# sndels/yuki

Hardware: AMD Instinct MI355X
Metric: Mray/s (primary+secondary), Path integrator @1080p (higher is better)
Workload: dtype f32; 1 GPU; cfg3: city 40x20 displaced icospheres, 1,024,012 triangles, SAH BVH (max_shapes_in_node 1), Path 8 bounces, Stratified 8x8, 1920x1080; triangles=1024012, spp=64, max_depth=8, tiles=8160, partition=single GPU, frames_in_flight=2

## Files before the change

yuki_amd/csrc/yk_context.cpp:

```cpp
#include <hip/hip_runtime.h>

#include <algorithm>
#include <chrono>
#include <cstdio>
#include <cstdlib>
#include <cstring>
#include <mutex>
#include <string>
#include <vector>

#include "yk_internal.h"

extern "C" {

uint32_t yk_abi_version(void) { return YK_ABI_VERSION; }

const char* yk_status_string(yk_status s) {
    switch (s) {
        case YK_OK: return "ok";
        case YK_ERR_INVALID_ARGUMENT: return "invalid argument";
        case YK_ERR_NO_DEVICE: return "no HIP device";
        case YK_ERR_DEVICE: return "HIP error";
        case YK_ERR_OUT_OF_MEMORY: return "out of device memory";
        case YK_ERR_UNSUPPORTED: return "unsupported on the device path";
        case YK_ERR_BVH_BUILD: return "BVH build failed";
        case YK_ERR_CANCELLED: return "cancelled";
        case YK_ERR_STACK_OVERFLOW: return "traversal stack overflow";
    }
    return "unknown";
}

yk_status yk_context_create(int device, yk_context** out) {
    if (!out) return YK_ERR_INVALID_ARGUMENT;
    *out = nullptr;
    int count = 0;
    if (hipGetDeviceCount(&count) != hipSuccess || count <= 0) return YK_ERR_NO_DEVICE;
    if (device < 0 || device >= count) return YK_ERR_INVALID_ARGUMENT;
    if (hipSetDevice(device) != hipSuccess) return YK_ERR_NO_DEVICE;
    yk_context* ctx = new yk_context();
    ctx->device = device;
    hipDeviceProp_t prop;
    if (hipGetDeviceProperties(&prop, device) == hipSuccess) ctx->n_cu = prop.multiProcessorCount;
    if (hipStreamCreateWithFlags(&ctx->stream, hipStreamNonBlocking) != hipSuccess ||
        hipEventCreateWithFlags(&ctx->ws[0].done, hipEventDisableTiming) != hipSuccess ||
        hipEventCreateWithFlags(&ctx->ws[1].done, hipEventDisableTiming) != hipSuccess ||
        hipEventCreateWithFlags(&ctx->ev_in, hipEventDisableTiming) != hipSuccess ||
        hipEventCreateWithFlags(&ctx->ev_out, hipEventDisableTiming) != hipSuccess ||
        hipStreamCreateWithFlags(&ctx->ws[0].side, hipStreamNonBlocking) != hipSuccess ||
        hipEventCreateWithFlags(&ctx->ws[0].ev_shade, hipEventDisableTiming) != hipSuccess ||
        hipEventCreateWithFlags(&ctx->ws[1].ev_shade, hipEventDisableTiming) != hipSuccess ||
        hipEventCreateWithFlags(&ctx->ws[0].ev_acc, hipEventDisableTiming) != hipSuccess ||
        hipEventCreateWithFlags(&ctx->ws[1].ev_acc, hipEventDisableTiming) != hipSuccess ||
        hipEventCreateWithFlags(&ctx->ws[0].ev_batch, hipEventDisableTiming) != hipSuccess ||
        hipEventCreateWithFlags(&ctx->ws[1].ev_batch, hipEventDisableTiming) != hipSuccess) {
        delete ctx;
        return YK_ERR_DEVICE;
    }
    ctx->ws[0].stream = ctx->stream;
    void* host_word = nullptr;
    if (hipHostMalloc(&host_word, 128, hipHostMallocMapped | hipHostMallocCoherent) == hipSuccess) {
        void* dev_word = nullptr;
        if (hipHostGetDevicePointer(&dev_word, host_word, 0) == hipSuccess) {
            ctx->cancel_host = static_cast<unsigned*>(host_word);
            ctx->cancel_host_dev = static_cast<const unsigned*>(dev_word);
            std::memset(host_word, 0, 128);
            ctx->cancel_host[16] = 1u;
        } else {
            (void)hipHostFree(host_word);
        }
    } else {
        (void)hipGetLastError();
    }
    if (const char* w = std::getenv("YK_WIDE_BVH")) ctx->wide_bvh = std::min(std::max(std::atoi(w), 0), 2);
    if (const char* w = std::getenv("YK_PACKET_BOUNCES")) ctx->packet_bounces = std::max(std::atoi(w), 0);
    if (const char* w = std::getenv("YK_PACKET_SHADOW_BOUNCES")) ctx->packet_shadow_bounces = std::max(std::atoi(w), 0);
    if (const char* w = std::getenv("YK_TOP_NODES")) ctx->top_nodes = std::min(std::max(std::atoi(w), 0), YK_TOP_MAX);
    *out = ctx;
    return YK_OK;
}

void yk_context_destroy(yk_context* ctx) {
    if (!ctx) return;
    (void)hipSetDevice(ctx->device);
    (void)hipStreamSynchronize(ctx->stream);
    if (ctx->ws[1].stream) (void)hipStreamSynchronize(ctx->ws[1].stream);
    for (WorkSet& w : ctx->ws) {
        for (int a = 0; a < 2; ++a)
            for (int b = 0; b < 4; ++b) w.path[a][b].release();
        DevBuf* wb[] = {&w.hit, &w.pend, &w.shO, &w.shD, &w.shC, &w.vis, &w.shq, &w.shO2, &w.shD2, &w.shq2, &w.ctrl, &w.spill, &w.spill_side};
        for (DevBuf* b : wb) b->release();
        if (w.done) (void)hipEventDestroy(w.done);
        if (w.ev_shade) (void)hipEventDestroy(w.ev_shade);
        if (w.ev_acc) (void)hipEventDestroy(w.ev_acc);
        if (w.ev_batch) (void)hipEventDestroy(w.ev_batch);
        if (w.side) {
            (void)hipStreamSynchronize(w.side);
            (void)hipStreamDestroy(w.side);
        }
    }
    if (ctx->ws[1].stream) (void)hipStreamDestroy(ctx->ws[1].stream);
    if (ctx->ev_in) (void)hipEventDestroy(ctx->ev_in);
    if (ctx->ev_out) (void)hipEventDestroy(ctx->ev_out);
    DevBuf* all[] = {&ctx->sample_buf, &ctx->pixel_xy, &ctx->pixel_aux, &ctx->tiles, &ctx->tile_off, &ctx->counters, &ctx->stats4, &ctx->hit4};
    for (DevBuf* b : all) b->release();
    for (DevBuf& b : ctx->scratch) b.release();
    ctx->tonemap.partials.release();
    ctx->tonemap.bounds.release();
    ctx->tonemap.samples.release();
    ctx->overlay.ids.release();
    if (ctx->tonemap.staging) (void)hipHostFree(ctx->tonemap.staging);
    if (ctx->tonemap.staged) (void)hipEventDestroy(ctx->tonemap.staged);
    for (hipEvent_t e : ctx->ev_pool) (void)hipEventDestroy(e);
    if (ctx->cancel_stream) {
        (void)hipStreamSynchronize(ctx->cancel_stream);
        (void)hipStreamDestroy(ctx->cancel_stream);
    }
    if (ctx->cancel_host) (void)hipHostFree(ctx->cancel_host);
    (void)hipStreamDestroy(ctx->stream);
    delete ctx;
}

yk_status yk_last_error(const yk_context* ctx, char* buf, size_t cap) {
    if (!ctx || !buf || cap == 0) return YK_ERR_INVALID_ARGUMENT;
    std::snprintf(buf, cap, "%s", ctx->last_error.c_str());
    return YK_OK;
}

void* yk_context_stream(const yk_context* ctx) { return ctx ? (void*)ctx->stream : nullptr; }

yk_status yk_context_set_option(yk_context* ctx, const char* key, int64_t value) {
    if (!ctx || !key) return YK_ERR_INVALID_ARGUMENT;
    YK_LOCK(ctx);
    std::string k(key);
    if (k == "batch_paths") {
        if (value < 64 || value > ((int64_t)1 << 29)) return YK_ERR_INVALID_ARGUMENT;
        ctx->batch_paths = value;
    } else if (k == "sample_buf_cap") {
        if (value < (1 << 20)) return YK_ERR_INVALID_ARGUMENT;
        ctx->sample_buf_cap = value;
    } else if (k == "streams") {
        if (value < 1 || value > 2) return YK_ERR_INVALID_ARGUMENT;
        ctx->streams = value;
    } else if (k == "packet_bounces") {
        if (value < 0) return YK_ERR_INVALID_ARGUMENT;
        ctx->packet_bounces = value;
    } else if (k == "packet_shadow_bounces") {
        if (value < 0) return YK_ERR_INVALID_ARGUMENT;
        ctx->packet_shadow_bounces = value;
    } else if (k == "shade_reorder") {
        ctx->shade_reorder = value != 0;
    } else if (k == "overlap_shadow") {
        ctx->overlap_shadow = value != 0;
    } else if (k == "top_nodes") {
        if (value < 0 || value > YK_TOP_MAX) return YK_ERR_INVALID_ARGUMENT;
        ctx->top_nodes = value;
    } else if (k == "wide_bvh") {
        if (value < 0 || value > 2) return YK_ERR_INVALID_ARGUMENT;
        ctx->wide_bvh = value;
    } else if (k == "bvh_builder") {
        if (value < 0 || value > 1) return YK_ERR_INVALID_ARGUMENT;
        ctx->bvh_builder = value;
    } else if (k == "bvh_small_range") {
        if (value < 0 || value > (1 << 20)) return YK_ERR_INVALID_ARGUMENT;
        ctx->bvh_small_range = value;
    } else if (k == "scene_layout") {
        if (value < 0 || value > 1) return YK_ERR_INVALID_ARGUMENT;
        ctx->scene_layout = value;
    } else if (k == "trace_stage_kernel") {
        if (value < 0 || value > 2) return YK_ERR_INVALID_ARGUMENT;
        ctx->trace_stage_kernel = value;
    } else if (k == "overlay_coop_min") {
        if (value < 1 || value > 65536) return YK_ERR_INVALID_ARGUMENT;
// ... 123 lines not shown
```

yuki_amd/csrc/yk_device.h:

```cpp
#pragma once
#include <hip/hip_runtime.h>
#include <stdint.h>

#include "../../include/yuki_hip.h"
#include "yk_bsdf.h"
#include "yk_rng.h"

namespace yk {

struct DevNode {
    float4 q0, q1, q2;
    uint4 q3;
};
static_assert(sizeof(DevNode) == 64, "DevNode must be 64 bytes");

#define YK_VIS_STRIDE(nl) ((nl) <= 4u ? 4u : (nl))
#define YK_LEAF_BIT 0x80000000u
#define YK_REF_NONE 0xffffffffu
#define YK_AXIS_SHIFT 28
#define YK_AXIS_MASK (3u << YK_AXIS_SHIFT)
#define YK_REF_INDEX_MAX ((1u << YK_AXIS_SHIFT) - 1u)
#define YK_TOP_BIT 0x40000000u
#define YK_TOP_MAX 1023

struct DevNode4 {
    float4 q0, q1, q2, q3, q4, q5;
    uint4 q6, q7;
};
static_assert(sizeof(DevNode4) == 128, "DevNode4 must be 128 bytes");

struct DevLight {
    uint32_t kind;
    float p[3];
    float i[3];
    float cos_total_width, cos_falloff_start;
    float w2l[16];
    float s2w[16];
    float n[3];
    float area;
};

struct DevSphere {
    float o2w[16];
    float w2o[16];
    float radius;
    int material;
    unsigned swaps_handedness;
    unsigned pad;
};

#define YK_PRIM_LAST 1u
#define YK_PRIM_SPHERE 2u
#define YK_PRIM_KIND_SHIFT 4
#define YK_HIT_KIND_SHIFT 28
#define YK_HIT_PRIM_MASK 0x0fffffffu
#define YK_HIT_WORD(prim, pflags) ((int)((prim) | ((((pflags) >> YK_PRIM_KIND_SHIFT) & 7u) << YK_HIT_KIND_SHIFT)))

#define YK_MESH_NORMALS 1u
#define YK_MESH_UVS 2u
#define YK_MESH_SWAPS 4u

struct DevScene {
    const DevNode* nodes;
    const DevNode4* nodes4;
    const DevNode* top_nodes;
    uint32_t n_top;
    const DevNode* top_nodes_any;
    uint32_t n_top_any;
    const float4* tris;
    const uint4* prim_shade;
    const float4* prim_attr;
    const DevSphere* spheres;
    uint32_t n_triangles;
    uint32_t root_ref;
    float root_bmin[3], root_bmax[3];
    const uint32_t* indices;
    const float* points;
    const float* normals;
    const float* uvs;
    const uint32_t* tri_mesh;
    const int32_t* tri_material;
    const int32_t* tri_area_light;
    const uint32_t* mesh_flags;
    const Material* materials;
    const DevLight* lights;
    uint32_t n_lights;
    float background[3];
    const float4* texels;
    const uint4* tex_info;
};

struct DevCamera {
    float c2w[16];
    float r2c[16];
};

struct PathBuffers {
    float4* rayO;
    float4* rayD;
    float4* thru;
    uint4* rngs;
};

#define YK_CTRL_WORDS 1024
#define YK_CTRL_ERR 3
#define YK_CTRL_CANCELLED 2
#define YK_CTRL_CAM_O (YK_CTRL_WORDS + 32)
#define YK_CTRL_ALLOC_WORDS (YK_CTRL_WORDS + 64)
#define YK_CTRL_HEADS 8
#define YK_CTRL_STRIDE 8
#define YK_CTRL_BOUNCE(b) (8 + YK_CTRL_STRIDE * (b))
#define YK_CTRL_SHQ 1
#define YK_CTRL_SHQ2 2
#define YK_CTRL_HEAD 3
#define YK_CTRL_MAX_DEPTH ((YK_CTRL_WORDS - 8) / YK_CTRL_STRIDE - 1)

struct CancelRef {
    const unsigned* host;
    unsigned* dev;
};
#define YK_HEAD_POISON 0xC0000000u

__device__ __forceinline__ bool cancel_raised(const CancelRef& c) { return c.dev && *c.dev != 0u; }
__device__ __forceinline__ bool cancel_relay(const CancelRef& c, unsigned* head) {
    if (!c.host || __hip_atomic_load(c.host, __ATOMIC_RELAXED, __HIP_MEMORY_SCOPE_SYSTEM) == 0u) return false;
    atomicOr(c.dev, 1u);
    atomicMax(head, YK_HEAD_POISON);
    return true;
}

struct RenderParams {
    SamplerCfg sampler;
    uint32_t max_depth;
    uint32_t has_clamp;
    float clamp;
    uint32_t integrator;
    uint32_t spe;
    uint32_t sample_base;
    CancelRef cancel;
};

__device__ __forceinline__ void split_sample_id(uint32_t sid, uint32_t spe, uint32_t& entry, uint32_t& k) {
    if ((spe & (spe - 1u)) == 0u) {
        entry = sid >> (31u - (uint32_t)__clz((int)spe));
        k = sid & (spe - 1u);
    } else {
        entry = sid / spe;
        k = sid % spe;
    }
}

}
```

yuki_amd/csrc/yk_internal.h:

```cpp
#pragma once
#include <hip/hip_runtime.h>

#include <atomic>
#include <chrono>
#include <memory>
#include <mutex>
#include <string>
#include <vector>

#include "yk_device.h"
#include "yk_host.h"
#include "yk_kernels.h"

using namespace yk;

struct DevBuf {
    void* p = nullptr;
    size_t bytes = 0;
    hipError_t ensure(size_t want) {
        if (want <= bytes) return hipSuccess;
        if (p) (void)hipFree(p);
        p = nullptr;
        bytes = 0;
        hipError_t e = hipMalloc(&p, want);
        if (e == hipSuccess) bytes = want;
        return e;
    }
    void release() {
        if (p) (void)hipFree(p);
        p = nullptr;
        bytes = 0;
    }
    template <class T> T* as() const { return reinterpret_cast<T*>(p); }
};

#define YK_BVH_SMALL_RANGE 32

struct yk_context {
    int device = 0;
    hipStream_t stream = nullptr;
    std::string last_error;
    int n_cu = 256;
    int64_t batch_paths = 128 << 20;
    int64_t packet_bounces = 1;
    int64_t packet_shadow_bounces = 1;
    int64_t shade_reorder = 1;
    int64_t overlap_shadow = 1;
    int64_t wide_bvh = 2;
    int64_t top_nodes = YK_TOP_MAX;
    int64_t bvh_builder = 0;
    int64_t bvh_small_range = YK_BVH_SMALL_RANGE;
    int64_t scene_layout = 0;
    int64_t trace_stage_kernel = 0;
    int64_t sample_buf_cap = (int64_t)64 << 30;
    int64_t time_kernels = 1;
    int64_t streams = 2;
    struct WorkSet {
        DevBuf path[2][4];
        DevBuf hit, pend, shO, shD, shC, vis, shq, shO2, shD2, shq2, ctrl, spill, spill_side;
        size_t cap_paths = 0;
        unsigned cap_lights = 0, cap_area = 0, cap_delta = 0;
        hipStream_t stream = nullptr;
        hipStream_t side = nullptr;
        hipEvent_t done = nullptr, ev_shade = nullptr, ev_acc = nullptr;
        hipEvent_t ev_batch = nullptr;
    } ws[2];
    DevBuf sample_buf, pixel_xy, pixel_aux, tiles, tile_off, counters, stats4, hit4, scratch[8];
    std::vector<hipEvent_t> ev_pool;
    hipEvent_t ev_in = nullptr, ev_out = nullptr;
    unsigned* cancel_host = nullptr;
    const unsigned* cancel_host_dev = nullptr;
    hipStream_t cancel_stream = nullptr;
    bool want_cancel_stream = false;
    std::atomic<bool> cancel_raised{false};
    struct ToneMapState {
        DevBuf partials, bounds, samples;
        uint32_t* staging = nullptr;
        size_t staging_words = 0;
        hipEvent_t staged = nullptr;
    } tonemap;
    struct OverlayState {
        DevBuf ids;
        int64_t coop_min = 32;
    } overlay;
    std::recursive_mutex mu;
};

typedef yk_context::WorkSet WorkSet;
static const uint32_t YK_WIDE_MAX_PATHS = 6u << 20;

struct DeviceTree {
    DevBuf nodes, depth, order;
    uint32_t n_nodes = 0, n_shapes = 0;
    uint32_t root_words[8] = {};
    void release() {
        nodes.release();
        depth.release();
        order.release();
    }
};

struct yk_scene {
    int device = -1;
    std::shared_ptr<const HostBvh> bvh;
    std::shared_ptr<HostBvh> bvh_lazy;
    DevBuf tree_nodes, tree_order;
    mutable std::once_flag tree_once;
    mutable std::atomic<uint32_t> tree_fetched{1};
    yk_scene_layout_info layout = {};
    size_t record_bytes[7] = {};
    uint32_t n_triangles = 0, n_spheres = 0, n_lights = 0, n_delta_lights = 0;
    bool wide_auto = false;
    yk_scene_info info;
    yk_bvh_build_info build_info;
    std::vector<uint8_t> shape_kind;
    DevBuf nodes, nodes4, top_nodes, top_nodes_any, tris, prim_shade, prim_attr, indices, points, normals, uvs, tri_mesh, tri_material, tri_area_light, mesh_flags, materials, lights, spheres, texels, tex_info;
    DevScene dev;
    bool on_device = false;
};

static inline DevScene dev_scene_for(const yk_scene* scene, uint64_t n) {
    DevScene ds = scene->dev;
    if (scene->wide_auto && n > YK_WIDE_MAX_PATHS) ds.nodes4 = nullptr;
    return ds;
}

struct yk_tile_list {
    int device = -1;
    std::vector<yk_tile> tiles;
    std::vector<uint16_t> samples;
    std::vector<uint32_t> off;
    DevBuf pixel_xy, pixel_sample;
};

static inline yk_status fail(yk_context* ctx, yk_status st, const std::string& msg) {
    if (ctx) ctx->last_error = msg;
    return st;
}

#define YK_LOCK(ctx) std::lock_guard<std::recursive_mutex> yk_lock_((ctx)->mu)
#define HIP_TRY(ctx, expr)                                                                                           \
    do {                                                                                                             \
        hipError_t _e = (expr);                                                                                      \
        if (_e != hipSuccess) {                                                                                      \
            return fail(ctx, _e == hipErrorOutOfMemory ? YK_ERR_OUT_OF_MEMORY : YK_ERR_DEVICE,                       \
                        std::string(#expr) + ": " + hipGetErrorString(_e));                                          \
        }                                                                                                            \
    } while (0)

#define YK_CATCH(ctx)                                                                                         \
    catch (const std::bad_alloc&) { return fail(ctx, YK_ERR_OUT_OF_MEMORY, "host allocation failed"); }      \
    catch (const std::exception& e) { return fail(ctx, YK_ERR_INVALID_ARGUMENT, std::string("exception: ") + e.what()); }


struct SceneImage;
yk_status yk_build_scene_image(yk_context* opt_ctx, const yk_scene_desc* d, std::shared_ptr<SceneImage>& out, bool device_builder_allowed = true);
yk_status yk_upload_scene_image(yk_context* ctx, const std::shared_ptr<SceneImage>& img, yk_scene** out);

const HostBvh* scene_host_tree(const yk_scene* scene);

static inline double now_seconds() {
    return std::chrono::duration<double>(std::chrono::steady_clock::now().time_since_epoch()).count();
}

bool build_bvh_device(yk_context* ctx, const std::vector<ShapeBounds>& bounds, uint32_t max_shapes_in_node, uint32_t split_method, uint32_t small_range, HostBvh& out, yk_bvh_build_info& bi,
                      DeviceTree* keep = nullptr);
bool build_bvh_levels(const std::vector<ShapeBounds>& bounds, uint32_t max_shapes_in_node, uint32_t split_method, uint32_t small_range, HostBvh& out, yk_bvh_build_info& bi);

uint32_t layout_scene_device(yk_context* ctx, yk_scene* s, const DeviceTree& tree, const uint32_t* d_user_order, const uint8_t* d_mat_kind, bool has_attr, uint32_t tree_depth, bool* order_applied);

Material make_material(const yk_material_desc& m);
DevLight make_light(const yk_light_desc& l);

#define YK_COUNTER_BYTES 256
unsigned* error_block(yk_context* ctx);
CancelRef cancel_ref(yk_context* ctx);
yk_status ensure_work_buffers(yk_context* ctx, WorkSet& ws, size_t paths, unsigned n_lights, unsigned n_delta_lights);
yk_status ensure_spill(yk_context* ctx, WorkSet& ws);
unsigned trace_grid(const yk_context* ctx);
PathBuffers path_buffers(WorkSet& ws, int which);
yk_status make_params(yk_context* ctx, const yk_sampler_desc* smp, const yk_integrator_desc* integ, RenderParams& prm);

struct KernelTimer {
    yk_context* ctx;
    bool on;
    std::vector<std::pair<int, int>> spans[3];
    size_t used = 0;
    int begin(hipStream_t s) {
        if (!on) return -1;
        if (used + 2 > ctx->ev_pool.size()) {
            size_t old = ctx->ev_pool.size();
            ctx->ev_pool.resize(old + 256);
            for (size_t i = old; i < ctx->ev_pool.size(); ++i) (void)hipEventCreate(&ctx->ev_pool[i]);
        }
        int a = (int)used;
        used += 2;
        (void)hipEventRecord(ctx->ev_pool[a], s);
        return a;
    }
    void end(int a, int cls, hipStream_t s) {
        if (a < 0) return;
        (void)hipEventRecord(ctx->ev_pool[a + 1], s);
        spans[cls].push_back(std::make_pair(a, a + 1));
    }
    double total(int cls) {
        double ms = 0.0;
        for (auto& sp : spans[cls]) {
            float t = 0.0f;
            if (hipEventElapsedTime(&t, ctx->ev_pool[sp.first], ctx->ev_pool[sp.second]) == hipSuccess) ms += t;
        }
        return ms * 1e-3;
    }
};

bool packet_kernel_traces_bounce(const yk_context* ctx, const yk_scene* scene, unsigned b);
void run_bounces(yk_context* ctx, WorkSet& ws, hipStream_t st, const yk_scene* scene, const RenderParams& prm, const uint32_t* pixel_xy,
                 const uint32_t* sample_index_tab, float4* sample_buf, KernelTimer& kt, unsigned long long* counters, bool coherent,
                 uint32_t n_paths, uint32_t sid_base, bool lean_camera_bounce, uint32_t* n_shadow_launches = nullptr);
```

yuki_amd/csrc/yk_kernels.h:

```cpp
#pragma once
#include <hip/hip_runtime.h>

#include "yk_device.h"

namespace yk {

unsigned trace_block_size();
unsigned trace_spill_depth();
unsigned trace_top_nodes();
unsigned trace_top_nodes_any();
unsigned packet_blocks_per_cu();
void launch_trace_closest_packet(hipStream_t s, unsigned grid, const DevScene& sc, const float4* rayO, const float4* rayD, const unsigned* count_ptr,
                                 unsigned* head, int* hit_tri, unsigned long long* ray_counter, const float4* lean_origin = nullptr, CancelRef cancel = CancelRef{nullptr, nullptr});
void launch_trace_any_packet(hipStream_t s, unsigned grid, const DevScene& sc, const float4* shO, const float4* shD, const unsigned* slot_of,
                             const unsigned* count_ptr, unsigned* head, unsigned char* vis, unsigned long long* shadow_counter, CancelRef cancel = CancelRef{nullptr, nullptr});
unsigned trace_blocks_per_cu();

void launch_pixel_table(hipStream_t s, const yk_tile* tiles, const uint32_t* tile_offset, uint32_t n_tiles, uint32_t n_pixels, uint32_t* pixel_xy,
                        const uint16_t* tile_sample = nullptr, uint32_t* pixel_sample = nullptr);
void launch_pixel_table_one(hipStream_t s, const yk_tile& tile, uint32_t n_pixels, uint32_t* pixel_xy, uint32_t tile_sample, uint32_t* pixel_sample);
void launch_raygen(hipStream_t s, const DevCamera& cam, const RenderParams& prm, const uint32_t* pixel_xy, const uint32_t* pixel_sample, uint64_t work0,
                   uint32_t n, PathBuffers out, float4* sample_buf, unsigned* count, float4* lean_origin = nullptr, const uint4* pixel_aux = nullptr);
void launch_pixel_sampler(hipStream_t s, const SamplerCfg& cfg, const uint32_t* pixel_xy, uint32_t n_pixels, uint4* pixel_aux);
void launch_raygen_user(hipStream_t s, const RenderParams& prm, const float* o, const float* d, const uint16_t* pixel, const uint32_t* sample_index,
                        uint32_t dimension, uint32_t n, PathBuffers out, float4* sample_buf, uint32_t* pixel_xy, unsigned* ctrl);
void launch_trace_closest(hipStream_t s, unsigned grid, const DevScene& sc, const float4* rayO, const float4* rayD, const float* t_max_opt,
                          const unsigned* count_ptr, unsigned* head, int* hit_tri, float4* hit_out, uint4* stats_out, uint2* spill,
                          unsigned spill_stride, unsigned* ctrl, unsigned long long* ray_counter, const unsigned* cancel_host = nullptr);
void launch_whitted(hipStream_t s, unsigned grid, const DevScene& sc, const RenderParams& prm, const uint32_t* pixel_xy, const uint32_t* sample_index_tab,
                    PathBuffers cur, uint32_t n, float4* sample_buf, uint2* spill, unsigned spill_stride, unsigned* ctrl, unsigned long long* counters);
unsigned whitted_max_depth();
void launch_path_debug(hipStream_t s, unsigned grid, const DevScene& sc, const RenderParams& prm, const uint32_t* pixel_xy, const uint32_t* sample_index_tab,
                       PathBuffers cur, uint32_t n, float4* sample_buf, uint32_t* out_counts, float4* out_rays, unsigned ray_cap, uint32_t* out_n_rays,
                       float min_len, uint2* spill, unsigned spill_stride, unsigned* ctrl);
void launch_trace_any(hipStream_t s, unsigned grid, const DevScene& sc, const float4* shO, const float4* shD, const unsigned* slot_of,
                      const unsigned* count_ptr, unsigned* head, unsigned char* vis, uint2* spill, unsigned spill_stride, unsigned* ctrl,
                      unsigned long long* shadow_counter, const unsigned* cancel_host = nullptr);
void launch_shade(hipStream_t s, unsigned grid, const DevScene& sc, const RenderParams& prm, const uint32_t* pixel_xy, const uint32_t* sample_index_tab,
                  PathBuffers cur, PathBuffers nxt, const int* hit_tri, float4* pend, float4* shO, float4* shD, float4* shC, unsigned char* vis,
                  unsigned* shq, float4* shO2, float4* shD2, unsigned* shq2, unsigned* bc, unsigned split_delta, unsigned reorder, unsigned block_slots, unsigned sid_base, const float4* lean_origin);
void launch_accumulate(hipStream_t s, unsigned grid, const RenderParams& prm, PathBuffers cur, const float4* pend, const float4* shC,
                       const unsigned char* vis, unsigned nl, float4* sample_buf, const unsigned* bc, unsigned first, unsigned sid_base);
void launch_resolve(hipStream_t s, const float4* sample_buf, uint32_t n_pixels, uint32_t spp, float* out_rgb);
void launch_resolve_passes(hipStream_t s, const float4* sample_buf, uint32_t n_pixels, uint32_t n_passes, float* out_rgb, size_t pass_stride);
void launch_film_scatter(hipStream_t s, const uint32_t* pixel_xy, uint32_t n_pixels, const float* tile_rgb, uint32_t res_x, float* film_rgb, int accumulate,
                         uint32_t n_passes = 1, size_t pass_stride = 0);
void launch_debug_shade(hipStream_t s, const DevScene& sc, uint32_t integrator, PathBuffers cur, const int* hit_tri, const uint4* stats, uint32_t n,
                        float4* sample_buf);
void launch_device_math(hipStream_t s, int fn, size_t n, const float* a, const float* b, float* out);
void launch_sampler_sequence(hipStream_t s, const SamplerCfg& cfg, uint32_t px, uint32_t py, uint32_t sample_index, const uint8_t* dims, size_t n_draws,
                             float* out);
void launch_light_test(hipStream_t s, const DevLight& L, int index, size_t n, const float* p, const float* ng, const float* u, float* out);
void launch_bsdf_test(hipStream_t s, const Material& m, size_t n, const float* ng, const float* ns, const float* dpdu, const float* wo,
                      const float* wi_or_u, int sample, float* out);
void launch_pack_rays(hipStream_t s, size_t n, const float* o, const float* d, float4* rayO, float4* rayD);
void launch_pack_shadow_rays(hipStream_t s, size_t n, const float* o, const float* d, const float* t_max, const int* area_light, float4* shO,
                             float4* shD);
void launch_unpack_rays(hipStream_t s, size_t n, const float4* rayO, const float4* rayD, float* o, float* d);

}
```

yuki_amd/csrc/yk_kernels.hip:

```cpp
#include <hip/hip_runtime.h>

#include "yk_device.h"
#include "yk_geom.h"
#include "yk_kernels.h"
#include "yk_rng.h"
#include "yk_shade.h"
#include "yk_wave.h"

namespace yk {

__global__ void k_pixel_table(const yk_tile* tiles, const uint32_t* tile_offset, uint32_t n_tiles, uint32_t n_pixels,
                              uint32_t* pixel_xy, const uint16_t* tile_sample, uint32_t* pixel_sample) {
    uint32_t i = blockIdx.x * blockDim.x + threadIdx.x;
    if (i >= n_pixels) return;
    uint32_t lo = 0, hi = n_tiles;
    while (hi - lo > 1) {
        uint32_t mid = (lo + hi) >> 1;
        if (tile_offset[mid] <= i)
            lo = mid;
        else
            hi = mid;
    }
    yk_tile t = tiles[lo];
    uint32_t w = (uint32_t)t.x1 - t.x0;
    uint32_t r = i - tile_offset[lo];
    uint32_t x = t.x0 + r % w, y = t.y0 + r / w;
    pixel_xy[i] = x | (y << 16);
    if (tile_sample) pixel_sample[i] = tile_sample[lo];
}

__global__ void k_pixel_table_one(yk_tile t, uint32_t n_pixels, uint32_t* pixel_xy, uint32_t tile_sample, uint32_t* pixel_sample) {
    uint32_t i = blockIdx.x * blockDim.x + threadIdx.x;
    if (i >= n_pixels) return;
    uint32_t w = (uint32_t)t.x1 - t.x0;
    pixel_xy[i] = (t.x0 + i % w) | ((t.y0 + i / w) << 16);
    if (pixel_sample) pixel_sample[i] = tile_sample;
}

__global__ void k_pixel_sampler(SamplerCfg cfg, const uint32_t* pixel_xy, uint32_t n_pixels, uint4* pixel_aux) {
    uint32_t i = blockIdx.x * blockDim.x + threadIdx.x;
    if (i >= n_pixels) return;
    const uint32_t xy = pixel_xy[i];
    const PixelSampler ps = pixel_sampler(cfg, xy & 0xffffu, xy >> 16);
    pixel_aux[i] = make_uint4((unsigned)ps.stream, (unsigned)(ps.stream >> 32), ps.hash0, 0u);
}

__device__ __forceinline__ void camera_ray(const DevCamera& cam, float fx, float fy, V3& o, V3& d) {
    V3 p_camera = xf_point(cam.r2c, V3{fx, fy, 0.0f});
    V3 dir = normalize(p_camera);
    o = xf_point(cam.c2w, V3{0.0f, 0.0f, 0.0f});
    d = xf_vector(cam.c2w, dir);
}

__global__ void k_raygen(DevCamera cam, RenderParams prm, const uint32_t* pixel_xy, const uint32_t* pixel_sample, uint64_t work0, uint32_t n,
                         PathBuffers out, float4* sample_buf, unsigned* count, float4* lean_origin, const uint4* pixel_aux) {
    uint32_t i = blockIdx.x * blockDim.x + threadIdx.x;
    if (cancel_raised(prm.cancel)) return;
    if (i == 0) *count = n;
    if (i >= n) return;
    const uint32_t w = (uint32_t)(work0 + i);
    uint32_t pix, ks;
    split_sample_id(w, prm.spe, pix, ks);
    const uint32_t s = (pixel_sample ? pixel_sample[pix] : prm.sample_base) + ks;
    uint32_t xy = pixel_xy[pix];
    uint32_t px = xy & 0xffffu, py = xy >> 16;
    SamplerState st;
    float ux, uy;
    if (pixel_aux) {
        const uint4 a = pixel_aux[pix];
        PixelSampler ps;
        ps.stream = (u64)a.x | ((u64)a.y << 32);
        ps.hash0 = a.z;
        st = sampler_start_camera(prm.sampler, ps, px, py, s, ux, uy);
    } else {
        st = sampler_start(prm.sampler, px, py, s, 0);
        sampler_get_2d(prm.sampler, st, ux, uy);
    }
    V3 o, d;
    camera_ray(cam, (float)px + ux, (float)py + uy, o, d);
    if (lean_origin) {
        if (i == 0) *lean_origin = make_float4(o.x, o.y, o.z, __uint_as_float(0u));
    } else {
        out.rayO[i] = make_float4(o.x, o.y, o.z, __uint_as_float(0u));
        out.thru[i] = make_float4(1.0f, 1.0f, 1.0f, __uint_as_float(st.dimension));
    }
    out.rayD[i] = make_float4(d.x, d.y, d.z, __uint_as_float((uint32_t)w));
    out.rngs[i] = make_uint4((unsigned)st.rng.state, (unsigned)(st.rng.state >> 32), (unsigned)st.rng.inc, (unsigned)(st.rng.inc >> 32));
    if (prm.integrator != YK_INTEGRATOR_PATH || prm.max_depth == 0) sample_buf[w] = make_float4(0.0f, 0.0f, 0.0f, 0.0f);
}

__global__ void k_raygen_user(RenderParams prm, const float* ray_o, const float* ray_d, const uint16_t* pixel, const uint32_t* sample_index,
                              uint32_t dimension, uint32_t n, PathBuffers out, float4* sample_buf, uint32_t* pixel_xy, unsigned* count) {
    uint32_t i = blockIdx.x * blockDim.x + threadIdx.x;
    if (i == 0) *count = n;
    if (i >= n) return;
    uint32_t px = pixel[2 * i], py = pixel[2 * i + 1];
    pixel_xy[i] = px | (py << 16);
    SamplerState st = sampler_start(prm.sampler, px, py, sample_index[i], dimension);
    if (prm.sampler.kind == 1) st.dimension = dimension;
    out.rayO[i] = make_float4(ray_o[3 * i], ray_o[3 * i + 1], ray_o[3 * i + 2], __uint_as_float(0u));
    out.rayD[i] = make_float4(ray_d[3 * i], ray_d[3 * i + 1], ray_d[3 * i + 2], __uint_as_float(i));
    out.thru[i] = make_float4(1.0f, 1.0f, 1.0f, __uint_as_float(st.dimension));
    out.rngs[i] = make_uint4((unsigned)st.rng.state, (unsigned)(st.rng.state >> 32), (unsigned)st.rng.inc, (unsigned)(st.rng.inc >> 32));
    if (prm.integrator != YK_INTEGRATOR_PATH || prm.max_depth == 0) sample_buf[i] = make_float4(0.0f, 0.0f, 0.0f, 0.0f);
}

#ifndef SHADE_CAP
#define SHADE_CAP 335
#endif
#ifndef SHADE_CAPQ
#define SHADE_CAPQ 768
#endif
#ifndef SHADE_WIN
#define SHADE_WIN 8
#endif
#ifndef SHADE_MIN_WAVES
#define SHADE_MIN_WAVES 3
#endif
template <int CAP, int CAPQ> struct ShadeStaging {
    float4 pO[CAP], pD[CAP], pT[CAP];
    uint4 pR[CAP];
    float4 qO[CAPQ], qD[CAPQ];
    unsigned qS[CAPQ];
    unsigned fill_p, fill_q, gbase;
    unsigned q_delta;
    unsigned cancel;
    unsigned bucket[8];
    unsigned short order[SHADE_WIN * 256];
};

__device__ __forceinline__ unsigned block_append(bool want, unsigned* lds_fill) {
    unsigned long long mask = __ballot(want);
    unsigned total = (unsigned)__popcll(mask);
    unsigned prefix = (unsigned)__popcll(mask & ((1ull << lane_id()) - 1ull));
    unsigned base = 0;
    if (total && lane_id() == 0) base = atomicAdd(lds_fill, total);
    base = __shfl(base, 0);
    return base + prefix;
}

__device__ __forceinline__ unsigned valid_light_kind(const DevScene& sc, unsigned l) { return sc.lights[l].kind; }

#ifdef YK_SHADE_PROFILE
#include "../../tools/micro/shade_profile.h"
#else
#define YK_PROF_DECL
#define YK_PROF_STAMP(k)
#define YK_PROF_FLUSH
#endif

template <int BLOCK, int CAP, int CAPQ>
__global__ __launch_bounds__(BLOCK, SHADE_MIN_WAVES) void k_shade(DevScene sc, RenderParams prm, const uint32_t* pixel_xy, const uint32_t* sample_index_tab,
                                                 PathBuffers cur, PathBuffers nxt,
                                                 const int* hit_tri, float4* pend, float4* shO, float4* shD, float4* shC, unsigned char* vis,
                                                 unsigned* shq, float4* shO2, float4* shD2, unsigned* shq2, unsigned* bc, unsigned split_delta, unsigned reorder,
                                                 unsigned win_max, unsigned block_slots, unsigned sid_base, const float4* __restrict__ lean_origin) {
    const unsigned win_iters = min(win_max, max(1u, bc[0] / (BLOCK * block_slots)));
    static_assert(sizeof(ShadeStaging<CAP, CAPQ>) <= 53296, "k_shade: more LDS than the measured 53296 bytes per block (42 granules = 53760 cost the third block per CU)");
    __shared__ ShadeStaging<CAP, CAPQ> stg;
    const unsigned nl = sc.n_lights;
    unsigned* next_count = bc + YK_CTRL_STRIDE;
    unsigned* shq_count = bc + YK_CTRL_SHQ;
    if (threadIdx.x == 0) {
        stg.fill_p = 0;
        stg.fill_q = 0;
        stg.q_delta = 0;
        stg.cancel = cancel_raised(prm.cancel) ? 1u : 0u;
    }
    __syncthreads();
    const unsigned n = __builtin_amdgcn_readfirstlane((int)stg.cancel) ? 0u : bc[0];
    auto flush_q = [&](unsigned fill, unsigned delta) {
        if (threadIdx.x == 0) stg.gbase = atomicAdd(delta ? bc + YK_CTRL_SHQ2 : shq_count, fill);
        __syncthreads();
        const unsigned gb = stg.gbase;
        float4* dO = delta ? shO2 : shO;
        float4* dD = delta ? shD2 : shD;
        unsigned* dS = delta ? shq2 : shq;
        for (unsigned k = threadIdx.x; k < fill; k += BLOCK) {
            dO[gb + k] = stg.qO[k];
            dD[gb + k] = stg.qD[k];
            dS[gb + k] = stg.qS[k];
        }
        __syncthreads();
        if (threadIdx.x == 0) stg.fill_q = 0;
        __syncthreads();
    };
    auto flush_p = [&](unsigned fill) {
        if (threadIdx.x == 0) stg.gbase = atomicAdd(next_count, fill);
        __syncthreads();
        const unsigned gb = stg.gbase;
        for (unsigned k = threadIdx.x; k < fill; k += BLOCK) {
            nxt.rayO[gb + k] = stg.pO[k];
            nxt.rayD[gb + k] = stg.pD[k];
            nxt.thru[gb + k] = stg.pT[k];
            nxt.rngs[gb + k] = stg.pR[k];
        }
        __syncthreads();
        if (threadIdx.x == 0) stg.fill_p = 0;
        __syncthreads();
    };
    const bool per_iter = !split_delta && BLOCK * nl <= (unsigned)CAPQ;
    const unsigned WIN = win_iters * BLOCK;
    const unsigned n_win = (n + WIN - 1) / WIN;
    YK_PROF_DECL
    for (unsigned w = blockIdx.x; w < n_win; w += gridDim.x) {
      const unsigned wbase = w * WIN;
      unsigned n_sub = win_iters;
      YK_PROF_STAMP(0)
      if (reorder) {
        if (threadIdx.x < 8) stg.bucket[threadIdx.x] = 0;
        __syncthreads();
        unsigned key[SHADE_WIN], rank[SHADE_WIN];
#pragma unroll
        for (int k = 0; k < SHADE_WIN; ++k) {
            const unsigned i0 = wbase + k * BLOCK + threadIdx.x;
            const bool in = (unsigned)k < win_iters && i0 < n;
            const int t = in ? hit_tri[i0] : -1;
            key[k] = !in ? 7u : (t < 0 ? 6u : ((unsigned)t >> YK_HIT_KIND_SHIFT));
        }
#pragma unroll
        for (int k = 0; k < SHADE_WIN; ++k) {
            rank[k] = 0;
            if ((unsigned)k >= win_iters) continue;
            for (unsigned q = 0; q < 8; ++q) {
                const unsigned long long m = __ballot(key[k] == q);
                if (m == 0ull) continue;
                unsigned b0 = 0;
                if (lane_id() == 0) b0 = atomicAdd(&stg.bucket[q], (unsigned)__popcll(m));
                b0 = __shfl(b0, 0);
                if (key[k] == q) rank[k] = b0 + (unsigned)__popcll(m & ((1ull << lane_id()) - 1ull));
            }
        }
        __syncthreads();
        unsigned first[8];
        {
            unsigned acc = 0;
            for (unsigned q = 0; q < 8; ++q) {
                first[q] = acc;
                acc += stg.bucket[q];
            }
            n_sub = (acc - stg.bucket[7] + BLOCK - 1) / BLOCK;
        }
#pragma unroll
        for (int k = 0; k < SHADE_WIN; ++k)
            if ((unsigned)k < win_iters) stg.order[first[key[k]] + rank[k]] = (unsigned short)(k * BLOCK + threadIdx.x);
        __syncthreads();
      } else {
        const unsigned left = n - wbase;
        n_sub = left >= WIN ? win_iters : (left + BLOCK - 1) / BLOCK;
      }
      for (unsigned sub = 0; sub < n_sub; ++sub) {
        const unsigned i = wbase + (reorder ? (unsigned)stg.order[sub * BLOCK + threadIdx.x] : sub * BLOCK + threadIdx.x);
        const bool valid = i < n;
        bool alive = false;
        YK_PROF_STAMP(1)
        if (per_iter) {
            __syncthreads();
            const unsigned fq = stg.fill_q, fp = stg.fill_p, staged = stg.q_delta;
            __syncthreads();
            if (fq && fq + BLOCK * nl > CAPQ) flush_q(fq, staged);
            if (fp + BLOCK > CAP) flush_p(fp);
        }
        float4 nO = make_float4(0, 0, 0, 0), nD = nO, nT = nO;
        uint4 nR = make_uint4(0, 0, 0, 0);
        V3 o = V3{0, 0, 0}, d = V3{0, 0, 1};
        RGB beta = RGB{0, 0, 0};
        unsigned flags = 0, sid = 0, bounces = 0;
        bool specular_bounce = false, hit = false;
        SamplerState st;
        st.rng.state = 0;
        st.rng.inc = 1;
        st.px = st.py = st.sample_index = st.dimension = 0;
        PathVertex v;
        v.sf.p = v.sf.n = v.sf.ns = v.sf.dpdus = v.sf.wo = V3{0, 0, 1};
        v.sf.material = 0;
        v.sf.area_light = -1;
        v.sf.u = v.sf.v = 0.0f;
        v.mat.kind = MK_BLACK;
        v.fr.s = v.fr.t = v.fr.n = v.fr.ng = V3{0, 0, 1};
        v.wo = V3{0, 0, 1};
        if (valid) {
            float4 a, c;
            const float4 b = cur.rayD[i];
            if (lean_origin) {
                a = *lean_origin;
                c = make_float4(1.0f, 1.0f, 1.0f, __uint_as_float(2u));
            } else {
                a = cur.rayO[i];
                c = cur.thru[i];
            }
            uint4 r = cur.rngs[i];
            o = f4_xyz(a);
            d = f4_xyz(b);
            flags = __float_as_uint(a.w);
            sid = __float_as_uint(b.w);
            beta = RGB{c.x, c.y, c.z};
            bounces = flags & 0xffu;
            specular_bounce = (flags >> 8) & 1u;
            st = path_sampler(prm, pixel_xy, sample_index_tab, r, __float_as_uint(c.w), sid);
            int tri = hit_tri[i];
            hit = tri >= 0;
            if (hit) vertex_setup(sc, (uint32_t)tri & YK_HIT_PRIM_MASK, o, d, v);
        }
        YK_PROF_STAMP(2)
        const unsigned vs = YK_VIS_STRIDE(nl);
        unsigned vword = 0u;
        for (unsigned l = 0; l < nl; ++l) {
            const unsigned slot = i * nl + l, vslot = i * vs + l;
            NeeSample ne;
            ne.want = false;
            ne.contrib = RGB{0, 0, 0};
            ne.so = V3{0, 0, 0};
            ne.sd = V3{0, 0, 1};
            ne.al = -1;
            if (valid && hit) ne = vertex_light(sc, prm, st, l, v);
            const bool want = ne.want;
            if (vs == 4u)
                vword |= (want ? 1u : 0u) << (8u * l);
            else if (valid)
                vis[vslot] = want ? 1 : 0;
            if (!per_iter) {
                __syncthreads();
                const unsigned f = stg.fill_q, staged = stg.q_delta;
                const unsigned delta = (split_delta && valid_light_kind(sc, l) != YK_LIGHT_RECT) ? 1u : 0u;
                __syncthreads();
                if (f && (staged != delta || f + BLOCK > CAPQ)) flush_q(f, staged);
                if (threadIdx.x == 0) stg.q_delta = delta;
            }
            unsigned q = block_append(want, &stg.fill_q);
            if (want) {
                stg.qO[q] = make_float4(ne.so.x, ne.so.y, ne.so.z, 0.9999f);
                stg.qD[q] = make_float4(ne.sd.x, ne.sd.y, ne.sd.z, __uint_as_float((unsigned)ne.al));
                stg.qS[q] = vslot;
                shC[slot] = make_float4(ne.contrib.r, ne.contrib.g, ne.contrib.b, 0.0f);
            }
        }
        if (vs == 4u && valid) reinterpret_cast<unsigned*>(vis)[i] = vword;
        YK_PROF_STAMP(3)
        if (valid) {
            unsigned kind = 0;
            RGB term = RGB{0, 0, 0};
            if (!hit) {
                term = vertex_miss_term(sc, beta);
                kind = YK_PEND_MISS;
            } else {
                VertexEnd e = vertex_finish(sc, prm, st, v, beta, bounces, specular_bounce);
                term = e.term;
                kind = e.kind;
                alive = e.alive;
                if (e.sampled) {
                    nO = make_float4(e.no.x, e.no.y, e.no.z, __uint_as_float((bounces & 0xffu) | (specular_bounce ? 0x100u : 0u)));
                    nD = make_float4(e.wi.x, e.wi.y, e.wi.z, __uint_as_float(sid));
                    nT = make_float4(beta.r, beta.g, beta.b, __uint_as_float(st.dimension));
                    nR = make_uint4((unsigned)st.rng.state, (unsigned)(st.rng.state >> 32), (unsigned)st.rng.inc, (unsigned)(st.rng.inc >> 32));
                }
            }
            pend[i] = make_float4(term.r, term.g, term.b, __uint_as_float((kind << YK_PEND_KIND_SHIFT) | (sid - sid_base)));
        }
        YK_PROF_STAMP(4)
        if (!per_iter) {
            __syncthreads();
            const unsigned f = stg.fill_p;
            __syncthreads();
            if (f + BLOCK > CAP) flush_p(f);
        }
        unsigned j = block_append(alive, &stg.fill_p);
        if (alive) {
            stg.pO[j] = nO;
            stg.pD[j] = nD;
            stg.pT[j] = nT;
            stg.pR[j] = nR;
        }
        YK_PROF_STAMP(5)
      }
      if (reorder) __syncthreads();
    }
    YK_PROF_FLUSH
    __syncthreads();
    {
        const unsigned fq = stg.fill_q, fp = stg.fill_p;
        if (fq) flush_q(fq, stg.q_delta);
        if (fp) flush_p(fp);
    }
}

__global__ void k_accumulate(RenderParams prm, PathBuffers cur, const float4* pend, const float4* shC, const unsigned char* vis, unsigned nl,
                             float4* sample_buf, const unsigned* bc, unsigned first, unsigned sid_base) {
    const unsigned n = cancel_raised(prm.cancel) ? 0u : bc[0];
    for (unsigned i = blockIdx.x * blockDim.x + threadIdx.x; i < n; i += gridDim.x * blockDim.x) {
        float4 p = pend[i];
        const unsigned kind = __float_as_uint(p.w) >> YK_PEND_KIND_SHIFT;
        const unsigned sid = sid_base + (__float_as_uint(p.w) & YK_PEND_SID_MASK);
        RGB beta = RGB{1.0f, 1.0f, 1.0f};
        if (!first && !(kind & YK_PEND_MISS)) {
            const float4 c = cur.thru[i];
            beta = RGB{c.x, c.y, c.z};
        }
        RGB L = RGB{0.0f, 0.0f, 0.0f};
        if (!first) {
            const float4 acc = sample_buf[sid];
            L = RGB{acc.x, acc.y, acc.z};
        }
        RGB radiance = RGB{0.0f, 0.0f, 0.0f};
        if (!(kind & YK_PEND_MISS)) {
            const unsigned vs = YK_VIS_STRIDE(nl);
            const unsigned vword = vs == 4u ? reinterpret_cast<const unsigned*>(vis)[i] : 0u;
            for (unsigned l = 0; l < nl; ++l) {
                const unsigned slot = i * nl + l;
                const unsigned verdict = vs == 4u ? (vword >> (8u * l)) & 255u : (unsigned)vis[i * vs + l];
                if (verdict == 1u) {
                    float4 ct = shC[slot];
                    radiance = radiance + RGB{ct.x, ct.y, ct.z};
                }
            }
        }
        L = vertex_accumulate(prm, L, beta, radiance, RGB{p.x, p.y, p.z}, kind);
        sample_buf[sid] = make_float4(L.r, L.g, L.b, 0.0f);
    }
}

__global__ void k_resolve(const float4* sample_buf, uint32_t n_pixels, uint32_t spp, float* out_rgb) {
    uint32_t p = blockIdx.x * blockDim.x + threadIdx.x;
    if (p >= n_pixels) return;
    RGB color = RGB{0.0f, 0.0f, 0.0f};
    const float4* s = sample_buf + (size_t)p * spp;
    uint32_t k = 0;
    for (; k + 8 <= spp; k += 8) {
        float4 v[8];
#pragma unroll
        for (int j = 0; j < 8; ++j) v[j] = s[k + j];
#pragma unroll
        for (int j = 0; j < 8; ++j) color = color + RGB{v[j].x, v[j].y, v[j].z};
    }
    for (; k < spp; ++k) {
        float4 v = s[k];
        color = color + RGB{v.x, v.y, v.z};
    }
    color = color / (float)spp;
    out_rgb[3 * (size_t)p + 0] = color.r;
    out_rgb[3 * (size_t)p + 1] = color.g;
    out_rgb[3 * (size_t)p + 2] = color.b;
}

__global__ void k_resolve_passes(const float4* sample_buf, uint32_t n_pixels, uint32_t n_passes, float* out_rgb, size_t pass_stride) {
    const size_t i = (size_t)blockIdx.x * blockDim.x + threadIdx.x;
    if (i >= (size_t)n_pixels * n_passes) return;
    const uint32_t p = (uint32_t)(i / n_passes), k = (uint32_t)(i % n_passes);
    const float4 v = sample_buf[i];
    float* o = out_rgb + (size_t)k * pass_stride + 3 * (size_t)p;
    o[0] = v.x;
    o[1] = v.y;
    o[2] = v.z;
}

__global__ void k_film_scatter(const uint32_t* pixel_xy, uint32_t n_pixels, const float* tile_rgb, uint32_t res_x, float* film_rgb, int accumulate,
                               uint32_t n_passes, size_t pass_stride) {
    uint32_t p = blockIdx.x * blockDim.x + threadIdx.x;
    if (p >= n_pixels) return;
    uint32_t xy = pixel_xy[p];
    size_t dst = (size_t)(xy >> 16) * res_x + (xy & 0xffffu);
    if (accumulate) {
        float r = film_rgb[3 * dst + 0], g = film_rgb[3 * dst + 1], b = film_rgb[3 * dst + 2];
        for (uint32_t k = 0; k < n_passes; ++k) {
            const float* t = tile_rgb + (size_t)k * pass_stride + 3 * (size_t)p;
            r += t[0];
            g += t[1];
            b += t[2];
        }
        film_rgb[3 * dst + 0] = r;
        film_rgb[3 * dst + 1] = g;
        film_rgb[3 * dst + 2] = b;
        return;
    }
    film_rgb[3 * dst + 0] = tile_rgb[3 * (size_t)p + 0];
    film_rgb[3 * dst + 1] = tile_rgb[3 * (size_t)p + 1];
    film_rgb[3 * dst + 2] = tile_rgb[3 * (size_t)p + 2];
}

__global__ void k_debug_shade(DevScene sc, uint32_t integrator, PathBuffers cur, const int* hit_tri, const uint4* stats, uint32_t n,
                              float4* sample_buf) {
    uint32_t i = blockIdx.x * blockDim.x + threadIdx.x;
    if (i >= n) return;
    unsigned sid = __float_as_uint(cur.rayD[i].w);
    int tri = hit_tri[i];
    RGB c = RGB{0.0f, 0.0f, 0.0f};
    if (integrator == YK_INTEGRATOR_BVH_INTERSECTIONS) {
        uint4 s = stats[i];
        c = RGB{(float)s.x, (float)s.y, tri >= 0 ? (float)s.y : 0.0f};
    } else if (tri >= 0 && integrator == YK_INTEGRATOR_SHADING_UVS) {
        V3 o = f4_xyz(cur.rayO[i]), d = f4_xyz(cur.rayD[i]);
        Surface sf = hit_surface_prim(sc, (uint32_t)tri & YK_HIT_PRIM_MASK, o, d, true);
        c = RGB{sf.u, sf.v, 0.0f};
    } else if (tri >= 0) {
        V3 o = f4_xyz(cur.rayO[i]), d = f4_xyz(cur.rayD[i]);
        Surface sf = hit_surface_prim(sc, (uint32_t)tri & YK_HIT_PRIM_MASK, o, d);
        V3 nn = integrator == YK_INTEGRATOR_GEOMETRY_NORMALS ? sf.n : sf.ns;
// ... 99 lines not shown
        out[8 * i + 4] = s.f.g;
        out[8 * i + 5] = s.f.b;
        out[8 * i + 6] = s.pdf;
        out[8 * i + 7] = (float)s.type;
    }
}

__global__ void k_light_test(DevLight L, int index, size_t n, const float* p, const float* ng, const float* u, float* out) {
    size_t i = blockIdx.x * (size_t)blockDim.x + threadIdx.x;
    if (i >= n) return;
    const V3 sp = ld3(p, (uint32_t)i), nn = ld3(ng, (uint32_t)i);
    LightSample ls = sample_light(L, index, sp, u[2 * i], u[2 * i + 1]);
    V3 offset = nn * 0.001f;
    V3 so = dot(ls.p1 - sp, nn) > 0.0f ? sp + offset : sp - offset;
    V3 sd = ls.p1 - so;
    float* o = out + 18 * i;
    o[0] = ls.l.x; o[1] = ls.l.y; o[2] = ls.l.z;
    o[3] = ls.li.r; o[4] = ls.li.g; o[5] = ls.li.b;
    o[6] = ls.pdf;
    o[7] = ls.has_vis ? 1.0f : 0.0f;
    o[8] = (float)ls.area_light;
    o[9] = ls.p1.x; o[10] = ls.p1.y; o[11] = ls.p1.z;
    o[12] = so.x; o[13] = so.y; o[14] = so.z;
    o[15] = sd.x; o[16] = sd.y; o[17] = sd.z;
}

__global__ void k_pack_rays(size_t n, const float* o, const float* d, float4* rayO, float4* rayD) {
    size_t i = blockIdx.x * (size_t)blockDim.x + threadIdx.x;
    if (i >= n) return;
    rayO[i] = make_float4(o[3 * i], o[3 * i + 1], o[3 * i + 2], 0.0f);
    rayD[i] = make_float4(d[3 * i], d[3 * i + 1], d[3 * i + 2], 0.0f);
}
__global__ void k_pack_shadow_rays(size_t n, const float* o, const float* d, const float* t_max, const int* area_light, float4* shO, float4* shD) {
    size_t i = blockIdx.x * (size_t)blockDim.x + threadIdx.x;
    if (i >= n) return;
    shO[i] = make_float4(o[3 * i], o[3 * i + 1], o[3 * i + 2], t_max[i]);
    shD[i] = make_float4(d[3 * i], d[3 * i + 1], d[3 * i + 2], __uint_as_float((unsigned)(area_light ? area_light[i] : -1)));
}
__global__ void k_unpack_rays(size_t n, const float4* rayO, const float4* rayD, float* o, float* d) {
    size_t i = blockIdx.x * (size_t)blockDim.x + threadIdx.x;
    if (i >= n) return;
    float4 a = rayO[i], b = rayD[i];
    o[3 * i] = a.x; o[3 * i + 1] = a.y; o[3 * i + 2] = a.z;
    d[3 * i] = b.x; d[3 * i + 1] = b.y; d[3 * i + 2] = b.z;
}

#ifdef YK_SHADE_PROFILE
}
extern "C" int yk_debug_shade_profile(unsigned long long* out8, int reset) {
    unsigned long long zero[8] = {0, 0, 0, 0, 0, 0, 0, 0};
    (void)hipDeviceSynchronize();
    int rc = (int)hipMemcpyFromSymbol(out8, HIP_SYMBOL(yk::yk_shade_prof), sizeof(zero));
    if (reset) rc |= (int)hipMemcpyToSymbol(HIP_SYMBOL(yk::yk_shade_prof), zero, sizeof(zero));
    return rc;
}
namespace yk {
#endif

static inline unsigned blocks_for(size_t n, unsigned bs) { return (unsigned)((n + bs - 1) / bs); }

void launch_pixel_table(hipStream_t s, const yk_tile* tiles, const uint32_t* tile_offset, uint32_t n_tiles, uint32_t n_pixels, uint32_t* pixel_xy,
                        const uint16_t* tile_sample, uint32_t* pixel_sample) {
    if (!n_pixels) return;
    hipLaunchKernelGGL(k_pixel_table, dim3(blocks_for(n_pixels, 256)), dim3(256), 0, s, tiles, tile_offset, n_tiles, n_pixels, pixel_xy, tile_sample,
                       pixel_sample);
}
void launch_pixel_table_one(hipStream_t s, const yk_tile& tile, uint32_t n_pixels, uint32_t* pixel_xy, uint32_t tile_sample, uint32_t* pixel_sample) {
    if (!n_pixels) return;
    hipLaunchKernelGGL(k_pixel_table_one, dim3(blocks_for(n_pixels, 256)), dim3(256), 0, s, tile, n_pixels, pixel_xy, tile_sample, pixel_sample);
}
void launch_pixel_sampler(hipStream_t s, const SamplerCfg& cfg, const uint32_t* pixel_xy, uint32_t n_pixels, uint4* pixel_aux) {
    if (!n_pixels) return;
    hipLaunchKernelGGL(k_pixel_sampler, dim3(blocks_for(n_pixels, 256)), dim3(256), 0, s, cfg, pixel_xy, n_pixels, pixel_aux);
}
void launch_raygen(hipStream_t s, const DevCamera& cam, const RenderParams& prm, const uint32_t* pixel_xy, const uint32_t* pixel_sample, uint64_t work0,
                   uint32_t n, PathBuffers out, float4* sample_buf, unsigned* count, float4* lean_origin, const uint4* pixel_aux) {
    hipLaunchKernelGGL(k_raygen, dim3(blocks_for(n, 256)), dim3(256), 0, s, cam, prm, pixel_xy, pixel_sample, work0, n, out, sample_buf, count, lean_origin, pixel_aux);
}
void launch_raygen_user(hipStream_t s, const RenderParams& prm, const float* o, const float* d, const uint16_t* pixel, const uint32_t* sample_index,
                        uint32_t dimension, uint32_t n, PathBuffers out, float4* sample_buf, uint32_t* pixel_xy, unsigned* ctrl) {
    hipLaunchKernelGGL(k_raygen_user, dim3(blocks_for(n, 256)), dim3(256), 0, s, prm, o, d, pixel, sample_index, dimension, n, out, sample_buf,
                       pixel_xy, ctrl);
}
void launch_shade(hipStream_t s, unsigned grid, const DevScene& sc, const RenderParams& prm, const uint32_t* pixel_xy, const uint32_t* sample_index_tab,
                  PathBuffers cur, PathBuffers nxt,
                  const int* hit_tri, float4* pend, float4* shO, float4* shD, float4* shC, unsigned char* vis, unsigned* shq, float4* shO2,
                  float4* shD2, unsigned* shq2, unsigned* bc, unsigned split_delta, unsigned reorder, unsigned block_slots, unsigned sid_base, const float4* lean_origin) {
    hipLaunchKernelGGL((k_shade<256, SHADE_CAP, SHADE_CAPQ>), dim3(grid), dim3(256), 0, s, sc, prm, pixel_xy, sample_index_tab, cur, nxt, hit_tri, pend, shO, shD, shC, vis, shq,
                       shO2, shD2, shq2, bc, split_delta, reorder, (unsigned)SHADE_WIN, block_slots, sid_base, lean_origin);
}
void launch_accumulate(hipStream_t s, unsigned grid, const RenderParams& prm, PathBuffers cur, const float4* pend, const float4* shC,
                       const unsigned char* vis, unsigned nl, float4* sample_buf, const unsigned* bc, unsigned first, unsigned sid_base) {
    hipLaunchKernelGGL(k_accumulate, dim3(grid), dim3(256), 0, s, prm, cur, pend, shC, vis, nl, sample_buf, bc, first, sid_base);
}
void launch_resolve(hipStream_t s, const float4* sample_buf, uint32_t n_pixels, uint32_t spp, float* out_rgb) {
    if (!n_pixels) return;
    hipLaunchKernelGGL(k_resolve, dim3(blocks_for(n_pixels, 256)), dim3(256), 0, s, sample_buf, n_pixels, spp, out_rgb);
}
void launch_resolve_passes(hipStream_t s, const float4* sample_buf, uint32_t n_pixels, uint32_t n_passes, float* out_rgb, size_t pass_stride) {
    if (!n_pixels) return;
    hipLaunchKernelGGL(k_resolve_passes, dim3(blocks_for((size_t)n_pixels * n_passes, 256)), dim3(256), 0, s, sample_buf, n_pixels, n_passes, out_rgb, pass_stride);
}
void launch_film_scatter(hipStream_t s, const uint32_t* pixel_xy, uint32_t n_pixels, const float* tile_rgb, uint32_t res_x, float* film_rgb, int accumulate,
                         uint32_t n_passes, size_t pass_stride) {
    if (!n_pixels) return;
    hipLaunchKernelGGL(k_film_scatter, dim3(blocks_for(n_pixels, 256)), dim3(256), 0, s, pixel_xy, n_pixels, tile_rgb, res_x, film_rgb, accumulate, n_passes, pass_stride);
}
void launch_debug_shade(hipStream_t s, const DevScene& sc, uint32_t integrator, PathBuffers cur, const int* hit_tri, const uint4* stats, uint32_t n,
                        float4* sample_buf) {
    hipLaunchKernelGGL(k_debug_shade, dim3(blocks_for(n, 256)), dim3(256), 0, s, sc, integrator, cur, hit_tri, stats, n, sample_buf);
}
void launch_device_math(hipStream_t s, int fn, size_t n, const float* a, const float* b, float* out) {
    hipLaunchKernelGGL(k_device_math, dim3(blocks_for(n, 256)), dim3(256), 0, s, fn, n, a, b, out);
}
void launch_sampler_sequence(hipStream_t s, const SamplerCfg& cfg, uint32_t px, uint32_t py, uint32_t sample_index, const uint8_t* dims, size_t n_draws,
                             float* out) {
    hipLaunchKernelGGL(k_sampler_sequence, dim3(1), dim3(64), 0, s, cfg, px, py, sample_index, dims, n_draws, out);
}
void launch_light_test(hipStream_t s, const DevLight& L, int index, size_t n, const float* p, const float* ng, const float* u, float* out) {
    hipLaunchKernelGGL(k_light_test, dim3(blocks_for(n, 256)), dim3(256), 0, s, L, index, n, p, ng, u, out);
}
void launch_bsdf_test(hipStream_t s, const Material& m, size_t n, const float* ng, const float* ns, const float* dpdu, const float* wo,
                      const float* wi_or_u, int sample, float* out) {
    hipLaunchKernelGGL(k_bsdf_test, dim3(blocks_for(n, 256)), dim3(256), 0, s, m, n, ng, ns, dpdu, wo, wi_or_u, sample, out);
}
void launch_pack_rays(hipStream_t s, size_t n, const float* o, const float* d, float4* rayO, float4* rayD) {
    hipLaunchKernelGGL(k_pack_rays, dim3(blocks_for(n, 256)), dim3(256), 0, s, n, o, d, rayO, rayD);
}
void launch_pack_shadow_rays(hipStream_t s, size_t n, const float* o, const float* d, const float* t_max, const int* area_light, float4* shO,
                             float4* shD) {
    hipLaunchKernelGGL(k_pack_shadow_rays, dim3(blocks_for(n, 256)), dim3(256), 0, s, n, o, d, t_max, area_light, shO, shD);
}
void launch_unpack_rays(hipStream_t s, size_t n, const float4* rayO, const float4* rayD, float* o, float* d) {
    hipLaunchKernelGGL(k_unpack_rays, dim3(blocks_for(n, 256)), dim3(256), 0, s, n, rayO, rayD, o, d);
}

}
```

yuki_amd/csrc/yk_packet.hip:

```cpp
#include <hip/hip_runtime.h>

#include "yk_device.h"
#include "yk_geom.h"
#include "yk_kernels.h"
#include "yk_traverse.h"
#include "yk_wave.h"

namespace yk {

#define YK_PKT_STACK 64
#define YK_PKT_BLOCK 256

__device__ __forceinline__ unsigned uni(unsigned v) { return (unsigned)__builtin_amdgcn_readfirstlane((int)v); }
__device__ __forceinline__ unsigned long long uni64(unsigned long long v) { return (unsigned long long)uni((unsigned)v) | ((unsigned long long)uni((unsigned)(v >> 32)) << 32); }
__device__ __forceinline__ bool in_mask(unsigned long long m) { return (m >> lane_id()) & 1ull; }

struct PktStack {
    uint4* base;
    __device__ __forceinline__ void push(int sp, unsigned ref, unsigned which, unsigned long long mask) {
        if (lane_id() == 0) base[sp] = make_uint4(ref, which, (unsigned)mask, (unsigned)(mask >> 32));
    }
    __device__ __forceinline__ void at(int sp, unsigned& ref, unsigned& which, unsigned long long& mask) const {
        const uint4 e = base[sp];
        ref = uni(e.x);
// ... 33 lines not shown
    int sp = 0;
    for (;;) {
        bool need_pop = false;
        if (cur & YK_LEAF_BIT) {
            leaf_closest<SPHERES, true, false>(sc, cur & ~YK_LEAF_BIT, in_mask(cmask), r, nullptr, [&](unsigned prim, float4, unsigned pflags, const TriHit&) {
                best = YK_HIT_WORD(prim, pflags);
            });
            need_pop = true;
        } else {
            const NodeBoxes nb = load_node_uniform(sc.nodes, cur);
            const bool mine = in_mask(cmask);
            float t0, t1;
            const float t_def = deferred_t_max(r.t_max);
            const bool r0 = mine && slab(nb.lo0, nb.hi0, r.o, r.inv, t_def, t0);
            const bool r1 = mine && slab(nb.lo1, nb.hi1, r.o, r.inv, t_def, t1);
            const bool h0 = r0 && t0 <= r.t_max, h1 = r1 && t1 <= r.t_max;
            const unsigned long long m0 = __ballot(h0), m1 = __ballot(h1);
            const bool swap = (sg >> nb.axis) & 1u;
            const unsigned near_ref = swap ? nb.ref1 : nb.ref0, far_ref = swap ? nb.ref0 : nb.ref1;
            const unsigned long long m_near = swap ? m1 : m0, m_far = swap ? m0 : m1;
            const unsigned long long m_far_def = __ballot(swap ? r0 : r1);
            if (m_near) {
                if (m_far_def) {
                    stk.push(sp, cur, swap ? 0u : 1u, m_far_def);
                    ++sp;
                }
                cur = near_ref;
                cmask = m_near;
            } else if (m_far) {
                cur = far_ref;
                cmask = m_far;
            } else {
                need_pop = true;
            }
        }
        if (need_pop) {
            for (;;) {
                if (sp == 0) return;
                --sp;
                unsigned parent, which;
                unsigned long long mask;
                stk.at(sp, parent, which, mask);
                const NodeBoxes nb = load_node_uniform(sc.nodes, parent);
                float t;
                const bool h = in_mask(mask) && (which ? slab(nb.lo1, nb.hi1, r.o, r.inv, r.t_max, t) : slab(nb.lo0, nb.hi0, r.o, r.inv, r.t_max, t));
                const unsigned long long m = __ballot(h);
                if (m) {
                    cur = which ? nb.ref1 : nb.ref0;
                    cmask = m;
                    break;
                }
            }
        }
    }
}

template <bool SPHERES>
__global__ __launch_bounds__(YK_PKT_BLOCK, 8) void k_trace_closest_packet(DevScene sc, const float4* __restrict__ rayO, const float4* __restrict__ rayD,
                                                                          const unsigned* count_ptr, unsigned* head, int* __restrict__ hit_tri,
                                                                          unsigned long long* ray_counter, const float4* __restrict__ lean_origin, CancelRef cancel) {
    __shared__ uint4 lds_stack[(YK_PKT_BLOCK / YK_WAVE) * YK_PKT_STACK];
    PktStack stk;
    stk.base = lds_stack + (threadIdx.x / YK_WAVE) * YK_PKT_STACK;
    const unsigned n = queue_length(count_ptr, cancel, ray_counter);
    claim_packets(n, head, cancel, [&](unsigned base) {
        const unsigned idx = base + lane_id();
        const bool valid = idx < n;
        const float4 ro = !valid ? make_float4(0, 0, 0, 0) : (rayO ? rayO[idx] : *lean_origin), rd = valid ? rayD[idx] : make_float4(0, 0, 1, 0);
        TraceRay r = ray_setup(f4_xyz(ro), f4_xyz(rd), __builtin_inff());
        const bool alive = valid && root_hit(sc, r);
        int best = -1;
        unsigned long long remaining = __ballot(alive);
        while (remaining) {
            const int first = __ffsll((long long)remaining) - 1;
            const unsigned sg = (unsigned)__builtin_amdgcn_readlane((int)r.negmask, first);
            const unsigned long long group = __ballot(alive && r.negmask == sg);
            remaining &= ~group;
            pkt_closest_group<SPHERES>(sc, stk, r, best, group, sg);
        }
        if (valid) hit_tri[idx] = best;
    });
}

template <bool SPHERES>
__global__ __launch_bounds__(YK_PKT_BLOCK, 8) void k_trace_any_packet(DevScene sc, const float4* __restrict__ shO, const float4* __restrict__ shD,
                                                                      const unsigned* __restrict__ slot_of, const unsigned* count_ptr, unsigned* head,
                                                                      unsigned char* __restrict__ vis, unsigned long long* shadow_counter, CancelRef cancel) {
    __shared__ uint4 lds_stack[(YK_PKT_BLOCK / YK_WAVE) * YK_PKT_STACK];
    PktStack stk;
    stk.base = lds_stack + (threadIdx.x / YK_WAVE) * YK_PKT_STACK;
    const unsigned n = queue_length(count_ptr, cancel, shadow_counter);
    claim_packets(n, head, cancel, [&](unsigned base) {
        const unsigned k = base + lane_id();
        const bool valid = k < n;
        const float4 ro = valid ? shO[k] : make_float4(0, 0, 0, 0), rd = valid ? shD[k] : make_float4(0, 0, 1, 0);
        const TraceRay r = ray_setup(f4_xyz(ro), f4_xyz(rd), ro.w);
        const int area_light = (int)__float_as_uint(rd.w);
        const unsigned slot = valid ? (slot_of ? slot_of[k] : k) : 0u;
        const bool alive = valid && root_hit(sc, r);
        bool occluded = false;
        unsigned long long cmask = __ballot(alive);
        if (cmask) {
            const unsigned sg = (unsigned)__builtin_amdgcn_readlane((int)r.negmask, __ffsll((long long)cmask) - 1);
            unsigned cur = sc.root_ref;
            int sp = 0;
            for (;;) {
                bool need_pop = false;
                if (cur & YK_LEAF_BIT) {
                    unsigned prim = cur & ~YK_LEAF_BIT;
                    for (;;) {
                        cf4* tq = as_const(sc.tris + 3 * prim);
                        const float4 v0 = ldc(tq, 0), v1 = ldc(tq, 1), v2 = ldc(tq, 2);
                        TriHit h;
                        if (in_mask(cmask) && !occluded && prim_hit<SPHERES>(sc, r, v0, v1, v2, h) && occludes(v0, area_light)) occluded = true;
                        if (__float_as_uint(v2.w) & YK_PRIM_LAST) break;
                        ++prim;
                    }
                    need_pop = true;
                } else {
                    const NodeBoxes nb = load_node_uniform(sc.nodes, cur);
                    const bool mine = in_mask(cmask) && !occluded;
                    float t0, t1;
                    const bool h0 = mine && slab(nb.lo0, nb.hi0, r.o, r.inv, r.t_max, t0);
                    const bool h1 = mine && slab(nb.lo1, nb.hi1, r.o, r.inv, r.t_max, t1);
                    const unsigned long long m0 = __ballot(h0), m1 = __ballot(h1);
                    const bool swap = (sg >> nb.axis) & 1u;
                    const unsigned near_ref = swap ? nb.ref1 : nb.ref0, far_ref = swap ? nb.ref0 : nb.ref1;
                    const unsigned long long m_near = swap ? m1 : m0, m_far = swap ? m0 : m1;
                    if (m_near) {
                        if (m_far) {
                            stk.push(sp, far_ref, 0u, m_far);
                            ++sp;
                        }
                        cur = near_ref;
                        cmask = m_near;
                    } else if (m_far) {
                        cur = far_ref;
                        cmask = m_far;
                    } else {
                        need_pop = true;
                    }
                }
                if (need_pop) {
                    const unsigned long long occ = __ballot(occluded);
                    bool done = false;
                    for (;;) {
                        if (sp == 0) {
                            done = true;
                            break;
                        }
                        --sp;
                        unsigned ref, which;
                        unsigned long long mask;
                        stk.at(sp, ref, which, mask);
                        mask &= ~occ;
                        if (mask) {
                            cur = ref;
                            cmask = mask;
                            break;
                        }
                    }
                    if (done) break;
                }
            }
        }
        if (valid) {
            if (occluded)
                vis[slot] = slot_of ? 2 : 1;
            else if (!slot_of)
                vis[slot] = 0;
        }
    });
}

unsigned packet_blocks_per_cu() { return 8u; }

void launch_trace_closest_packet(hipStream_t s, unsigned grid, const DevScene& sc, const float4* rayO, const float4* rayD, const unsigned* count_ptr,
                                 unsigned* head, int* hit_tri, unsigned long long* ray_counter, const float4* lean_origin, CancelRef cancel) {
    if (sc.spheres)
        hipLaunchKernelGGL((k_trace_closest_packet<true>), dim3(grid), dim3(YK_PKT_BLOCK), 0, s, sc, rayO, rayD, count_ptr, head, hit_tri, ray_counter, lean_origin, cancel);
    else
        hipLaunchKernelGGL((k_trace_closest_packet<false>), dim3(grid), dim3(YK_PKT_BLOCK), 0, s, sc, rayO, rayD, count_ptr, head, hit_tri, ray_counter, lean_origin, cancel);
}
void launch_trace_any_packet(hipStream_t s, unsigned grid, const DevScene& sc, const float4* shO, const float4* shD, const unsigned* slot_of,
                             const unsigned* count_ptr, unsigned* head, unsigned char* vis, unsigned long long* shadow_counter, CancelRef cancel) {
    if (sc.spheres)
        hipLaunchKernelGGL((k_trace_any_packet<true>), dim3(grid), dim3(YK_PKT_BLOCK), 0, s, sc, shO, shD, slot_of, count_ptr, head, vis, shadow_counter, cancel);
    else
        hipLaunchKernelGGL((k_trace_any_packet<false>), dim3(grid), dim3(YK_PKT_BLOCK), 0, s, sc, shO, shD, slot_of, count_ptr, head, vis, shadow_counter, cancel);
}

}
```

yuki_amd/csrc/yk_render.cpp:

```cpp
#include <hip/hip_runtime.h>

#include <algorithm>
#include <chrono>
#include <cstdio>
#include <cstdlib>
#include <cstring>
#include <mutex>
#include <string>
#include <thread>
#include <vector>

#include "yk_internal.h"
#ifdef YK_EXPERIMENT_SORT
#include "../../tools/micro/ray_sort_experiment.h"
#endif
#ifdef YK_EXPERIMENT_GRAPH
#include "../../tools/micro/graph_replay_experiment.h"
#endif

unsigned* error_block(yk_context* ctx) { return reinterpret_cast<unsigned*>(ctx->counters.as<unsigned long long>() + 16); }
CancelRef cancel_ref(yk_context* ctx) { return CancelRef{ctx->cancel_host_dev, ctx->cancel_host_dev ? error_block(ctx) + YK_CTRL_CANCELLED : nullptr}; }

yk_status ensure_work_buffers(yk_context* ctx, WorkSet& ws, size_t paths, unsigned n_lights, unsigned n_delta_lights) {
    HIP_TRY(ctx, ctx->counters.ensure(YK_COUNTER_BYTES));
    unsigned nl = std::max(1u, n_lights);
    unsigned na = nl, nd = std::max(1u, n_delta_lights);
    if (paths <= ws.cap_paths && nl <= ws.cap_lights && na <= ws.cap_area && nd <= ws.cap_delta) return YK_OK;
    paths = std::max(paths, ws.cap_paths);
    nl = std::max(nl, ws.cap_lights);
    na = std::max(na, ws.cap_area);
    nd = std::max(nd, ws.cap_delta);
    for (int a = 0; a < 2; ++a)
        for (int b = 0; b < 4; ++b) HIP_TRY(ctx, ws.path[a][b].ensure(paths * 16));
    HIP_TRY(ctx, ws.hit.ensure(paths * 4));
    HIP_TRY(ctx, ws.pend.ensure(paths * 16));
    HIP_TRY(ctx, ws.shC.ensure(paths * nl * 16));
    HIP_TRY(ctx, ws.vis.ensure(paths * YK_VIS_STRIDE(nl)));
    HIP_TRY(ctx, ws.shO.ensure(paths * na * 16));
    HIP_TRY(ctx, ws.shD.ensure(paths * na * 16));
    HIP_TRY(ctx, ws.shq.ensure(paths * na * 4));
    HIP_TRY(ctx, ws.shO2.ensure(paths * nd * 16));
    HIP_TRY(ctx, ws.shD2.ensure(paths * nd * 16));
    HIP_TRY(ctx, ws.shq2.ensure(paths * nd * 4));
    HIP_TRY(ctx, ws.ctrl.ensure(YK_CTRL_ALLOC_WORDS * 4));
    ws.cap_paths = paths;
    ws.cap_lights = nl;
    ws.cap_area = na;
    ws.cap_delta = nd;
    return YK_OK;
}

unsigned trace_grid(const yk_context* ctx) { return (unsigned)ctx->n_cu * trace_blocks_per_cu(); }

yk_status ensure_spill(yk_context* ctx, WorkSet& ws) {
    size_t threads = (size_t)trace_grid(ctx) * trace_block_size();
    HIP_TRY(ctx, ws.spill.ensure(threads * trace_spill_depth() * 8));
    HIP_TRY(ctx, ws.spill_side.ensure(threads * trace_spill_depth() * 8));
    return YK_OK;
}

PathBuffers path_buffers(WorkSet& ws, int which) {
    PathBuffers p;
    p.rayO = ws.path[which][0].as<float4>();
    p.rayD = ws.path[which][1].as<float4>();
    p.thru = ws.path[which][2].as<float4>();
    p.rngs = ws.path[which][3].as<uint4>();
    return p;
}

yk_status make_params(yk_context* ctx, const yk_sampler_desc* smp, const yk_integrator_desc* integ, RenderParams& prm) {
    if (!smp || !integ) return fail(ctx, YK_ERR_INVALID_ARGUMENT, "null sampler/integrator");
    std::memset(&prm, 0, sizeof(prm));
    prm.sampler.kind = smp->kind;
    prm.sampler.nx = smp->nx;
    prm.sampler.ny = smp->kind == YK_SAMPLER_UNIFORM ? 1 : smp->ny;
    prm.sampler.jitter = smp->jitter;
    prm.sampler.seed = smp->seed;
    if (smp->kind > 1 || prm.sampler.nx == 0 || prm.sampler.ny == 0) return fail(ctx, YK_ERR_INVALID_ARGUMENT, "bad sampler");
    uint64_t spp = (uint64_t)prm.sampler.nx * prm.sampler.ny;
    if (spp > 0xFFFFu) return fail(ctx, YK_ERR_INVALID_ARGUMENT, "samples per pixel exceed u16 (integrators/mod.rs:139)");
    prm.sampler.spp = (unsigned)spp;
    prm.spe = (unsigned)spp;
    prm.max_depth = integ->max_depth;
    prm.has_clamp = integ->has_clamp;
    prm.clamp = integ->indirect_clamp;
    prm.integrator = integ->kind;
    if (integ->kind == YK_INTEGRATOR_WHITTED && integ->max_depth > whitted_max_depth())
        return fail(ctx, YK_ERR_UNSUPPORTED, "Whitted: max_depth above 16 is not supported on the device");
    if (integ->kind > YK_INTEGRATOR_SHADING_UVS) return fail(ctx, YK_ERR_INVALID_ARGUMENT, "bad integrator kind");
    return YK_OK;
}


bool packet_kernel_traces_bounce(const yk_context* ctx, const yk_scene* scene, unsigned b) {
    return b < (unsigned)ctx->packet_bounces && scene->bvh->depth <= 64;
}

void run_bounces(yk_context* ctx, WorkSet& ws, hipStream_t st, const yk_scene* scene, const RenderParams& prm, const uint32_t* pixel_xy,
                        const uint32_t* sample_index_tab, float4* sample_buf, KernelTimer& kt, unsigned long long* counters, bool coherent,
                        uint32_t n_paths, uint32_t sid_base, bool lean_camera_bounce, uint32_t* n_shadow_launches) {
    unsigned* ctrl = ws.ctrl.as<unsigned>();
    unsigned* errblk = error_block(ctx);
    const DevScene ds = dev_scene_for(scene, n_paths);
    auto fit = [](unsigned full, uint64_t items) { return (unsigned)std::min<uint64_t>(full, std::max<uint64_t>(1, (items + 255) / 256)); };
    const uint64_t n_shadow_max = (uint64_t)n_paths * std::max(1u, scene->n_lights);
    const unsigned tg = fit(trace_grid(ctx), n_paths), tg_any = fit(trace_grid(ctx), n_shadow_max);
    const unsigned pg_full = (unsigned)ctx->n_cu * packet_blocks_per_cu();
    const unsigned pg = fit(pg_full, n_paths), pg_any = fit(pg_full, n_shadow_max);
    static const unsigned shade_bpc = std::getenv("YK_SHADE_BPC") ? (unsigned)std::atoi(std::getenv("YK_SHADE_BPC")) : 256u;
    const unsigned sg = fit((unsigned)ctx->n_cu * shade_bpc, n_paths);
    const unsigned spill_stride = trace_grid(ctx) * trace_block_size();
    unsigned cur = 0;
    const bool overlap = ctx->overlap_shadow != 0 && ws.side != nullptr;
    hipStream_t sb = overlap ? ws.side : st;
    for (unsigned b = 0; b < prm.max_depth; ++b) {
        PathBuffers pc = path_buffers(ws, (int)cur), pn = path_buffers(ws, (int)(cur ^ 1u));
        const bool packet = coherent && packet_kernel_traces_bounce(ctx, scene, b);
        const float4* lean_origin = (b == 0 && lean_camera_bounce) ? reinterpret_cast<const float4*>(ctrl + YK_CTRL_CAM_O) : nullptr;
        const bool packet_shadow = coherent && b < (unsigned)ctx->packet_shadow_bounces && scene->bvh->depth <= 64 && scene->n_delta_lights > 0;
        const bool split = packet_shadow && scene->n_lights > scene->n_delta_lights;
        const bool all_delta = packet_shadow && !split;
        unsigned* bc = ctrl + YK_CTRL_BOUNCE(b);
        int e = kt.begin(st);
        if (packet)
            launch_trace_closest_packet(st, pg, ds, lean_origin ? nullptr : pc.rayO, pc.rayD, bc, bc + YK_CTRL_HEAD, ws.hit.as<int>(), counters, lean_origin, prm.cancel);
        else {
            launch_trace_closest(st, tg, ds, pc.rayO, pc.rayD, nullptr, bc, bc + YK_CTRL_HEAD, ws.hit.as<int>(), nullptr, nullptr,
                                 ws.spill.as<uint2>(), spill_stride, errblk, counters, prm.cancel.host);
        }
        kt.end(e, 0, st);
        if (overlap && b > 0) (void)hipStreamWaitEvent(st, ws.ev_acc, 0);
        e = kt.begin(st);
        launch_shade(st, sg, ds, prm, pixel_xy, sample_index_tab, pc, pn, ws.hit.as<int>(), ws.pend.as<float4>(), ws.shO.as<float4>(),
                     ws.shD.as<float4>(), ws.shC.as<float4>(), ws.vis.as<unsigned char>(), ws.shq.as<unsigned>(), ws.shO2.as<float4>(),
                     ws.shD2.as<float4>(), ws.shq2.as<unsigned>(), bc, split ? 1u : 0u, (b > 0 && ctx->shade_reorder) ? 1u : 0u, 3u * (unsigned)ctx->n_cu, sid_base, lean_origin);
        kt.end(e, 2, st);
#ifdef YK_EXPERIMENT_SORT
        YK_SORT_AFTER_SHADE
#endif
        if (overlap) {
            (void)hipEventRecord(ws.ev_shade, st);
            (void)hipStreamWaitEvent(sb, ws.ev_shade, 0);
        }
        e = kt.begin(sb);
        uint2* any_spill = (overlap ? ws.spill_side : ws.spill).as<uint2>();
        if (all_delta) {
            launch_trace_any_packet(sb, pg_any, ds, ws.shO.as<float4>(), ws.shD.as<float4>(), ws.shq.as<unsigned>(), bc + YK_CTRL_SHQ,
                                    bc + YK_CTRL_HEAD + 1, ws.vis.as<unsigned char>(), counters + 1, prm.cancel);
        } else {
            launch_trace_any(sb, tg_any, ds, ws.shO.as<float4>(), ws.shD.as<float4>(), ws.shq.as<unsigned>(), bc + YK_CTRL_SHQ,
                             bc + YK_CTRL_HEAD + 1, ws.vis.as<unsigned char>(), any_spill, spill_stride, errblk, counters + 1, prm.cancel.host);
            if (split && n_shadow_launches) ++*n_shadow_launches;
            if (split)
                launch_trace_any_packet(sb, pg_any, ds, ws.shO2.as<float4>(), ws.shD2.as<float4>(), ws.shq2.as<unsigned>(), bc + YK_CTRL_SHQ2,
                                        bc + YK_CTRL_HEAD + 2, ws.vis.as<unsigned char>(), counters + 1, prm.cancel);
        }
        kt.end(e, 1, sb);
        if (n_shadow_launches) ++*n_shadow_launches;
        launch_accumulate(sb, sg, prm, pc, ws.pend.as<float4>(), ws.shC.as<float4>(), ws.vis.as<unsigned char>(), ds.n_lights, sample_buf, bc, b == 0 ? 1u : 0u, sid_base);
        if (overlap) (void)hipEventRecord(ws.ev_acc, sb);
        if (kt.on && std::getenv("YK_DEBUG_BOUNCES")) {
            unsigned h[YK_CTRL_STRIDE + 1];
            (void)hipStreamSynchronize(st);
            (void)hipStreamSynchronize(sb);
            (void)hipMemcpy(h, bc, sizeof(h), hipMemcpyDeviceToHost);
            float tt = 0, ts = 0, th = 0;
            (void)hipEventElapsedTime(&tt, ctx->ev_pool[kt.spans[0].back().first], ctx->ev_pool[kt.spans[0].back().second]);
            (void)hipEventElapsedTime(&ts, ctx->ev_pool[kt.spans[1].back().first], ctx->ev_pool[kt.spans[1].back().second]);
            (void)hipEventElapsedTime(&th, ctx->ev_pool[kt.spans[2].back().first], ctx->ev_pool[kt.spans[2].back().second]);
            std::fprintf(stderr, "bounce %u: rays %u trace %.3f ms (%.0f Mray/s) | shadow rays %u %.3f ms (%.0f Mray/s) | shade %.3f ms | survivors %u\n", b, h[0],
                         tt, h[0] / (tt * 1e3), h[YK_CTRL_SHQ] + h[YK_CTRL_SHQ2], ts, (h[YK_CTRL_SHQ] + h[YK_CTRL_SHQ2]) / (ts * 1e3), th, h[YK_CTRL_STRIDE]);
        }
        cur ^= 1u;
    }
    if (overlap) (void)hipStreamWaitEvent(st, ws.ev_acc, 0);
}

static double now_ms() { return std::chrono::duration<double, std::milli>(std::chrono::steady_clock::now().time_since_epoch()).count(); }
static const bool g_debug_cancel = std::getenv("YK_DEBUG_CANCEL") != nullptr;

static void raise_cancel(yk_context* ctx, bool from_render_thread = true) {
    if (!ctx->cancel_host) return;
    const double t0 = g_debug_cancel ? now_ms() : 0.0;
    ctx->cancel_raised.store(true, std::memory_order_release);
    __atomic_store_n(ctx->cancel_host, 1u, __ATOMIC_RELEASE);
    if (from_render_thread && !ctx->cancel_stream) ctx->want_cancel_stream = true;
    if (from_render_thread && ctx->cancel_stream && ctx->counters.p)
        (void)hipMemcpyAsync(error_block(ctx) + YK_CTRL_CANCELLED, ctx->cancel_host + 16, 4, hipMemcpyHostToDevice, ctx->cancel_stream);
    if (g_debug_cancel) std::fprintf(stderr, "[yk cancel] raise: %s, %.3f ms\n", ctx->cancel_stream ? "host word + device word" : "host word only (first interruption)", now_ms() - t0);
}

static yk_status clear_cancel(yk_context* ctx) {
    if (!ctx->cancel_host || !ctx->cancel_raised.load(std::memory_order_acquire)) return YK_OK;
    HIP_TRY(ctx, hipStreamSynchronize(ctx->stream));
    if (ctx->cancel_stream) HIP_TRY(ctx, hipStreamSynchronize(ctx->cancel_stream));
    for (WorkSet& w : ctx->ws) {
        if (w.stream && w.stream != ctx->stream) HIP_TRY(ctx, hipStreamSynchronize(w.stream));
        if (w.side) HIP_TRY(ctx, hipStreamSynchronize(w.side));
    }
    __atomic_store_n(ctx->cancel_host, 0u, __ATOMIC_RELEASE);
    ctx->cancel_raised.store(false, std::memory_order_release);
    if (ctx->want_cancel_stream && !ctx->cancel_stream) {
        if (hipStreamCreateWithFlags(&ctx->cancel_stream, hipStreamNonBlocking) != hipSuccess) ctx->cancel_stream = nullptr;
        ctx->want_cancel_stream = false;
    }
    return YK_OK;
}

static bool poll_until(yk_context* ctx, hipEvent_t done, yk_cancel_fn cancel, void* user) {
    while (hipEventQuery(done) == hipErrorNotReady) {
        if (cancel(user)) {
            raise_cancel(ctx);
            return true;
        }
        std::this_thread::sleep_for(std::chrono::microseconds(100));
    }
    return false;
}
static bool wait_polling(yk_context* ctx, hipEvent_t done, hipStream_t st, yk_cancel_fn cancel, void* user) {
    const bool fired = cancel ? poll_until(ctx, done, cancel, user) : false;
    (void)hipStreamSynchronize(st);
    return fired;
}

static yk_status render_tiles_impl(yk_context* ctx, const yk_scene* scene, const yk_camera* camera, const yk_sampler_desc* sampler,
                                   const yk_integrator_desc* integrator, const yk_tile* tiles, const uint16_t* tile_samples, size_t n_tiles,
                                   void* d_out_rgb, void* stream, yk_render_stats* stats, yk_cancel_fn cancel, void* user,
                                   const yk_tile_list* prepared = nullptr, uint32_t n_passes = 1, int64_t uniform_first_sample = -1) try {
    if (!ctx) return YK_ERR_INVALID_ARGUMENT;
    YK_LOCK(ctx);
    if (prepared) {
        if (prepared->device != ctx->device) return fail(ctx, YK_ERR_INVALID_ARGUMENT, "tile list was not created on this context's device");
        tiles = prepared->tiles.data();
        tile_samples = prepared->samples.empty() ? nullptr : prepared->samples.data();
        n_tiles = prepared->tiles.size();
    }
    if (!scene || !camera || !tiles || n_tiles == 0 || !d_out_rgb) return fail(ctx, YK_ERR_INVALID_ARGUMENT, "null argument");
    if (!scene->on_device || scene->device != ctx->device) return fail(ctx, YK_ERR_INVALID_ARGUMENT, "scene was not created on this context's device");
    RenderParams prm;
    yk_status ps = make_params(ctx, sampler, integrator, prm);
    if (ps != YK_OK) return ps;
    if (prm.integrator == YK_INTEGRATOR_PATH && prm.max_depth > YK_CTRL_MAX_DEPTH)
        return fail(ctx, YK_ERR_INVALID_ARGUMENT, "max_depth too large");
    (void)hipSetDevice(ctx->device);
    {
        yk_status cs = clear_cancel(ctx);
        if (cs != YK_OK) return cs;
    }
    hipStream_t caller = (hipStream_t)stream;
    hipStream_t st = ctx->stream;
    if (caller) {
        HIP_TRY(ctx, hipEventRecord(ctx->ev_in, caller));
        HIP_TRY(ctx, hipStreamWaitEvent(st, ctx->ev_in, 0));
    }
    struct HandBack {
        yk_context* c;
        hipStream_t caller, st;
        ~HandBack() {
            if (!caller) return;
            if (hipEventRecord(c->ev_out, st) == hipSuccess) (void)hipStreamWaitEvent(caller, c->ev_out, 0);
        }
    } hand_back{ctx, caller, st};

    std::vector<uint32_t> off(n_tiles + 1, 0);
    uint64_t total_px = 0;
    for (size_t t = 0; t < n_tiles; ++t) {
        if (tiles[t].x0 >= tiles[t].x1 || tiles[t].y0 >= tiles[t].y1) return fail(ctx, YK_ERR_INVALID_ARGUMENT, "Bounds2 with a dimension <= 0");
        total_px += (uint64_t)(tiles[t].x1 - tiles[t].x0) * (uint64_t)(tiles[t].y1 - tiles[t].y0);
        if (total_px > 0xFFFFFFFFull) return fail(ctx, YK_ERR_INVALID_ARGUMENT, "too many pixels in one call");
        off[t + 1] = (uint32_t)total_px;
    }
    const bool accumulating = tile_samples != nullptr || uniform_first_sample >= 0;
    if (tile_samples && uniform_first_sample >= 0) return fail(ctx, YK_ERR_INVALID_ARGUMENT, "an accumulating tile list carries its own sample indices");
    if (n_passes == 0 || n_passes > 0xFFFFu || (!accumulating && n_passes != 1)) return fail(ctx, YK_ERR_INVALID_ARGUMENT, "bad number of passes");
    const uint32_t spp = accumulating ? n_passes : prm.sampler.spp;
    prm.spe = spp;
    if (accumulating) {
        for (size_t t = 0; tile_samples && t < n_tiles; ++t)
            if ((uint64_t)tile_samples[t] + n_passes > prm.sampler.spp)
                return fail(ctx, YK_ERR_INVALID_ARGUMENT, "FilmTile.sample (+ passes) beyond the sampler's samples per pixel");
        if (uniform_first_sample >= 0 && (uint64_t)uniform_first_sample + n_passes > prm.sampler.spp)
            return fail(ctx, YK_ERR_INVALID_ARGUMENT, "first_sample (+ passes) beyond the sampler's samples per pixel");
        if (uniform_first_sample >= 0) prm.sample_base = (uint32_t)uniform_first_sample;
    }
    const bool sample_table = tile_samples != nullptr;
    uint64_t max_px_chunk = std::min<uint64_t>(0xFFFFFFF0ull / spp, (uint64_t)ctx->sample_buf_cap / (16ull * spp));
    if (max_px_chunk == 0) return fail(ctx, YK_ERR_INVALID_ARGUMENT, "sample_buf_cap too small for one pixel");

    DevCamera cam;
    std::memcpy(cam.c2w, camera->camera_to_world, 64);
    std::memcpy(cam.r2c, camera->raster_to_camera, 64);

    const bool is_path = prm.integrator == YK_INTEGRATOR_PATH;
    const uint64_t total_work = total_px * spp;
    size_t batch = (size_t)std::min<uint64_t>((uint64_t)ctx->batch_paths, total_work);
    const int n_ws = (ctx->streams >= 2 && is_path && !stream && total_work > batch) ? 2 : 1;
    {
        size_t free_b = 0, total_b = 0;
        if (batch > ctx->ws[0].cap_paths && hipMemGetInfo(&free_b, &total_b) == hipSuccess) {
            const size_t per_path = (148 + 53 * (size_t)std::max(1u, scene->n_lights) + 36) * (size_t)n_ws;
            const size_t fit = (free_b / 2) / per_path;
            if (fit >= 65536 && batch > fit) batch = fit;
        }
    }
    if (n_ws == 2 && !ctx->ws[1].stream) {
        HIP_TRY(ctx, hipStreamCreateWithFlags(&ctx->ws[1].stream, hipStreamNonBlocking));
        HIP_TRY(ctx, hipStreamCreateWithFlags(&ctx->ws[1].side, hipStreamNonBlocking));
    }
    for (int w = 0; w < n_ws; ++w) {
        yk_status wb = ensure_work_buffers(ctx, ctx->ws[w], batch, scene->n_lights, scene->n_delta_lights);
        if (wb != YK_OK) return wb;
        if ((wb = ensure_spill(ctx, ctx->ws[w])) != YK_OK) return wb;
    }
    HIP_TRY(ctx, ctx->tiles.ensure(n_tiles * sizeof(yk_tile)));
    HIP_TRY(ctx, ctx->tile_off.ensure((n_tiles + 1) * 4));
    if (!is_path && prm.integrator == YK_INTEGRATOR_BVH_INTERSECTIONS) HIP_TRY(ctx, ctx->stats4.ensure(batch * 16));

    unsigned long long* counters = ctx->counters.as<unsigned long long>();
    HIP_TRY(ctx, hipMemsetAsync(counters, 0, YK_COUNTER_BYTES, st));
    unsigned* errblk = error_block(ctx);
    prm.cancel = cancel_ref(ctx);
    KernelTimer kt;
    kt.ctx = ctx;
    kt.on = stats != nullptr && ctx->time_kernels != 0 && (total_work >= (1u << 20) || ctx->time_kernels > 1);
    struct EventPair {
        hipEvent_t a = nullptr, b = nullptr;
        ~EventPair() {
            if (a) (void)hipEventDestroy(a);
            if (b) (void)hipEventDestroy(b);
        }
    } frame_ev;
    hipEvent_t& ev0 = frame_ev.a;
    hipEvent_t& ev1 = frame_ev.b;
    if (stats) {
        HIP_TRY(ctx, hipEventCreate(&ev0));
        HIP_TRY(ctx, hipEventCreate(&ev1));
        HIP_TRY(ctx, hipEventRecord(ev0, st));
    }
#ifdef YK_EXPERIMENT_GRAPH
    YK_GRAPH_BEGIN
#endif
    uint32_t n_batches = 0, n_trace = 0, n_shadow = 0;
    float* out = reinterpret_cast<float*>(d_out_rgb);

    size_t t_begin = 0;
    while (t_begin < n_tiles) {
        size_t t_end = t_begin;
        while (t_end < n_tiles && (uint64_t)(off[t_end + 1] - off[t_begin]) <= max_px_chunk) ++t_end;
        if (t_end == t_begin) return fail(ctx, YK_ERR_INVALID_ARGUMENT, "a single tile exceeds sample_buf_cap");
        const uint32_t px0 = off[t_begin], npx = off[t_end] - off[t_begin];
        HIP_TRY(ctx, ctx->sample_buf.ensure((size_t)npx * spp * 16));
        float4* sample_buf = ctx->sample_buf.as<float4>();
        uint32_t* pixel_xy = nullptr;
        uint32_t* pixel_sample = nullptr;
        const uint16_t* d_tile_sample = nullptr;
        if (prepared) {
            pixel_xy = prepared->pixel_xy.as<uint32_t>() + px0;
            if (sample_table) pixel_sample = prepared->pixel_sample.as<uint32_t>() + px0;
        } else if (t_end - t_begin == 1) {
            HIP_TRY(ctx, ctx->pixel_xy.ensure((size_t)npx * 4));
            pixel_xy = ctx->pixel_xy.as<uint32_t>();
            if (sample_table) {
                HIP_TRY(ctx, ctx->scratch[5].ensure((size_t)npx * 4));
                pixel_sample = ctx->scratch[5].as<uint32_t>();
            }
            launch_pixel_table_one(st, tiles[t_begin], npx, pixel_xy, sample_table ? tile_samples[t_begin] : 0u, pixel_sample);
        } else {
        std::vector<uint32_t> loc(t_end - t_begin + 1);
        for (size_t t = t_begin; t <= t_end; ++t) loc[t - t_begin] = off[t] - px0;
        HIP_TRY(ctx, hipMemcpyAsync(ctx->tiles.p, tiles + t_begin, (t_end - t_begin) * sizeof(yk_tile), hipMemcpyHostToDevice, st));
        HIP_TRY(ctx, hipMemcpyAsync(ctx->tile_off.p, loc.data(), loc.size() * 4, hipMemcpyHostToDevice, st));
        HIP_TRY(ctx, hipStreamSynchronize(st));
        HIP_TRY(ctx, ctx->pixel_xy.ensure((size_t)npx * 4));
        pixel_xy = ctx->pixel_xy.as<uint32_t>();
        if (sample_table) {
            HIP_TRY(ctx, ctx->scratch[4].ensure((t_end - t_begin) * 2));
            HIP_TRY(ctx, ctx->scratch[5].ensure((size_t)npx * 4));
            HIP_TRY(ctx, hipMemcpyAsync(ctx->scratch[4].p, tile_samples + t_begin, (t_end - t_begin) * 2, hipMemcpyHostToDevice, st));
            d_tile_sample = ctx->scratch[4].as<uint16_t>();
            pixel_sample = ctx->scratch[5].as<uint32_t>();
        }
        launch_pixel_table(st, ctx->tiles.as<yk_tile>(), ctx->tile_off.as<uint32_t>(), (uint32_t)(t_end - t_begin), npx, pixel_xy, d_tile_sample, pixel_sample);
        }
        HIP_TRY(ctx, ctx->pixel_aux.ensure((size_t)npx * 16));
        launch_pixel_sampler(st, prm.sampler, pixel_xy, npx, ctx->pixel_aux.as<uint4>());
        if (n_ws == 2) {
            HIP_TRY(ctx, hipEventRecord(ctx->ws[0].done, st));
            HIP_TRY(ctx, hipStreamWaitEvent(ctx->ws[1].stream, ctx->ws[0].done, 0));
        }

        const uint64_t work = (uint64_t)npx * spp;
        int which = 0;
        bool ws_busy[2] = {false, false};
        for (uint64_t w0 = 0; w0 < work; w0 += batch) {
            WorkSet& ws = ctx->ws[which];
            bool fired = cancel && ws_busy[which] && poll_until(ctx, ws.ev_batch, cancel, user);
            if (!fired && cancel && cancel(user)) {
                raise_cancel(ctx);
                fired = true;
            }
            if (fired) {
                const double t0 = g_debug_cancel ? now_ms() : 0.0;
                (void)hipStreamSynchronize(st);
                const double t1 = g_debug_cancel ? now_ms() : 0.0;
                if (n_ws == 2) (void)hipStreamSynchronize(ctx->ws[1].stream);
                if (g_debug_cancel) {
                    unsigned words[4] = {0, 0, 0, 0};
                    (void)hipMemcpy(words, error_block(ctx), sizeof words, hipMemcpyDeviceToHost);
                    std::fprintf(stderr, "[yk cancel] drain: stream0 %.3f ms, stream1 %.3f ms, batch %llu of %llu, device word %u\n", t1 - t0, now_ms() - t1,
                                 (unsigned long long)(w0 / batch), (unsigned long long)((work + batch - 1) / batch), words[YK_CTRL_CANCELLED]);
                }
                return fail(ctx, YK_ERR_CANCELLED, "cancelled by early_termination_predicate");
            }
            hipStream_t bs = n_ws == 2 ? ws.stream : st;
            unsigned* ctrl = ws.ctrl.as<unsigned>();
            const uint32_t n = (uint32_t)std::min<uint64_t>(batch, work - w0);
            HIP_TRY(ctx, hipMemsetAsync(ctrl, 0, YK_CTRL_WORDS * 4, bs));
            const bool lean = is_path && prm.max_depth > 0 && packet_kernel_traces_bounce(ctx, scene, 0);
            launch_raygen(bs, cam, prm, pixel_xy, pixel_sample, w0, n, path_buffers(ws, 0), sample_buf, ctrl + YK_CTRL_BOUNCE(0),
                          lean ? reinterpret_cast<float4*>(ctrl + YK_CTRL_CAM_O) : nullptr, ctx->pixel_aux.as<uint4>());
            ++n_batches;
            if (is_path) {
                run_bounces(ctx, ws, bs, scene, prm, pixel_xy, pixel_sample, sample_buf, kt, counters, true, n, (uint32_t)w0, lean, &n_shadow);
                n_trace += prm.max_depth;
            } else if (prm.integrator == YK_INTEGRATOR_WHITTED) {
                int e = kt.begin(bs);
                launch_whitted(bs, trace_grid(ctx), scene->dev, prm, pixel_xy, pixel_sample, path_buffers(ws, 0), n, sample_buf, ws.spill.as<uint2>(),
                               trace_grid(ctx) * trace_block_size(), errblk, counters);
                kt.end(e, 0, bs);
                ++n_trace;
            } else {
                PathBuffers pc = path_buffers(ws, 0);
                const bool want_stats = prm.integrator == YK_INTEGRATOR_BVH_INTERSECTIONS;
                int e = kt.begin(bs);
                launch_trace_closest(bs, trace_grid(ctx), dev_scene_for(scene, n), pc.rayO, pc.rayD, nullptr, ctrl + YK_CTRL_BOUNCE(0), ctrl + YK_CTRL_BOUNCE(0) + YK_CTRL_HEAD, ws.hit.as<int>(), nullptr,
                                     want_stats ? ctx->stats4.as<uint4>() : nullptr, ws.spill.as<uint2>(), trace_grid(ctx) * trace_block_size(), errblk,
                                     counters);
                kt.end(e, 0, bs);
                launch_debug_shade(bs, scene->dev, prm.integrator, pc, ws.hit.as<int>(), ctx->stats4.as<uint4>(), n, sample_buf);
                ++n_trace;
            }
            if (cancel) {
                HIP_TRY(ctx, hipEventRecord(ws.ev_batch, bs));
                ws_busy[which] = true;
            }
            if (n_ws == 2) which ^= 1;
        }
        if (n_ws == 2) {
            HIP_TRY(ctx, hipEventRecord(ctx->ws[1].done, ctx->ws[1].stream));
            HIP_TRY(ctx, hipStreamWaitEvent(st, ctx->ws[1].done, 0));
        }
        if (accumulating)
            launch_resolve_passes(st, sample_buf, npx, spp, out + 3 * (size_t)px0, 3 * (size_t)total_px);
        else
            launch_resolve(st, sample_buf, npx, spp, out + 3 * (size_t)px0);
        t_begin = t_end;
    }
    HIP_TRY(ctx, hipGetLastError());
#ifdef YK_EXPERIMENT_GRAPH
    YK_GRAPH_END
#endif
    if (stats) {
        HIP_TRY(ctx, hipEventRecord(ev1, st));
        if (wait_polling(ctx, ev1, st, cancel, user)) return fail(ctx, YK_ERR_CANCELLED, "cancelled by early_termination_predicate");
        if (ctx->cancel_raised.load(std::memory_order_acquire)) return fail(ctx, YK_ERR_CANCELLED, "interrupted (yk_context_interrupt)");
        HIP_TRY(ctx, hipGetLastError());
        std::memset(stats, 0, sizeof(*stats));
        unsigned long long host_counters[YK_COUNTER_BYTES / 8];
        HIP_TRY(ctx, hipMemcpy(host_counters, counters, YK_COUNTER_BYTES, hipMemcpyDeviceToHost));
        unsigned host_err[4];
        std::memcpy(host_err, host_counters + 16, sizeof(host_err));
        float ms = 0.0f;
        (void)hipEventElapsedTime(&ms, ev0, ev1);
        stats->rays = host_counters[0];
        stats->shadow_rays = host_counters[1];
        stats->samples = total_px * spp;
        stats->seconds_total = ms * 1e-3;
        stats->seconds_trace = kt.total(0);
        stats->seconds_shadow = kt.total(1);
        stats->seconds_shade = kt.total(2);
        stats->trace_launches = n_trace;
        stats->shadow_launches = n_shadow;
        stats->batches = n_batches;
        if (host_err[YK_CTRL_ERR] & 1u) return fail(ctx, YK_ERR_STACK_OVERFLOW, "BVH traversal stack exceeded 64 entries (bvh.rs:174)");
    } else if (scene->bvh->depth > 64) {
        unsigned host_err[4];
        HIP_TRY(ctx, hipMemcpyAsync(host_err, errblk, sizeof(host_err), hipMemcpyDeviceToHost, st));
        HIP_TRY(ctx, hipStreamSynchronize(st));
        if (host_err[YK_CTRL_ERR] & 1u) return fail(ctx, YK_ERR_STACK_OVERFLOW, "BVH traversal stack exceeded 64 entries (bvh.rs:174)");
    }
    return YK_OK;
} YK_CATCH(ctx)

static yk_status render_tiles_host(yk_context* ctx, const yk_scene* scene, const yk_camera* camera, const yk_sampler_desc* sampler,
                                   const yk_integrator_desc* integrator, const yk_tile* tiles, const uint16_t* tile_samples, size_t n_tiles,
                                   float* out_rgb, yk_render_stats* stats, yk_cancel_fn cancel, void* user, uint32_t n_passes = 1);

extern "C" {

yk_status yk_render_tiles_device(yk_context* ctx, const yk_scene* scene, const yk_camera* camera, const yk_sampler_desc* sampler,
                                 const yk_integrator_desc* integrator, const yk_tile* tiles, size_t n_tiles, void* d_out_rgb, void* stream,
                                 yk_render_stats* stats, yk_cancel_fn cancel, void* user) {
    return render_tiles_impl(ctx, scene, camera, sampler, integrator, tiles, nullptr, n_tiles, d_out_rgb, stream, stats, cancel, user);
}

yk_status yk_render_tiles_accumulating_device(yk_context* ctx, const yk_scene* scene, const yk_camera* camera, const yk_sampler_desc* sampler,
                                              const yk_integrator_desc* integrator, const yk_tile* tiles, const uint16_t* tile_samples, size_t n_tiles,
                                              void* d_out_rgb, void* stream, yk_render_stats* stats, yk_cancel_fn cancel, void* user) {
    if (!ctx) return YK_ERR_INVALID_ARGUMENT;
    YK_LOCK(ctx);
// ... 187 lines not shown
    yk_status st = yk_render_tiles(ctx, scene, camera, sampler, integrator, tile, 1, tile_pixels, &stats, nullptr, nullptr);
    if (st == YK_OK && out_rays) *out_rays = stats.rays;
    return st;
}

}

static yk_status film_tiles_device(yk_context* ctx, const yk_tile* tiles, size_t n_tiles, const void* d_tile_rgb, uint16_t res_x, uint16_t res_y,
                                   void* d_film_rgb, void* stream, int accumulate);

extern "C" {

yk_status yk_film_update_tiles_device(yk_context* ctx, const yk_tile* tiles, size_t n_tiles, const void* d_tile_rgb, uint16_t res_x, uint16_t res_y,
                                      void* d_film_rgb, void* stream) {
    return film_tiles_device(ctx, tiles, n_tiles, d_tile_rgb, res_x, res_y, d_film_rgb, stream, 0);
}

yk_status yk_film_accumulate_tiles_device(yk_context* ctx, const yk_tile* tiles, size_t n_tiles, const void* d_tile_rgb, uint16_t res_x, uint16_t res_y,
                                          void* d_film_rgb, void* stream) {
    return film_tiles_device(ctx, tiles, n_tiles, d_tile_rgb, res_x, res_y, d_film_rgb, stream, 1);
}

}

static yk_status film_tiles_device(yk_context* ctx, const yk_tile* tiles, size_t n_tiles, const void* d_tile_rgb, uint16_t res_x, uint16_t res_y,
                                   void* d_film_rgb, void* stream, int accumulate) try {
    if (!ctx) return YK_ERR_INVALID_ARGUMENT;
    YK_LOCK(ctx);
    if (!tiles || !d_tile_rgb || !d_film_rgb || n_tiles == 0) return fail(ctx, YK_ERR_INVALID_ARGUMENT, "null argument");
    (void)hipSetDevice(ctx->device);
    hipStream_t st = stream ? (hipStream_t)stream : ctx->stream;
    std::vector<uint32_t> off(n_tiles + 1, 0);
    uint64_t total = 0;
    for (size_t t = 0; t < n_tiles; ++t) {
        if (tiles[t].x1 > res_x || tiles[t].y1 > res_y || tiles[t].x0 >= tiles[t].x1 || tiles[t].y0 >= tiles[t].y1)
            return fail(ctx, YK_ERR_INVALID_ARGUMENT, "update_tile: Tile doesn't fit film");
        total += (uint64_t)(tiles[t].x1 - tiles[t].x0) * (uint64_t)(tiles[t].y1 - tiles[t].y0);
        if (total > 0xFFFFFFFFull) return fail(ctx, YK_ERR_INVALID_ARGUMENT, "too many pixels");
        off[t + 1] = (uint32_t)total;
    }
    HIP_TRY(ctx, ctx->scratch[1].ensure(n_tiles * sizeof(yk_tile)));
    HIP_TRY(ctx, ctx->scratch[2].ensure((n_tiles + 1) * 4));
    HIP_TRY(ctx, ctx->scratch[3].ensure(total * 4));
    HIP_TRY(ctx, hipMemcpyAsync(ctx->scratch[1].p, tiles, n_tiles * sizeof(yk_tile), hipMemcpyHostToDevice, st));
    HIP_TRY(ctx, hipMemcpyAsync(ctx->scratch[2].p, off.data(), off.size() * 4, hipMemcpyHostToDevice, st));
    HIP_TRY(ctx, hipStreamSynchronize(st));
    launch_pixel_table(st, ctx->scratch[1].as<yk_tile>(), ctx->scratch[2].as<uint32_t>(), (uint32_t)n_tiles, (uint32_t)total, ctx->scratch[3].as<uint32_t>());
    launch_film_scatter(st, ctx->scratch[3].as<uint32_t>(), (uint32_t)total, reinterpret_cast<const float*>(d_tile_rgb), res_x,
                        reinterpret_cast<float*>(d_film_rgb), accumulate);
    HIP_TRY(ctx, hipGetLastError());
    HIP_TRY(ctx, hipStreamSynchronize(st));
    return YK_OK;
} YK_CATCH(ctx)

extern "C" {

yk_status yk_li(yk_context* ctx, const yk_scene* scene, const yk_sampler_desc* sampler, const yk_integrator_desc* integrator, size_t n,
                const float* ray_o, const float* ray_d, const uint16_t* pixel_xy, const uint32_t* sample_index, uint32_t dimension, float* out_li,
                uint32_t* out_ray_counts) try {
    if (!ctx) return YK_ERR_INVALID_ARGUMENT;
    YK_LOCK(ctx);
    if (!scene || !ray_o || !ray_d || !pixel_xy || !sample_index || !out_li || n == 0) return fail(ctx, YK_ERR_INVALID_ARGUMENT, "null argument");
    if (!scene->on_device || scene->device != ctx->device) return fail(ctx, YK_ERR_INVALID_ARGUMENT, "scene was not created on this context's device");
    if (n > ((size_t)1 << 28)) return fail(ctx, YK_ERR_INVALID_ARGUMENT, "too many rays");
    RenderParams prm;
    yk_status ps = make_params(ctx, sampler, integrator, prm);
    if (ps != YK_OK) return ps;
    if (prm.integrator != YK_INTEGRATOR_PATH && prm.integrator != YK_INTEGRATOR_WHITTED)
        return fail(ctx, YK_ERR_UNSUPPORTED, "yk_li implements the Path and Whitted integrators");
    prm.spe = 1;
    for (size_t i = 0; i < n; ++i)
        if (sample_index[i] >= prm.sampler.spp) return fail(ctx, YK_ERR_INVALID_ARGUMENT, "sample_index >= samples per pixel");
    if (prm.max_depth > YK_CTRL_MAX_DEPTH) return fail(ctx, YK_ERR_INVALID_ARGUMENT, "max_depth too large");
    (void)hipSetDevice(ctx->device);
    hipStream_t st = ctx->stream;
    yk_status wb = ensure_work_buffers(ctx, ctx->ws[0], n, scene->n_lights, scene->n_delta_lights);
    if (wb != YK_OK) return wb;
    if ((wb = ensure_spill(ctx, ctx->ws[0])) != YK_OK) return wb;
    HIP_TRY(ctx, ctx->scratch[4].ensure(n * 12));
    HIP_TRY(ctx, ctx->scratch[5].ensure(n * 12));
    HIP_TRY(ctx, ctx->scratch[6].ensure(n * 4));
    HIP_TRY(ctx, ctx->scratch[7].ensure(n * 4));
    HIP_TRY(ctx, ctx->pixel_xy.ensure(n * 4));
    HIP_TRY(ctx, ctx->sample_buf.ensure(n * 16));
    HIP_TRY(ctx, hipMemcpyAsync(ctx->scratch[4].p, ray_o, n * 12, hipMemcpyHostToDevice, st));
    HIP_TRY(ctx, hipMemcpyAsync(ctx->scratch[5].p, ray_d, n * 12, hipMemcpyHostToDevice, st));
    HIP_TRY(ctx, hipMemcpyAsync(ctx->scratch[6].p, pixel_xy, n * 4, hipMemcpyHostToDevice, st));
    HIP_TRY(ctx, hipMemcpyAsync(ctx->scratch[7].p, sample_index, n * 4, hipMemcpyHostToDevice, st));
    unsigned* ctrl = ctx->ws[0].ctrl.as<unsigned>();
    unsigned long long* counters = ctx->counters.as<unsigned long long>();
    HIP_TRY(ctx, hipMemsetAsync(counters, 0, YK_COUNTER_BYTES, st));
    HIP_TRY(ctx, hipMemsetAsync(ctrl, 0, YK_CTRL_WORDS * 4, st));
    launch_raygen_user(st, prm, ctx->scratch[4].as<float>(), ctx->scratch[5].as<float>(), ctx->scratch[6].as<uint16_t>(), ctx->scratch[7].as<uint32_t>(),
                       dimension, (uint32_t)n, path_buffers(ctx->ws[0], 0), ctx->sample_buf.as<float4>(), ctx->pixel_xy.as<uint32_t>(), ctrl + YK_CTRL_BOUNCE(0));
    KernelTimer kt;
    kt.ctx = ctx;
    kt.on = false;
    if (prm.integrator == YK_INTEGRATOR_WHITTED)
        launch_whitted(st, trace_grid(ctx), scene->dev, prm, ctx->pixel_xy.as<uint32_t>(), ctx->scratch[7].as<uint32_t>(), path_buffers(ctx->ws[0], 0), (uint32_t)n,
                       ctx->sample_buf.as<float4>(), ctx->ws[0].spill.as<uint2>(), trace_grid(ctx) * trace_block_size(), error_block(ctx), counters);
    else
        run_bounces(ctx, ctx->ws[0], st, scene, prm, ctx->pixel_xy.as<uint32_t>(), ctx->scratch[7].as<uint32_t>(), ctx->sample_buf.as<float4>(), kt, counters, false, (uint32_t)n, 0u, false);
    HIP_TRY(ctx, hipGetLastError());
    std::vector<float> tmp(n * 4);
    unsigned host_err[4];
    HIP_TRY(ctx, hipMemcpyAsync(tmp.data(), ctx->sample_buf.p, n * 16, hipMemcpyDeviceToHost, st));
    HIP_TRY(ctx, hipMemcpyAsync(host_err, error_block(ctx), sizeof(host_err), hipMemcpyDeviceToHost, st));
    HIP_TRY(ctx, hipStreamSynchronize(st));
    if (host_err[YK_CTRL_ERR] & 1u) return fail(ctx, YK_ERR_STACK_OVERFLOW, "BVH traversal stack exceeded 64 entries (bvh.rs:174)");
    for (size_t i = 0; i < n; ++i) {
        out_li[3 * i] = tmp[4 * i];
        out_li[3 * i + 1] = tmp[4 * i + 1];
        out_li[3 * i + 2] = tmp[4 * i + 2];
    }
    if (out_ray_counts) std::memset(out_ray_counts, 0, n * 4);
    return YK_OK;
} YK_CATCH(ctx)

yk_status yk_li_debug(yk_context* ctx, const yk_scene* scene, const yk_sampler_desc* sampler, const yk_integrator_desc* integrator, size_t n,
                      const float* ray_o, const float* ray_d, const uint16_t* pixel_xy, const uint32_t* sample_index, uint32_t dimension, uint32_t ray_cap,
                      float* out_li, uint32_t* out_ray_counts, yk_integrator_ray* out_rays, uint32_t* out_n_rays) try {
    if (!ctx) return YK_ERR_INVALID_ARGUMENT;
    YK_LOCK(ctx);
    if (!scene || !ray_o || !ray_d || !pixel_xy || !sample_index || !out_li || !out_n_rays || (ray_cap && !out_rays) || n == 0)
        return fail(ctx, YK_ERR_INVALID_ARGUMENT, "null argument");
    if (!scene->on_device || scene->device != ctx->device) return fail(ctx, YK_ERR_INVALID_ARGUMENT, "scene was not created on this context's device");
    if (n > ((size_t)1 << 28)) return fail(ctx, YK_ERR_INVALID_ARGUMENT, "too many rays");
    if ((uint64_t)n * ray_cap > YK_LI_DEBUG_MAX_RECORDS) return fail(ctx, YK_ERR_INVALID_ARGUMENT, "n * ray_cap exceeds YK_LI_DEBUG_MAX_RECORDS");
    RenderParams prm;
    yk_status ps = make_params(ctx, sampler, integrator, prm);
    if (ps != YK_OK) return ps;
    if (prm.integrator != YK_INTEGRATOR_PATH) return fail(ctx, YK_ERR_UNSUPPORTED, "yk_li_debug implements the Path integrator (the others keep the trait's default)");
    prm.spe = 1;
    for (size_t i = 0; i < n; ++i)
        if (sample_index[i] >= prm.sampler.spp) return fail(ctx, YK_ERR_INVALID_ARGUMENT, "sample_index >= samples per pixel");
    (void)hipSetDevice(ctx->device);
    yk_status cs = clear_cancel(ctx);
    if (cs != YK_OK) return cs;
    hipStream_t st = ctx->stream;
    yk_status wb = ensure_work_buffers(ctx, ctx->ws[0], n, scene->n_lights, scene->n_delta_lights);
    if (wb != YK_OK) return wb;
    if ((wb = ensure_spill(ctx, ctx->ws[0])) != YK_OK) return wb;
    const size_t rec_bytes = (size_t)n * ray_cap * sizeof(yk_integrator_ray);
    HIP_TRY(ctx, ctx->scratch[0].ensure(std::max<size_t>(rec_bytes, 32)));
    HIP_TRY(ctx, ctx->scratch[1].ensure(n * 4));
    HIP_TRY(ctx, ctx->scratch[2].ensure(n * 4));
    HIP_TRY(ctx, ctx->scratch[4].ensure(n * 12));
    HIP_TRY(ctx, ctx->scratch[5].ensure(n * 12));
    HIP_TRY(ctx, ctx->scratch[6].ensure(n * 4));
    HIP_TRY(ctx, ctx->scratch[7].ensure(n * 4));
    HIP_TRY(ctx, ctx->pixel_xy.ensure(n * 4));
    HIP_TRY(ctx, ctx->sample_buf.ensure(n * 16));
    HIP_TRY(ctx, hipMemcpyAsync(ctx->scratch[4].p, ray_o, n * 12, hipMemcpyHostToDevice, st));
    HIP_TRY(ctx, hipMemcpyAsync(ctx->scratch[5].p, ray_d, n * 12, hipMemcpyHostToDevice, st));
    HIP_TRY(ctx, hipMemcpyAsync(ctx->scratch[6].p, pixel_xy, n * 4, hipMemcpyHostToDevice, st));
    HIP_TRY(ctx, hipMemcpyAsync(ctx->scratch[7].p, sample_index, n * 4, hipMemcpyHostToDevice, st));
    unsigned* ctrl = ctx->ws[0].ctrl.as<unsigned>();
    HIP_TRY(ctx, hipMemsetAsync(ctx->counters.p, 0, YK_COUNTER_BYTES, st));
    HIP_TRY(ctx, hipMemsetAsync(ctrl, 0, YK_CTRL_WORDS * 4, st));
    if (rec_bytes) HIP_TRY(ctx, hipMemsetAsync(ctx->scratch[0].p, 0, rec_bytes, st));
    prm.cancel = cancel_ref(ctx);
    launch_raygen_user(st, prm, ctx->scratch[4].as<float>(), ctx->scratch[5].as<float>(), ctx->scratch[6].as<uint16_t>(), ctx->scratch[7].as<uint32_t>(),
                       dimension, (uint32_t)n, path_buffers(ctx->ws[0], 0), ctx->sample_buf.as<float4>(), ctx->pixel_xy.as<uint32_t>(), ctrl + YK_CTRL_BOUNCE(0));
    const float* lo = scene->dev.root_bmin;
    const float* hi = scene->dev.root_bmax;
    const float dx = hi[0] - lo[0], dy = hi[1] - lo[1], dz = hi[2] - lo[2];
    const int axis = (dx > dy && dx > dz) ? 0 : (dy > dz ? 1 : 2);
    const float min_len = (hi[axis] - lo[axis]) / 10.0f;
    launch_path_debug(st, trace_grid(ctx), scene->dev, prm, ctx->pixel_xy.as<uint32_t>(), ctx->scratch[7].as<uint32_t>(), path_buffers(ctx->ws[0], 0), (uint32_t)n,
                      ctx->sample_buf.as<float4>(), ctx->scratch[1].as<uint32_t>(), ctx->scratch[0].as<float4>(), ray_cap, ctx->scratch[2].as<uint32_t>(), min_len,
                      ctx->ws[0].spill.as<uint2>(), trace_grid(ctx) * trace_block_size(), error_block(ctx));
    HIP_TRY(ctx, hipGetLastError());
    std::vector<float> tmp(n * 4);
    std::vector<uint32_t> counts(n), n_rays(n);
    unsigned host_err[4];
    HIP_TRY(ctx, hipMemcpyAsync(tmp.data(), ctx->sample_buf.p, n * 16, hipMemcpyDeviceToHost, st));
    HIP_TRY(ctx, hipMemcpyAsync(counts.data(), ctx->scratch[1].p, n * 4, hipMemcpyDeviceToHost, st));
    HIP_TRY(ctx, hipMemcpyAsync(n_rays.data(), ctx->scratch[2].p, n * 4, hipMemcpyDeviceToHost, st));
    HIP_TRY(ctx, hipMemcpyAsync(host_err, error_block(ctx), sizeof(host_err), hipMemcpyDeviceToHost, st));
    HIP_TRY(ctx, hipStreamSynchronize(st));
    if (ctx->cancel_raised.load(std::memory_order_acquire) || host_err[YK_CTRL_CANCELLED])
        return fail(ctx, YK_ERR_CANCELLED, "interrupted (yk_context_interrupt)");
    if (host_err[YK_CTRL_ERR] & 1u) return fail(ctx, YK_ERR_STACK_OVERFLOW, "BVH traversal stack exceeded 64 entries (bvh.rs:174)");
    if (rec_bytes) HIP_TRY(ctx, hipMemcpy(out_rays, ctx->scratch[0].p, rec_bytes, hipMemcpyDeviceToHost));
    for (size_t i = 0; i < n; ++i) {
        out_li[3 * i] = tmp[4 * i];
        out_li[3 * i + 1] = tmp[4 * i + 1];
        out_li[3 * i + 2] = tmp[4 * i + 2];
    }
    if (out_ray_counts) std::memcpy(out_ray_counts, counts.data(), n * 4);
    std::memcpy(out_n_rays, n_rays.data(), n * 4);
    return YK_OK;
} YK_CATCH(ctx)

}
```

yuki_amd/csrc/yk_shade.h:

```cpp
#pragma once
#include "yk_device.h"
#include "yk_geom.h"
#include "yk_rng.h"

namespace yk {

struct PathVertex {
    Surface sf;
    Material mat;
    Frame fr;
    V3 wo;
};

__device__ __forceinline__ SamplerState path_sampler(const RenderParams& prm, const uint32_t* pixel_xy, const uint32_t* sample_index_tab, uint4 rng,
                                                     uint32_t dimension, uint32_t sid) {
    SamplerState st;
    st.rng.state = (u64)rng.x | ((u64)rng.y << 32);
    st.rng.inc = (u64)rng.z | ((u64)rng.w << 32);
    st.dimension = dimension;
    uint32_t pix, ks;
    split_sample_id(sid, prm.spe, pix, ks);
    const uint32_t xy = pixel_xy[pix];
    st.px = xy & 0xffffu;
    st.py = xy >> 16;
    st.sample_index = (sample_index_tab ? sample_index_tab[pix] : prm.sample_base) + ks;
    return st;
}

__device__ __forceinline__ void vertex_setup_material(const DevScene& sc, V3 d, PathVertex& v) {
    v.mat = sc.materials[v.sf.material];
    if (v.mat.tex) {
        RGB kd = texture_eval(sc, v.mat.tex - 1u, v.sf.u, v.sf.v);
        v.mat.a[0] = kd.r;
        v.mat.a[1] = kd.g;
        v.mat.a[2] = kd.b;
        if (is_black(kd)) v.mat.kind = MK_BLACK;
    }
    v.fr = make_frame(v.sf.n, v.sf.ns, v.sf.dpdus);
    v.wo = -d;
}
__device__ __forceinline__ void vertex_setup(const DevScene& sc, uint32_t prim, V3 o, V3 d, PathVertex& v) {
    v.sf = hit_surface_prim(sc, prim, o, d);
    vertex_setup_material(sc, d, v);
}

struct NeeSample {
    bool want;
    bool has_ray;
    RGB contrib;
    V3 so, sd;
    int al;
};
__device__ __forceinline__ void vertex_shadow_ray(const PathVertex& v, const LightSample& ls, V3& so, V3& sd) {
    V3 offset = v.sf.n * 0.001f;
    so = dot(ls.p1 - v.sf.p, v.sf.n) > 0.0f ? v.sf.p + offset : v.sf.p - offset;
    sd = ls.p1 - so;
}
template <bool RAY_ALWAYS = false>
__device__ __forceinline__ NeeSample vertex_light(const DevScene& sc, const RenderParams& prm, SamplerState& st, unsigned l, const PathVertex& v) {
    NeeSample r;
    r.want = false;
    r.has_ray = false;
    r.contrib = RGB{0, 0, 0};
    r.so = V3{0, 0, 0};
    r.sd = V3{0, 0, 1};
    r.al = -1;
    float ux, uy;
    sampler_get_2d(prm.sampler, st, ux, uy);
    LightSample ls = sample_light(sc.lights[l], (int)l, v.sf.p, ux, uy);
    if (!is_black(ls.li)) {
        RGB f = bsdf_f(v.mat, v.fr, v.sf.wo, ls.l);
        if (ls.has_vis && !is_black(f)) {
            r.contrib = f * ls.li * rclamp(dot_nv(v.sf.ns, ls.l), 0.0f, 1.0f) / ls.pdf;
            vertex_shadow_ray(v, ls, r.so, r.sd);
            r.al = ls.area_light;
            r.want = true;
        } else if (RAY_ALWAYS && ls.has_vis) {
            vertex_shadow_ray(v, ls, r.so, r.sd);
            r.has_ray = true;
        }
    }
    return r;
}

#define YK_PEND_MISS 1u
#define YK_PEND_EMISSION 2u
#define YK_PEND_CLAMP 4u
#define YK_PEND_KIND_SHIFT 29
#define YK_PEND_SID_MASK 0x1fffffffu

__device__ __forceinline__ RGB vertex_miss_term(const DevScene& sc, RGB beta) { return beta * RGB{sc.background[0], sc.background[1], sc.background[2]}; }

struct VertexEnd {
    RGB term;
    unsigned kind;
    bool alive, sampled;
    V3 no, wi;
    unsigned lobe;
};
__device__ __forceinline__ VertexEnd vertex_finish(const DevScene& sc, const RenderParams& prm, SamplerState& st, const PathVertex& v, RGB& beta, unsigned& bounces,
                                                    bool& specular_bounce) {
    VertexEnd e;
    e.term = RGB{0, 0, 0};
    e.kind = 0;
    e.alive = false;
// ... 47 lines not shown
```

yuki_amd/csrc/yk_trace.hip:

```cpp
#include <hip/hip_runtime.h>

#include "yk_device.h"
#include "yk_geom.h"
#include "yk_kernels.h"
#include "yk_shade.h"
#include "yk_traverse.h"
#include "yk_wave.h"

#ifndef TRACE_BLOCK
#define TRACE_BLOCK 256
#endif
#ifndef TRACE_LDS
#define TRACE_LDS 8
#endif
#ifndef TRACE_TOP
#define TRACE_TOP 95
#endif
#ifndef TRACE_ANY_TOP
#define TRACE_ANY_TOP 224
#endif
#ifndef TRACE_ANY_LDS
#define TRACE_ANY_LDS TRACE_LDS
#endif
#ifndef TRACE_MIN_WAVES
// ... 300 lines not shown
                prefetch(idx);
                pf_valid = true;
            }
        }
        if (!__any(active)) {
            if (work.exhausted && !__any(pf_valid)) break;
            continue;
        }
        const bool on_leaf = active && (cur & YK_LEAF_BIT);
        const bool on_node = active && !(cur & YK_LEAF_BIT);
        const unsigned n_leaf = (unsigned)__popcll(__ballot(on_leaf));
        if (__any(on_node) && n_leaf < (unsigned)LEAF_MIN) {
            if (on_node) active = node_step();
        } else if (on_leaf) {
            active = leaf_step();
        }
    }
}

template <int BLOCK, int LDS_DEPTH, int PF_MIN, int START_MIN, int LEAF_MIN, int CHUNK, bool SPHERES, bool API, bool WIDE>
__global__ __launch_bounds__(BLOCK, TRACE_MIN_WAVES) void k_trace_closest_pt(DevScene sc, const float4* __restrict__ rayO, const float4* __restrict__ rayD,
                                                            const float* __restrict__ t_max_opt, const unsigned* count_ptr, unsigned* head,
                                                            int* __restrict__ hit_tri, float4* __restrict__ hit_out, uint2* spill,
                                                            unsigned spill_stride, unsigned* ctrl, unsigned long long* ray_counter, const unsigned* cancel_host) {
    __shared__ unsigned long long lds_stack[LDS_DEPTH * BLOCK];
    __shared__ float4 lds_top[WIDE ? 1 : TRACE_TOP * 4];
    if (!WIDE) fill_top<BLOCK>(lds_top, sc.top_nodes, sc.n_top);
    auto stk = make_stack<BLOCK, LDS_DEPTH>(lds_stack, spill, spill_stride);
    const CancelRef cancel = CancelRef{cancel_host, cancel_host ? ctrl + YK_CTRL_CANCELLED : nullptr};
    const unsigned n = queue_length(count_ptr, cancel, ray_counter);
    const unsigned root = WIDE ? 0u : (sc.n_top ? YK_TOP_BIT : sc.root_ref);
    unsigned* err = ctrl + YK_CTRL_ERR;

    float4 pf_o = make_float4(0, 0, 0, 0), pf_d = make_float4(0, 0, 1, 0);
    float pf_t = 0.0f;
    unsigned pf_idx = 0, ray_i = 0, cur = 0;
    TraceRay r = idle_ray();
    int sp = 0, best = -1;
    TriHit best_hit = TriHit{0, 0, 0, 0};
    const auto retire = [&]() {
        hit_tri[ray_i] = best;
        if (API && hit_out) hit_out[ray_i] = make_float4(best_hit.t, best_hit.b0, best_hit.b1, best_hit.b2);
        return false;
    };
    persistent_rays<PF_MIN, START_MIN, LEAF_MIN, CHUNK>(
        n, head, cancel, cur,
        [&](unsigned idx) {
            pf_o = rayO[idx];
            pf_d = rayD[idx];
            pf_t = (API && t_max_opt) ? t_max_opt[idx] : __builtin_inff();
            pf_idx = idx;
        },
        [&]() {
            r = ray_setup(f4_xyz(pf_o), f4_xyz(pf_d), API ? pf_t : __builtin_inff());
            ray_i = pf_idx;
            if (!root_hit(sc, r)) {
                hit_tri[ray_i] = -1;
                return false;
            }
            cur = root;
            sp = 0;
            best = -1;
            return true;
        },
        [&]() {
            if (WIDE) {
                if (node4_step<true>(sc.nodes4, r, stk, sp, cur, err)) return true;
            } else {
                const NodeBoxes nb = load_node(lds_top, sc.nodes, cur);
                YK_EXPERIMENT_NODE(sc.nodes + cur, nb);
                if (node2_closest<false>(nb, r, stk, sp, cur, err, nullptr) != STEP_POP) return true;
            }
            return pop_closest<false>(stk, sp, r.t_max, cur, nullptr) || retire();
        },
        [&]() {
            leaf_closest<SPHERES, false, false>(sc, cur & ~YK_LEAF_BIT, true, r, nullptr, [&](unsigned prim, float4 v1, unsigned pflags, const TriHit& h) {
                if (API) best_hit = h;
                best = API ? (int)__float_as_uint(v1.w) : YK_HIT_WORD(prim, pflags);
            });
            return pop_closest<false>(stk, sp, r.t_max, cur, nullptr) || retire();
        });
}

template <int BLOCK, int LDS_DEPTH, int PF_MIN, int START_MIN, int LEAF_MIN, int CHUNK, bool SPHERES, bool WIDE>
__global__ __launch_bounds__(BLOCK, TRACE_MIN_WAVES) void k_trace_any_pt(DevScene sc, const float4* __restrict__ shO, const float4* __restrict__ shD,
                                                        const unsigned* __restrict__ slot_of, const unsigned* count_ptr, unsigned* head,
                                                        unsigned char* __restrict__ vis, uint2* spill, unsigned spill_stride, unsigned* ctrl,
                                                        unsigned long long* shadow_counter, const unsigned* cancel_host) {
    __shared__ unsigned lds_stack[LDS_DEPTH * BLOCK];
    __shared__ float4 lds_top[WIDE ? 1 : TRACE_ANY_TOP * 4];
    if (!WIDE) fill_top<BLOCK>(lds_top, sc.top_nodes_any, sc.n_top_any);
    auto stk = make_stack<BLOCK, LDS_DEPTH>(lds_stack, spill, spill_stride);
    const CancelRef cancel = CancelRef{cancel_host, cancel_host ? ctrl + YK_CTRL_CANCELLED : nullptr};
    const unsigned n = queue_length(count_ptr, cancel, shadow_counter);
    const unsigned root = WIDE ? 0u : (sc.n_top_any ? YK_TOP_BIT : sc.root_ref);
    unsigned* err = ctrl + YK_CTRL_ERR;

    float4 pf_o = make_float4(0, 0, 0, 0), pf_d = make_float4(0, 0, 1, 0);
    unsigned pf_slot = 0, slot = 0, cur = 0;
    TraceRay r = idle_ray();
    int sp = 0, area_light = -1;
    const auto unoccluded = [&]() {
        if (!slot_of) vis[slot] = 0;
        return false;
    };
    persistent_rays<PF_MIN, START_MIN, LEAF_MIN, CHUNK>(
        n, head, cancel, cur,
        [&](unsigned k) {
            pf_o = shO[k];
            pf_d = shD[k];
            pf_slot = slot_of ? slot_of[k] : k;
        },
        [&]() {
            r = ray_setup(f4_xyz(pf_o), f4_xyz(pf_d), pf_o.w);
            area_light = (int)__float_as_uint(pf_d.w);
            slot = pf_slot;
            if (!root_hit(sc, r)) return unoccluded();
            cur = root;
            sp = 0;
            return true;
        },
        [&]() {
            const bool entered = WIDE ? node4_step<false>(sc.nodes4, r, stk, sp, cur, err)
                                      : node2_any(load_node(lds_top, sc.nodes, cur), r, stk, sp, cur, err) != STEP_POP;
            if (entered) return true;
            return pop_any(stk, sp, cur) || unoccluded();
        },
        [&]() {
            if (leaf_any<SPHERES>(sc, cur & ~YK_LEAF_BIT, r, area_light)) {
                vis[slot] = slot_of ? 2 : 1;
                return false;
            }
            return pop_any(stk, sp, cur) || unoccluded();
        });
}

template <int BLOCK, int LDS_DEPTH, bool STATS>
__global__ __launch_bounds__(BLOCK) void k_trace_closest(DevScene sc, const float4* rayO, const float4* rayD, const float* t_max_opt,
                                                         const unsigned* count_ptr, unsigned* head, int* hit_tri, float4* hit_out,
                                                         uint4* stats_out, uint2* spill, unsigned spill_stride, unsigned* ctrl,
                                                         unsigned long long* ray_counter) {
    __shared__ unsigned long long lds_stack[LDS_DEPTH * BLOCK];
    auto stk = make_stack<BLOCK, LDS_DEPTH>(lds_stack, spill, spill_stride);
    const unsigned n = queue_length(count_ptr, CancelRef{nullptr, nullptr}, ray_counter);
    for (;;) {
        unsigned base = 0;
        if (lane_id() == 0) base = atomicAdd(head, YK_WAVE);
        base = __shfl(base, 0);
        if (base >= n) break;
        unsigned i = base + lane_id();
        if (i < n) {
            float4 ro = rayO[i], rd = rayD[i];
            float tm = t_max_opt ? t_max_opt[i] : __builtin_inff();
            int tri;
            TriHit h = TriHit{0.0f, 0.0f, 0.0f, 0.0f};
            TraceStats s = TraceStats{0, 0, 0};
            traverse_closest<STATS>(sc, ray_setup(f4_xyz(ro), f4_xyz(rd), tm), stk, tri, h, &s, ctrl + YK_CTRL_ERR);
            hit_tri[i] = tri;
            if (hit_out) hit_out[i] = make_float4(h.t, h.b0, h.b1, h.b2);
            if (STATS) stats_out[i] = make_uint4(s.node_tests, s.node_hits, s.shape_tests, 0u);
        }
    }
}


#define YK_WHITTED_MAX_DEPTH 16
struct WhittedFrame {
    RGB sum;
    RGB pend_f;
    float pend_cos;
    bool t_valid;
    V3 t_o, t_d;
    RGB t_f;
    float t_cos;
};

template <int BLOCK, int LDS_DEPTH>
__global__ __launch_bounds__(BLOCK) void k_whitted(DevScene sc, RenderParams prm, const uint32_t* pixel_xy, const uint32_t* sample_index_tab, PathBuffers cur,
                                                   uint32_t n, float4* sample_buf, uint2* spill, unsigned spill_stride, unsigned* ctrl,
                                                   unsigned long long* counters) {
    __shared__ unsigned long long lds_stack[LDS_DEPTH * BLOCK];
    auto stk = make_stack<BLOCK, LDS_DEPTH>(lds_stack, spill, spill_stride);
    unsigned* err = ctrl + YK_CTRL_ERR;
    unsigned long long n_rays = 0, n_shadow = 0;
    if (cancel_raised(prm.cancel)) n = 0;
    for (uint32_t i = blockIdx.x * BLOCK + threadIdx.x; i < n; i += gridDim.x * BLOCK) {
        const float4 a = cur.rayO[i], b = cur.rayD[i], c = cur.thru[i];
        V3 o = f4_xyz(a), d = f4_xyz(b);
        const unsigned sid = __float_as_uint(b.w);
        SamplerState st = path_sampler(prm, pixel_xy, sample_index_tab, cur.rngs[i], __float_as_uint(c.w), sid);
        WhittedFrame frames[YK_WHITTED_MAX_DEPTH];
        int sp = 0;
        bool is_specular = false;
        RGB ret = RGB{0.0f, 0.0f, 0.0f};
        for (;;) {
            n_rays += 1;
            int shape;
            TriHit th = TriHit{0.0f, 0.0f, 0.0f, 0.0f};
            traverse_closest<false>(sc, ray_setup(o, d, __builtin_inff()), stk, shape, th, nullptr, err);
            bool called = false;
            if (shape < 0) {
                ret = RGB{sc.background[0], sc.background[1], sc.background[2]};
            } else {
                Surface sf = hit_surface(sc, (uint32_t)shape, o, d);
                Material mat = sc.materials[sf.material];
                if (mat.tex) {
                    RGB kd = texture_eval(sc, mat.tex - 1u, sf.u, sf.v);
                    mat.a[0] = kd.r;
                    mat.a[1] = kd.g;
                    mat.a[2] = kd.b;
                    if (is_black(kd)) mat.kind = MK_BLACK;
                }
                const Frame fr = make_frame(sf.n, sf.ns, sf.dpdus);
                RGB sum = RGB{0.0f, 0.0f, 0.0f};
                for (unsigned l = 0; l < sc.n_lights; ++l) {
                    float ux, uy;
                    sampler_get_2d(prm.sampler, st, ux, uy);
                    LightSample ls = sample_light(sc.lights[l], (int)l, sf.p, ux, uy);
                    if (is_black(ls.li)) continue;
                    RGB f = bsdf_f(mat, fr, sf.wo, ls.l);
                    if (!ls.has_vis || is_black(f)) continue;
                    V3 offset = sf.n * 0.001f;
                    V3 so = dot(ls.p1 - sf.p, sf.n) > 0.0f ? sf.p + offset : sf.p - offset;
                    n_shadow += 1;
                    if (!traverse_any(sc, ray_setup(so, ls.p1 - so, 0.9999f), ls.area_light, stk, err))
                        sum = sum + f * ls.li * rclamp(dot_nv(sf.ns, ls.l), 0.0f, 1.0f) / ls.pdf;
                }
                if (sp == 0 || is_specular) {
                    if (sf.area_light >= 0) {
                        const DevLight& L = sc.lights[sf.area_light];
                        sum = sum + (dot_nv(sf.n, -d) > 0.0f ? RGB{L.i[0], L.i[1], L.i[2]} : RGB{0.0f, 0.0f, 0.0f});
                    } else {
                        sum = sum + RGB{0.0f, 0.0f, 0.0f};
                    }
                }
                ret = sum;
                if ((unsigned)sp + 1u < prm.max_depth && mat.kind == MK_GLASS) {
                    BsdfSample rs = bsdf_sample_specular(mat, fr, sf.wo, BX_REFLECTION);
                    BsdfSample ts = bsdf_sample_specular(mat, fr, sf.wo, BX_TRANSMISSION);
                    if (rs.type != BX_NONE || ts.type != BX_NONE) {
                        WhittedFrame& fm = frames[sp];
                        fm.sum = sum;
                        fm.t_valid = false;
                        const BsdfSample& first = rs.type != BX_NONE ? rs : ts;
                        if (rs.type != BX_NONE && ts.type != BX_NONE) {
                            fm.t_valid = true;
                            fm.t_o = spawn_origin(sf.p, sf.n, ts.wi);
                            fm.t_d = ts.wi;
                            fm.t_f = ts.f;
                            fm.t_cos = fabsf(dot_nv(ts.wi, sf.ns));
                        }
                        fm.pend_f = first.f;
                        fm.pend_cos = fabsf(dot_nv(first.wi, sf.ns));
                        o = spawn_origin(sf.p, sf.n, first.wi);
                        d = first.wi;
                        is_specular = true;
                        ++sp;
                        called = true;
                    }
                }
            }
            if (called) continue;
            bool again = false;
            while (sp > 0) {
                WhittedFrame& fm = frames[sp - 1];
                fm.sum = fm.sum + fm.pend_f * ret * fm.pend_cos;
                if (fm.t_valid) {
                    fm.t_valid = false;
                    fm.pend_f = fm.t_f;
                    fm.pend_cos = fm.t_cos;
                    o = fm.t_o;
                    d = fm.t_d;
                    is_specular = true;
                    again = true;
                    break;
                }
                ret = fm.sum;
                --sp;
            }
            if (!again) break;
        }
        sample_buf[sid] = make_float4(ret.r, ret.g, ret.b, 0.0f);
    }
    for (int off = 32; off > 0; off >>= 1) {
        n_rays += __shfl_down(n_rays, off);
        n_shadow += __shfl_down(n_shadow, off);
    }
    if (lane_id() == 0 && counters) {
        if (n_rays) atomicAdd(counters, n_rays);
        if (n_shadow) atomicAdd(counters + 1, n_shadow);
    }
}

__device__ __forceinline__ void debug_ray_store(float4* out, uint32_t i, unsigned ray_cap, unsigned k, V3 o, V3 d, float t_max, unsigned type) {
    if (k >= ray_cap) return;
    float4* r = out + 2 * ((size_t)i * ray_cap + k);
    r[0] = make_float4(o.x, o.y, o.z, d.x);
    r[1] = make_float4(d.y, d.z, t_max, __uint_as_float(type));
}
__device__ __forceinline__ float root_exit(const DevScene& sc, V3 o, V3 d, float miss_len) {
    const float ix = 1.0f / d.x, iy = 1.0f / d.y, iz = 1.0f / d.z;
    const float t0x = (sc.root_bmin[0] - o.x) * ix, t0y = (sc.root_bmin[1] - o.y) * iy, t0z = (sc.root_bmin[2] - o.z) * iz;
    const float t1x = (sc.root_bmax[0] - o.x) * ix, t1y = (sc.root_bmax[1] - o.y) * iy, t1z = (sc.root_bmax[2] - o.z) * iz;
    const float tmin = rmax(rmax(rmin(t0x, t1x), rmax(rmin(t0y, t1y), rmin(t0z, t1z))), 0.0f);
    const float tmax = rmin(rmin(rmax(t0x, t1x), rmin(rmax(t0y, t1y), rmax(t0z, t1z))), __builtin_inff());
    return tmin <= tmax ? tmax : miss_len;
}

template <int BLOCK, int LDS_DEPTH>
__global__ __launch_bounds__(BLOCK) void k_path_debug(DevScene sc, RenderParams prm, const uint32_t* pixel_xy, const uint32_t* sample_index_tab, PathBuffers cur,
                                                      uint32_t n, float4* sample_buf, uint32_t* out_counts, float4* out_rays, unsigned ray_cap,
                                                      uint32_t* out_n_rays, float min_len, uint2* spill, unsigned spill_stride, unsigned* ctrl) {
    __shared__ unsigned long long lds_stack[LDS_DEPTH * BLOCK];
    auto stk = make_stack<BLOCK, LDS_DEPTH>(lds_stack, spill, spill_stride);
    unsigned* err = ctrl + YK_CTRL_ERR;
    if (cancel_raised(prm.cancel)) n = 0;
    for (uint32_t i = blockIdx.x * BLOCK + threadIdx.x; i < n; i += gridDim.x * BLOCK) {
        const float4 a = cur.rayO[i], b = cur.rayD[i], c = cur.thru[i];
        V3 o = f4_xyz(a), d = f4_xyz(b);
        const unsigned sid = __float_as_uint(b.w);
        SamplerState st = path_sampler(prm, pixel_xy, sample_index_tab, cur.rngs[i], __float_as_uint(c.w), sid);
        RGB L = RGB{0.0f, 0.0f, 0.0f}, beta = RGB{c.x, c.y, c.z};
        unsigned bounces = 0, n_closest = 0, k = 0, type = YK_RAY_DIRECT;
        bool specular_bounce = false, alive = prm.max_depth > 0;
        while (alive) {
            n_closest += 1;
            int shape;
            TriHit th = TriHit{0.0f, 0.0f, 0.0f, 0.0f};
            traverse_closest<false>(sc, ray_setup(o, d, __builtin_inff()), stk, shape, th, nullptr, err);
            if (shape < 0) {
                debug_ray_store(out_rays, i, ray_cap, k++, o, d, type == YK_RAY_DIRECT ? __builtin_inff() : root_exit(sc, o, d, min_len), type);
                L = vertex_accumulate(prm, L, RGB{1.0f, 1.0f, 1.0f}, RGB{0.0f, 0.0f, 0.0f}, vertex_miss_term(sc, beta), YK_PEND_MISS);
                break;
            }
            debug_ray_store(out_rays, i, ray_cap, k++, o, d, th.t, type);
            PathVertex v;
            v.sf = hit_surface(sc, (uint32_t)shape, o, d);
            vertex_setup_material(sc, d, v);
            debug_ray_store(out_rays, i, ray_cap, k++, v.sf.p, v.sf.n, min_len, YK_RAY_NORMAL);
            RGB radiance = RGB{0.0f, 0.0f, 0.0f};
            for (unsigned l = 0; l < sc.n_lights; ++l) {
                const NeeSample ne = vertex_light<true>(sc, prm, st, l, v);
                if (ne.want || ne.has_ray) debug_ray_store(out_rays, i, ray_cap, k++, ne.so, ne.sd, 0.9999f, YK_RAY_SHADOW);
                if (ne.want && !traverse_any(sc, ray_setup(ne.so, ne.sd, 0.9999f), ne.al, stk, err)) radiance = radiance + ne.contrib;
            }
            const RGB beta_in = beta;
            const VertexEnd e = vertex_finish(sc, prm, st, v, beta, bounces, specular_bounce);
            L = vertex_accumulate(prm, L, beta_in, radiance, e.term, e.kind);
            alive = e.alive;
            o = e.no;
            d = e.wi;
            type = (e.lobe & BX_REFLECTION) ? YK_RAY_REFLECTION : YK_RAY_REFRACTION;
        }
        sample_buf[sid] = make_float4(L.r, L.g, L.b, 0.0f);
        out_counts[i] = n_closest;
        out_n_rays[i] = k;
    }
}

#ifndef TRACE_PF_MIN
#define TRACE_PF_MIN 16
#endif
#ifndef TRACE_START_MIN
#define TRACE_START_MIN 8
#endif
#ifndef TRACE_LEAF_MIN
#define TRACE_LEAF_MIN 16
#endif
#ifndef TRACE_CHUNK
#define TRACE_CHUNK 128
#endif

unsigned trace_block_size() { return TRACE_BLOCK; }
unsigned trace_spill_depth() { return YK_STACK_CAP - TRACE_LDS; }
unsigned trace_top_nodes() { return TRACE_TOP; }
unsigned trace_top_nodes_any() { return TRACE_ANY_TOP; }
static_assert(TRACE_ANY_LDS * TRACE_BLOCK * 4 + TRACE_ANY_TOP * 64 <= TRACE_LDS * TRACE_BLOCK * 8 + TRACE_TOP * 64 + 1024, "the any-hit kernel must fit the block count of the closest-hit kernel");
static_assert(TRACE_ANY_LDS >= TRACE_LDS, "the spill buffer is sized for TRACE_LDS entries in LDS");
unsigned trace_blocks_per_cu() {
    unsigned by_lds = (160u * 1024u) / (TRACE_LDS * TRACE_BLOCK * 8u + TRACE_TOP * 64u);
    unsigned by_waves = (unsigned)TRACE_MIN_WAVES * 256u / TRACE_BLOCK;
    return by_lds < by_waves ? by_lds : by_waves;
}

void launch_trace_closest(hipStream_t s, unsigned grid, const DevScene& sc, const float4* rayO, const float4* rayD, const float* t_max_opt,
                          const unsigned* count_ptr, unsigned* head, int* hit_tri, float4* hit_out, uint4* stats_out, uint2* spill,
                          unsigned spill_stride, unsigned* ctrl, unsigned long long* ray_counter, const unsigned* cancel_host) {
    if (stats_out)
        hipLaunchKernelGGL((k_trace_closest<TRACE_BLOCK, TRACE_LDS, true>), dim3(grid), dim3(TRACE_BLOCK), 0, s, sc, rayO, rayD, t_max_opt, count_ptr,
                           head, hit_tri, hit_out, stats_out, spill, spill_stride, ctrl, ray_counter);
    else {
        const bool api = t_max_opt != nullptr || hit_out != nullptr;
#define YK_LAUNCH_CLOSEST(SPH, API, WIDE)                                                                                                              \
    hipLaunchKernelGGL((k_trace_closest_pt<TRACE_BLOCK, TRACE_LDS, TRACE_PF_MIN, TRACE_START_MIN, TRACE_LEAF_MIN, TRACE_CHUNK, SPH, API, WIDE>), dim3(grid), \
                       dim3(TRACE_BLOCK), 0, s, sc, rayO, rayD, t_max_opt, count_ptr, head, hit_tri, hit_out, spill, spill_stride, ctrl, ray_counter, cancel_host)
#define YK_LAUNCH_CLOSEST_W(SPH, API) \
    if (sc.nodes4) YK_LAUNCH_CLOSEST(SPH, API, true); else YK_LAUNCH_CLOSEST(SPH, API, false)
        if (sc.spheres) {
            if (api) { YK_LAUNCH_CLOSEST_W(true, true); } else { YK_LAUNCH_CLOSEST_W(true, false); }
        } else {
            if (api) { YK_LAUNCH_CLOSEST_W(false, true); } else { YK_LAUNCH_CLOSEST_W(false, false); }
        }
#undef YK_LAUNCH_CLOSEST_W
#undef YK_LAUNCH_CLOSEST
    }
}
void launch_whitted(hipStream_t s, unsigned grid, const DevScene& sc, const RenderParams& prm, const uint32_t* pixel_xy, const uint32_t* sample_index_tab,
                    PathBuffers cur, uint32_t n, float4* sample_buf, uint2* spill, unsigned spill_stride, unsigned* ctrl, unsigned long long* counters) {
    hipLaunchKernelGGL((k_whitted<TRACE_BLOCK, TRACE_LDS>), dim3(grid), dim3(TRACE_BLOCK), 0, s, sc, prm, pixel_xy, sample_index_tab, cur, n, sample_buf, spill,
                       spill_stride, ctrl, counters);
}
unsigned whitted_max_depth() { return YK_WHITTED_MAX_DEPTH; }
void launch_path_debug(hipStream_t s, unsigned grid, const DevScene& sc, const RenderParams& prm, const uint32_t* pixel_xy, const uint32_t* sample_index_tab,
                       PathBuffers cur, uint32_t n, float4* sample_buf, uint32_t* out_counts, float4* out_rays, unsigned ray_cap, uint32_t* out_n_rays,
                       float min_len, uint2* spill, unsigned spill_stride, unsigned* ctrl) {
    hipLaunchKernelGGL((k_path_debug<TRACE_BLOCK, TRACE_LDS>), dim3(grid), dim3(TRACE_BLOCK), 0, s, sc, prm, pixel_xy, sample_index_tab, cur, n, sample_buf,
                       out_counts, out_rays, ray_cap, out_n_rays, min_len, spill, spill_stride, ctrl);
}
void launch_trace_any(hipStream_t s, unsigned grid, const DevScene& sc, const float4* shO, const float4* shD, const unsigned* slot_of,
                      const unsigned* count_ptr, unsigned* head, unsigned char* vis, uint2* spill, unsigned spill_stride, unsigned* ctrl,
                      unsigned long long* shadow_counter, const unsigned* cancel_host) {
#define YK_LAUNCH_ANY(SPH, WIDE)                                                                                                                       \
    hipLaunchKernelGGL((k_trace_any_pt<TRACE_BLOCK, TRACE_ANY_LDS, TRACE_PF_MIN, TRACE_START_MIN, TRACE_LEAF_MIN, TRACE_CHUNK, SPH, WIDE>), dim3(grid),     \
                       dim3(TRACE_BLOCK), 0, s, sc, shO, shD, slot_of, count_ptr, head, vis, spill, spill_stride, ctrl, shadow_counter, cancel_host)
    if (sc.spheres) {
        if (sc.nodes4) YK_LAUNCH_ANY(true, true); else YK_LAUNCH_ANY(true, false);
    } else {
        if (sc.nodes4) YK_LAUNCH_ANY(false, true); else YK_LAUNCH_ANY(false, false);
    }
#undef YK_LAUNCH_ANY
}

}
```

Measured before the change: 2293 Mray/s.

## Slim path state: 64-bit RNG, packed shadow slot, miss accumulation in shade

Path RNG state drops from uint4 to uint2; the increment is presumably rebuilt from the new pixel_aux table. The separate shadow slot queues (shq/shq2) are removed and the slot is packed into the w component of the shadow origin, with dedicated render variants of the any-hit kernels that decode it. Paths that miss now accumulate into sample_buf directly in the shade kernel and mark their vis word as settled, so accumulate skips them. The aim is less memory traffic per path and per shadow ray. In exchange, miss accumulation moves into shade, which adds sample_buf reads and writes there, and this relies on shade and accumulate never touching the same sample in one bounce.

```diff
diff --git a/yuki_amd/csrc/yk_context.cpp b/yuki_amd/csrc/yk_context.cpp
--- a/yuki_amd/csrc/yk_context.cpp
+++ b/yuki_amd/csrc/yk_context.cpp
@@ -87,7 +87,7 @@
     for (WorkSet& w : ctx->ws) {
         for (int a = 0; a < 2; ++a)
             for (int b = 0; b < 4; ++b) w.path[a][b].release();
-        DevBuf* wb[] = {&w.hit, &w.pend, &w.shO, &w.shD, &w.shC, &w.vis, &w.shq, &w.shO2, &w.shD2, &w.shq2, &w.ctrl, &w.spill, &w.spill_side};
+        DevBuf* wb[] = {&w.hit, &w.pend, &w.shO, &w.shD, &w.shC, &w.vis, &w.shO2, &w.shD2, &w.ctrl, &w.spill, &w.spill_side};
         for (DevBuf* b : wb) b->release();
         if (w.done) (void)hipEventDestroy(w.done);
         if (w.ev_shade) (void)hipEventDestroy(w.ev_shade);
diff --git a/yuki_amd/csrc/yk_device.h b/yuki_amd/csrc/yk_device.h
--- a/yuki_amd/csrc/yk_device.h
+++ b/yuki_amd/csrc/yk_device.h
@@ -15,6 +15,7 @@
 static_assert(sizeof(DevNode) == 64, "DevNode must be 64 bytes");
 
 #define YK_VIS_STRIDE(nl) ((nl) <= 4u ? 4u : (nl))
+#define YK_VIS_SETTLED 3u
 #define YK_LEAF_BIT 0x80000000u
 #define YK_REF_NONE 0xffffffffu
 #define YK_AXIS_SHIFT 28
@@ -99,7 +100,7 @@
     float4* rayO;
     float4* rayD;
     float4* thru;
-    uint4* rngs;
+    uint2* rngs;
 };
 
 #define YK_CTRL_WORDS 1024
diff --git a/yuki_amd/csrc/yk_internal.h b/yuki_amd/csrc/yk_internal.h
--- a/yuki_amd/csrc/yk_internal.h
+++ b/yuki_amd/csrc/yk_internal.h
@@ -57,7 +57,7 @@
     int64_t streams = 2;
     struct WorkSet {
         DevBuf path[2][4];
-        DevBuf hit, pend, shO, shD, shC, vis, shq, shO2, shD2, shq2, ctrl, spill, spill_side;
+        DevBuf hit, pend, shO, shD, shC, vis, shO2, shD2, ctrl, spill, spill_side;
         size_t cap_paths = 0;
         unsigned cap_lights = 0, cap_area = 0, cap_delta = 0;
         hipStream_t stream = nullptr;
@@ -214,6 +214,6 @@
 };
 
 bool packet_kernel_traces_bounce(const yk_context* ctx, const yk_scene* scene, unsigned b);
-void run_bounces(yk_context* ctx, WorkSet& ws, hipStream_t st, const yk_scene* scene, const RenderParams& prm, const uint32_t* pixel_xy,
+void run_bounces(yk_context* ctx, WorkSet& ws, hipStream_t st, const yk_scene* scene, const RenderParams& prm, const uint32_t* pixel_xy, const uint4* pixel_aux,
                  const uint32_t* sample_index_tab, float4* sample_buf, KernelTimer& kt, unsigned long long* counters, bool coherent,
                  uint32_t n_paths, uint32_t sid_base, bool lean_camera_bounce, uint32_t* n_shadow_launches = nullptr);
diff --git a/yuki_amd/csrc/yk_kernels.h b/yuki_amd/csrc/yk_kernels.h
--- a/yuki_amd/csrc/yk_kernels.h
+++ b/yuki_amd/csrc/yk_kernels.h
@@ -14,6 +14,8 @@
                                  unsigned* head, int* hit_tri, unsigned long long* ray_counter, const float4* lean_origin = nullptr, CancelRef cancel = CancelRef{nullptr, nullptr});
 void launch_trace_any_packet(hipStream_t s, unsigned grid, const DevScene& sc, const float4* shO, const float4* shD, const unsigned* slot_of,
                              const unsigned* count_ptr, unsigned* head, unsigned char* vis, unsigned long long* shadow_counter, CancelRef cancel = CancelRef{nullptr, nullptr});
+void launch_trace_any_packet_render(hipStream_t s, unsigned grid, const DevScene& sc, const float4* shO, const float4* shD, const unsigned* count_ptr,
+                                    unsigned* head, unsigned char* vis, unsigned long long* shadow_counter, CancelRef cancel);
 unsigned trace_blocks_per_cu();
 
 void launch_pixel_table(hipStream_t s, const yk_tile* tiles, const uint32_t* tile_offset, uint32_t n_tiles, uint32_t n_pixels, uint32_t* pixel_xy,
@@ -27,18 +29,22 @@
 void launch_trace_closest(hipStream_t s, unsigned grid, const DevScene& sc, const float4* rayO, const float4* rayD, const float* t_max_opt,
                           const unsigned* count_ptr, unsigned* head, int* hit_tri, float4* hit_out, uint4* stats_out, uint2* spill,
                           unsigned spill_stride, unsigned* ctrl, unsigned long long* ray_counter, const unsigned* cancel_host = nullptr);
-void launch_whitted(hipStream_t s, unsigned grid, const DevScene& sc, const RenderParams& prm, const uint32_t* pixel_xy, const uint32_t* sample_index_tab,
+void launch_whitted(hipStream_t s, unsigned grid, const DevScene& sc, const RenderParams& prm, const uint32_t* pixel_xy, const uint4* pixel_aux, const uint32_t* sample_index_tab,
                     PathBuffers cur, uint32_t n, float4* sample_buf, uint2* spill, unsigned spill_stride, unsigned* ctrl, unsigned long long* counters);
 unsigned whitted_max_depth();
-void launch_path_debug(hipStream_t s, unsigned grid, const DevScene& sc, const RenderParams& prm, const uint32_t* pixel_xy, const uint32_t* sample_index_tab,
+void launch_path_debug(hipStream_t s, unsigned grid, const DevScene& sc, const RenderParams& prm, const uint32_t* pixel_xy, const uint4* pixel_aux, const uint32_t* sample_index_tab,
                        PathBuffers cur, uint32_t n, float4* sample_buf, uint32_t* out_counts, float4* out_rays, unsigned ray_cap, uint32_t* out_n_rays,
                        float min_len, uint2* spill, unsigned spill_stride, unsigned* ctrl);
 void launch_trace_any(hipStream_t s, unsigned grid, const DevScene& sc, const float4* shO, const float4* shD, const unsigned* slot_of,
                       const unsigned* count_ptr, unsigned* head, unsigned char* vis, uint2* spill, unsigned spill_stride, unsigned* ctrl,
                       unsigned long long* shadow_counter, const unsigned* cancel_host = nullptr);
-void launch_shade(hipStream_t s, unsigned grid, const DevScene& sc, const RenderParams& prm, const uint32_t* pixel_xy, const uint32_t* sample_index_tab,
+void launch_trace_any_render(hipStream_t s, unsigned grid, const DevScene& sc, const float4* shO, const float4* shD, const unsigned* count_ptr,
+                             unsigned* head, unsigned char* vis, uint2* spill, unsigned spill_stride, unsigned* ctrl, unsigned long long* shadow_counter,
+                             const unsigned* cancel_host);
+void launch_shade(hipStream_t s, unsigned grid, const DevScene& sc, const RenderParams& prm, const uint32_t* pixel_xy, const uint4* pixel_aux, const uint32_t* sample_index_tab,
                   PathBuffers cur, PathBuffers nxt, const int* hit_tri, float4* pend, float4* shO, float4* shD, float4* shC, unsigned char* vis,
-                  unsigned* shq, float4* shO2, float4* shD2, unsigned* shq2, unsigned* bc, unsigned split_delta, unsigned reorder, unsigned block_slots, unsigned sid_base, const float4* lean_origin);
+                  float4* shO2, float4* shD2, unsigned* bc, unsigned split_delta, unsigned reorder, unsigned block_slots, unsigned sid_base, const float4* lean_origin,
+                  float4* sample_buf, unsigned first);
 void launch_accumulate(hipStream_t s, unsigned grid, const RenderParams& prm, PathBuffers cur, const float4* pend, const float4* shC,
                        const unsigned char* vis, unsigned nl, float4* sample_buf, const unsigned* bc, unsigned first, unsigned sid_base);
 void launch_resolve(hipStream_t s, const float4* sample_buf, uint32_t n_pixels, uint32_t spp, float* out_rgb);
diff --git a/yuki_amd/csrc/yk_kernels.hip b/yuki_amd/csrc/yk_kernels.hip
--- a/yuki_amd/csrc/yk_kernels.hip
+++ b/yuki_amd/csrc/yk_kernels.hip
@@ -85,7 +85,7 @@
         out.thru[i] = make_float4(1.0f, 1.0f, 1.0f, __uint_as_float(st.dimension));
     }
     out.rayD[i] = make_float4(d.x, d.y, d.z, __uint_as_float((uint32_t)w));
-    out.rngs[i] = make_uint4((unsigned)st.rng.state, (unsigned)(st.rng.state >> 32), (unsigned)st.rng.inc, (unsigned)(st.rng.inc >> 32));
+    out.rngs[i] = make_uint2((unsigned)st.rng.state, (unsigned)(st.rng.state >> 32));
     if (prm.integrator != YK_INTEGRATOR_PATH || prm.max_depth == 0) sample_buf[w] = make_float4(0.0f, 0.0f, 0.0f, 0.0f);
 }
 
@@ -101,7 +101,7 @@
     out.rayO[i] = make_float4(ray_o[3 * i], ray_o[3 * i + 1], ray_o[3 * i + 2], __uint_as_float(0u));
     out.rayD[i] = make_float4(ray_d[3 * i], ray_d[3 * i + 1], ray_d[3 * i + 2], __uint_as_float(i));
     out.thru[i] = make_float4(1.0f, 1.0f, 1.0f, __uint_as_float(st.dimension));
-    out.rngs[i] = make_uint4((unsigned)st.rng.state, (unsigned)(st.rng.state >> 32), (unsigned)st.rng.inc, (unsigned)(st.rng.inc >> 32));
+    out.rngs[i] = make_uint2((unsigned)st.rng.state, (unsigned)(st.rng.state >> 32));
     if (prm.integrator != YK_INTEGRATOR_PATH || prm.max_depth == 0) sample_buf[i] = make_float4(0.0f, 0.0f, 0.0f, 0.0f);
 }
 
@@ -119,9 +119,8 @@
 #endif
 template <int CAP, int CAPQ> struct ShadeStaging {
     float4 pO[CAP], pD[CAP], pT[CAP];
-    uint4 pR[CAP];
+    uint2 pR[CAP];
     float4 qO[CAPQ], qD[CAPQ];
-    unsigned qS[CAPQ];
     unsigned fill_p, fill_q, gbase;
     unsigned q_delta;
     unsigned cancel;
@@ -150,11 +149,12 @@
 #endif
 
 template <int BLOCK, int CAP, int CAPQ>
-__global__ __launch_bounds__(BLOCK, SHADE_MIN_WAVES) void k_shade(DevScene sc, RenderParams prm, const uint32_t* pixel_xy, const uint32_t* sample_index_tab,
+__global__ __launch_bounds__(BLOCK, SHADE_MIN_WAVES) void k_shade(DevScene sc, RenderParams prm, const uint32_t* pixel_xy, const uint4* pixel_aux, const uint32_t* sample_index_tab,
                                                  PathBuffers cur, PathBuffers nxt,
                                                  const int* hit_tri, float4* pend, float4* shO, float4* shD, float4* shC, unsigned char* vis,
-                                                 unsigned* shq, float4* shO2, float4* shD2, unsigned* shq2, unsigned* bc, unsigned split_delta, unsigned reorder,
-                                                 unsigned win_max, unsigned block_slots, unsigned sid_base, const float4* __restrict__ lean_origin) {
+                                                 float4* shO2, float4* shD2, unsigned* bc, unsigned split_delta, unsigned reorder,
+                                                 unsigned win_max, unsigned block_slots, unsigned sid_base, const float4* __restrict__ lean_origin,
+                                                 float4* sample_buf, unsigned first) {
     const unsigned win_iters = min(win_max, max(1u, bc[0] / (BLOCK * block_slots)));
     static_assert(sizeof(ShadeStaging<CAP, CAPQ>) <= 53296, "k_shade: more LDS than the measured 53296 bytes per block (42 granules = 53760 cost the third block per CU)");
     __shared__ ShadeStaging<CAP, CAPQ> stg;
@@ -175,11 +175,9 @@
         const unsigned gb = stg.gbase;
         float4* dO = delta ? shO2 : shO;
         float4* dD = delta ? shD2 : shD;
-        unsigned* dS = delta ? shq2 : shq;
         for (unsigned k = threadIdx.x; k < fill; k += BLOCK) {
             dO[gb + k] = stg.qO[k];
             dD[gb + k] = stg.qD[k];
-            dS[gb + k] = stg.qS[k];
         }
         __syncthreads();
         if (threadIdx.x == 0) stg.fill_q = 0;
@@ -262,7 +260,7 @@
             if (fp + BLOCK > CAP) flush_p(fp);
         }
         float4 nO = make_float4(0, 0, 0, 0), nD = nO, nT = nO;
-        uint4 nR = make_uint4(0, 0, 0, 0);
+        uint2 nR = make_uint2(0, 0);
         V3 o = V3{0, 0, 0}, d = V3{0, 0, 1};
         RGB beta = RGB{0, 0, 0};
         unsigned flags = 0, sid = 0, bounces = 0;
@@ -289,7 +287,7 @@
                 a = cur.rayO[i];
                 c = cur.thru[i];
             }
-            uint4 r = cur.rngs[i];
+            uint2 r = cur.rngs[i];
             o = f4_xyz(a);
             d = f4_xyz(b);
             flags = __float_as_uint(a.w);
@@ -297,7 +295,7 @@
             beta = RGB{c.x, c.y, c.z};
             bounces = flags & 0xffu;
             specular_bounce = (flags >> 8) & 1u;
-            st = path_sampler(prm, pixel_xy, sample_index_tab, r, __float_as_uint(c.w), sid);
+            st = path_sampler(prm, pixel_xy, pixel_aux, sample_index_tab, r, __float_as_uint(c.w), sid);
             int tri = hit_tri[i];
             hit = tri >= 0;
             if (hit) vertex_setup(sc, (uint32_t)tri & YK_HIT_PRIM_MASK, o, d, v);
@@ -329,33 +327,39 @@
             }
             unsigned q = block_append(want, &stg.fill_q);
             if (want) {
-                stg.qO[q] = make_float4(ne.so.x, ne.so.y, ne.so.z, 0.9999f);
+                stg.qO[q] = make_float4(ne.so.x, ne.so.y, ne.so.z, __uint_as_float(vslot));
                 stg.qD[q] = make_float4(ne.sd.x, ne.sd.y, ne.sd.z, __uint_as_float((unsigned)ne.al));
-                stg.qS[q] = vslot;
                 shC[slot] = make_float4(ne.contrib.r, ne.contrib.g, ne.contrib.b, 0.0f);
             }
+        }
+        if (valid && !hit) {
+            if (vs == 4u)
+                vword = YK_VIS_SETTLED;
+            else
+                vis[i * vs] = YK_VIS_SETTLED;
         }
         if (vs == 4u && valid) reinterpret_cast<unsigned*>(vis)[i] = vword;
         YK_PROF_STAMP(3)
         if (valid) {
-            unsigned kind = 0;
-            RGB term = RGB{0, 0, 0};
             if (!hit) {
-                term = vertex_miss_term(sc, beta);
-                kind = YK_PEND_MISS;
+                RGB L = RGB{0.0f, 0.0f, 0.0f};
+                if (!first) {
+                    const float4 acc = sample_buf[sid];
+                    L = RGB{acc.x, acc.y, acc.z};
+                }
+                L = vertex_accumulate(prm, L, RGB{1.0f, 1.0f, 1.0f}, RGB{0.0f, 0.0f, 0.0f}, vertex_miss_term(sc, beta), YK_PEND_MISS);
+                sample_buf[sid] = make_float4(L.r, L.g, L.b, 0.0f);
             } else {
                 VertexEnd e = vertex_finish(sc, prm, st, v, beta, bounces, specular_bounce);
-                term = e.term;
-                kind = e.kind;
                 alive = e.alive;
                 if (e.sampled) {
                     nO = make_float4(e.no.x, e.no.y, e.no.z, __uint_as_float((bounces & 0xffu) | (specular_bounce ? 0x100u : 0u)));
                     nD = make_float4(e.wi.x, e.wi.y, e.wi.z, __uint_as_float(sid));
                     nT = make_float4(beta.r, beta.g, beta.b, __uint_as_float(st.dimension));
-                    nR = make_uint4((unsigned)st.rng.state, (unsigned)(st.rng.state >> 32), (unsigned)st.rng.inc, (unsigned)(st.rng.inc >> 32));
+                    nR = make_uint2((unsigned)st.rng.state, (unsigned)(st.rng.state >> 32));
                 }
+                pend[i] = make_float4(e.term.r, e.term.g, e.term.b, __uint_as_float((e.kind << YK_PEND_KIND_SHIFT) | (sid - sid_base)));
             }
-            pend[i] = make_float4(term.r, term.g, term.b, __uint_as_float((kind << YK_PEND_KIND_SHIFT) | (sid - sid_base)));
         }
         YK_PROF_STAMP(4)
         if (!per_iter) {
@@ -387,12 +391,15 @@
 __global__ void k_accumulate(RenderParams prm, PathBuffers cur, const float4* pend, const float4* shC, const unsigned char* vis, unsigned nl,
                              float4* sample_buf, const unsigned* bc, unsigned first, unsigned sid_base) {
     const unsigned n = cancel_raised(prm.cancel) ? 0u : bc[0];
+    const unsigned vs = YK_VIS_STRIDE(nl);
     for (unsigned i = blockIdx.x * blockDim.x + threadIdx.x; i < n; i += gridDim.x * blockDim.x) {
+        const unsigned vword = vs == 4u ? reinterpret_cast<const unsigned*>(vis)[i] : (unsigned)vis[i * vs];
+        if ((vword & 255u) == YK_VIS_SETTLED) continue;
         float4 p = pend[i];
         const unsigned kind = __float_as_uint(p.w) >> YK_PEND_KIND_SHIFT;
         const unsigned sid = sid_base + (__float_as_uint(p.w) & YK_PEND_SID_MASK);
         RGB beta = RGB{1.0f, 1.0f, 1.0f};
-        if (!first && !(kind & YK_PEND_MISS)) {
+        if (!first) {
             const float4 c = cur.thru[i];
             beta = RGB{c.x, c.y, c.z};
         }
@@ -402,16 +409,12 @@
             L = RGB{acc.x, acc.y, acc.z};
         }
         RGB radiance = RGB{0.0f, 0.0f, 0.0f};
-        if (!(kind & YK_PEND_MISS)) {
-            const unsigned vs = YK_VIS_STRIDE(nl);
-            const unsigned vword = vs == 4u ? reinterpret_cast<const unsigned*>(vis)[i] : 0u;
-            for (unsigned l = 0; l < nl; ++l) {
-                const unsigned slot = i * nl + l;
-                const unsigned verdict = vs == 4u ? (vword >> (8u * l)) & 255u : (unsigned)vis[i * vs + l];
-                if (verdict == 1u) {
-                    float4 ct = shC[slot];
-                    radiance = radiance + RGB{ct.x, ct.y, ct.z};
-                }
+        for (unsigned l = 0; l < nl; ++l) {
+            const unsigned slot = i * nl + l;
+            const unsigned verdict = vs == 4u ? (vword >> (8u * l)) & 255u : (unsigned)vis[i * vs + l];
+            if (verdict == 1u) {
+                float4 ct = shC[slot];
+                radiance = radiance + RGB{ct.x, ct.y, ct.z};
             }
         }
         L = vertex_accumulate(prm, L, beta, radiance, RGB{p.x, p.y, p.z}, kind);
@@ -677,12 +680,13 @@
     hipLaunchKernelGGL(k_raygen_user, dim3(blocks_for(n, 256)), dim3(256), 0, s, prm, o, d, pixel, sample_index, dimension, n, out, sample_buf,
                        pixel_xy, ctrl);
 }
-void launch_shade(hipStream_t s, unsigned grid, const DevScene& sc, const RenderParams& prm, const uint32_t* pixel_xy, const uint32_t* sample_index_tab,
+void launch_shade(hipStream_t s, unsigned grid, const DevScene& sc, const RenderParams& prm, const uint32_t* pixel_xy, const uint4* pixel_aux, const uint32_t* sample_index_tab,
                   PathBuffers cur, PathBuffers nxt,
-                  const int* hit_tri, float4* pend, float4* shO, float4* shD, float4* shC, unsigned char* vis, unsigned* shq, float4* shO2,
-                  float4* shD2, unsigned* shq2, unsigned* bc, unsigned split_delta, unsigned reorder, unsigned block_slots, unsigned sid_base, const float4* lean_origin) {
-    hipLaunchKernelGGL((k_shade<256, SHADE_CAP, SHADE_CAPQ>), dim3(grid), dim3(256), 0, s, sc, prm, pixel_xy, sample_index_tab, cur, nxt, hit_tri, pend, shO, shD, shC, vis, shq,
-                       shO2, shD2, shq2, bc, split_delta, reorder, (unsigned)SHADE_WIN, block_slots, sid_base, lean_origin);
+                  const int* hit_tri, float4* pend, float4* shO, float4* shD, float4* shC, unsigned char* vis, float4* shO2,
+                  float4* shD2, unsigned* bc, unsigned split_delta, unsigned reorder, unsigned block_slots, unsigned sid_base, const float4* lean_origin,
+                  float4* sample_buf, unsigned first) {
+    hipLaunchKernelGGL((k_shade<256, SHADE_CAP, SHADE_CAPQ>), dim3(grid), dim3(256), 0, s, sc, prm, pixel_xy, pixel_aux, sample_index_tab, cur, nxt, hit_tri, pend, shO, shD, shC, vis,
+                       shO2, shD2, bc, split_delta, reorder, (unsigned)SHADE_WIN, block_slots, sid_base, lean_origin, sample_buf, first);
 }
 void launch_accumulate(hipStream_t s, unsigned grid, const RenderParams& prm, PathBuffers cur, const float4* pend, const float4* shC,
                        const unsigned char* vis, unsigned nl, float4* sample_buf, const unsigned* bc, unsigned first, unsigned sid_base) {
diff --git a/yuki_amd/csrc/yk_packet.hip b/yuki_amd/csrc/yk_packet.hip
--- a/yuki_amd/csrc/yk_packet.hip
+++ b/yuki_amd/csrc/yk_packet.hip
@@ -139,7 +139,7 @@
     });
 }
 
-template <bool SPHERES>
+template <bool SPHERES, bool RENDER>
 __global__ __launch_bounds__(YK_PKT_BLOCK, 8) void k_trace_any_packet(DevScene sc, const float4* __restrict__ shO, const float4* __restrict__ shD,
                                                                       const unsigned* __restrict__ slot_of, const unsigned* count_ptr, unsigned* head,
                                                                       unsigned char* __restrict__ vis, unsigned long long* shadow_counter, CancelRef cancel) {
@@ -151,9 +151,9 @@
         const unsigned k = base + lane_id();
         const bool valid = k < n;
         const float4 ro = valid ? shO[k] : make_float4(0, 0, 0, 0), rd = valid ? shD[k] : make_float4(0, 0, 1, 0);
-        const TraceRay r = ray_setup(f4_xyz(ro), f4_xyz(rd), ro.w);
+        const TraceRay r = ray_setup(f4_xyz(ro), f4_xyz(rd), RENDER ? 0.9999f : ro.w);
         const int area_light = (int)__float_as_uint(rd.w);
-        const unsigned slot = valid ? (slot_of ? slot_of[k] : k) : 0u;
+        const unsigned slot = valid ? (RENDER ? __float_as_uint(ro.w) : (slot_of ? slot_of[k] : k)) : 0u;
         const bool alive = valid && root_hit(sc, r);
         bool occluded = false;
         unsigned long long cmask = __ballot(alive);
@@ -223,8 +223,8 @@
         }
         if (valid) {
             if (occluded)
-                vis[slot] = slot_of ? 2 : 1;
-            else if (!slot_of)
+                vis[slot] = (RENDER || slot_of) ? 2 : 1;
+            else if (!RENDER && !slot_of)
                 vis[slot] = 0;
         }
     });
@@ -242,9 +242,17 @@
 void launch_trace_any_packet(hipStream_t s, unsigned grid, const DevScene& sc, const float4* shO, const float4* shD, const unsigned* slot_of,
                              const unsigned* count_ptr, unsigned* head, unsigned char* vis, unsigned long long* shadow_counter, CancelRef cancel) {
     if (sc.spheres)
-        hipLaunchKernelGGL((k_trace_any_packet<true>), dim3(grid), dim3(YK_PKT_BLOCK), 0, s, sc, shO, shD, slot_of, count_ptr, head, vis, shadow_counter, cancel);
+        hipLaunchKernelGGL((k_trace_any_packet<true, false>), dim3(grid), dim3(YK_PKT_BLOCK), 0, s, sc, shO, shD, slot_of, count_ptr, head, vis, shadow_counter, cancel);
     else
-        hipLaunchKernelGGL((k_trace_any_packet<false>), dim3(grid), dim3(YK_PKT_BLOCK), 0, s, sc, shO, shD, slot_of, count_ptr, head, vis, shadow_counter, cancel);
-}
-
-}
+        hipLaunchKernelGGL((k_trace_any_packet<false, false>), dim3(grid), dim3(YK_PKT_BLOCK), 0, s, sc, shO, shD, slot_of, count_ptr, head, vis, shadow_counter, cancel);
+}
+void launch_trace_any_packet_render(hipStream_t s, unsigned grid, const DevScene& sc, const float4* shO, const float4* shD, const unsigned* count_ptr,
+                                    unsigned* head, unsigned char* vis, unsigned long long* shadow_counter, CancelRef cancel) {
+    const unsigned* slot_of = nullptr;
+    if (sc.spheres)
+        hipLaunchKernelGGL((k_trace_any_packet<true, true>), dim3(grid), dim3(YK_PKT_BLOCK), 0, s, sc, shO, shD, slot_of, count_ptr, head, vis, shadow_counter, cancel);
+    else
+        hipLaunchKernelGGL((k_trace_any_packet<false, true>), dim3(grid), dim3(YK_PKT_BLOCK), 0, s, sc, shO, shD, slot_of, count_ptr, head, vis, shadow_counter, cancel);
+}
+
+}
diff --git a/yuki_amd/csrc/yk_render.cpp b/yuki_amd/csrc/yk_render.cpp
--- a/yuki_amd/csrc/yk_render.cpp
+++ b/yuki_amd/csrc/yk_render.cpp
@@ -31,17 +31,15 @@
     na = std::max(na, ws.cap_area);
     nd = std::max(nd, ws.cap_delta);
     for (int a = 0; a < 2; ++a)
-        for (int b = 0; b < 4; ++b) HIP_TRY(ctx, ws.path[a][b].ensure(paths * 16));
+        for (int b = 0; b < 4; ++b) HIP_TRY(ctx, ws.path[a][b].ensure(paths * (b == 3 ? 8 : 16)));
     HIP_TRY(ctx, ws.hit.ensure(paths * 4));
     HIP_TRY(ctx, ws.pend.ensure(paths * 16));
     HIP_TRY(ctx, ws.shC.ensure(paths * nl * 16));
     HIP_TRY(ctx, ws.vis.ensure(paths * YK_VIS_STRIDE(nl)));
     HIP_TRY(ctx, ws.shO.ensure(paths * na * 16));
     HIP_TRY(ctx, ws.shD.ensure(paths * na * 16));
-    HIP_TRY(ctx, ws.shq.ensure(paths * na * 4));
     HIP_TRY(ctx, ws.shO2.ensure(paths * nd * 16));
     HIP_TRY(ctx, ws.shD2.ensure(paths * nd * 16));
-    HIP_TRY(ctx, ws.shq2.ensure(paths * nd * 4));
     HIP_TRY(ctx, ws.ctrl.ensure(YK_CTRL_ALLOC_WORDS * 4));
     ws.cap_paths = paths;
     ws.cap_lights = nl;
@@ -64,7 +62,7 @@
     p.rayO = ws.path[which][0].as<float4>();
     p.rayD = ws.path[which][1].as<float4>();
     p.thru = ws.path[which][2].as<float4>();
-    p.rngs = ws.path[which][3].as<uint4>();
+    p.rngs = ws.path[which][3].as<uint2>();
     return p;
 }
 
@@ -96,7 +94,7 @@
     return b < (unsigned)ctx->packet_bounces && scene->bvh->depth <= 64;
 }
 
-void run_bounces(yk_context* ctx, WorkSet& ws, hipStream_t st, const yk_scene* scene, const RenderParams& prm, const uint32_t* pixel_xy,
+void run_bounces(yk_context* ctx, WorkSet& ws, hipStream_t st, const yk_scene* scene, const RenderParams& prm, const uint32_t* pixel_xy, const uint4* pixel_aux,
                         const uint32_t* sample_index_tab, float4* sample_buf, KernelTimer& kt, unsigned long long* counters, bool coherent,
                         uint32_t n_paths, uint32_t sid_base, bool lean_camera_bounce, uint32_t* n_shadow_launches) {
     unsigned* ctrl = ws.ctrl.as<unsigned>();
@@ -131,9 +129,9 @@
         kt.end(e, 0, st);
         if (overlap && b > 0) (void)hipStreamWaitEvent(st, ws.ev_acc, 0);
         e = kt.begin(st);
-        launch_shade(st, sg, ds, prm, pixel_xy, sample_index_tab, pc, pn, ws.hit.as<int>(), ws.pend.as<float4>(), ws.shO.as<float4>(),
-                     ws.shD.as<float4>(), ws.shC.as<float4>(), ws.vis.as<unsigned char>(), ws.shq.as<unsigned>(), ws.shO2.as<float4>(),
-                     ws.shD2.as<float4>(), ws.shq2.as<unsigned>(), bc, split ? 1u : 0u, (b > 0 && ctx->shade_reorder) ? 1u : 0u, 3u * (unsigned)ctx->n_cu, sid_base, lean_origin);
+        launch_shade(st, sg, ds, prm, pixel_xy, pixel_aux, sample_index_tab, pc, pn, ws.hit.as<int>(), ws.pend.as<float4>(), ws.shO.as<float4>(),
+                     ws.shD.as<float4>(), ws.shC.as<float4>(), ws.vis.as<unsigned char>(), ws.shO2.as<float4>(),
+                     ws.shD2.as<float4>(), bc, split ? 1u : 0u, (b > 0 && ctx->shade_reorder) ? 1u : 0u, 3u * (unsigned)ctx->n_cu, sid_base, lean_origin, sample_buf, b == 0 ? 1u : 0u);
         kt.end(e, 2, st);
 #ifdef YK_EXPERIMENT_SORT
         YK_SORT_AFTER_SHADE
@@ -145,15 +143,15 @@
         e = kt.begin(sb);
         uint2* any_spill = (overlap ? ws.spill_side : ws.spill).as<uint2>();
         if (all_delta) {
-            launch_trace_any_packet(sb, pg_any, ds, ws.shO.as<float4>(), ws.shD.as<float4>(), ws.shq.as<unsigned>(), bc + YK_CTRL_SHQ,
-                                    bc + YK_CTRL_HEAD + 1, ws.vis.as<unsigned char>(), counters + 1, prm.cancel);
+            launch_trace_any_packet_render(sb, pg_any, ds, ws.shO.as<float4>(), ws.shD.as<float4>(), bc + YK_CTRL_SHQ,
+                                           bc + YK_CTRL_HEAD + 1, ws.vis.as<unsigned char>(), counters + 1, prm.cancel);
         } else {
-            launch_trace_any(sb, tg_any, ds, ws.shO.as<float4>(), ws.shD.as<float4>(), ws.shq.as<unsigned>(), bc + YK_CTRL_SHQ,
-                             bc + YK_CTRL_HEAD + 1, ws.vis.as<unsigned char>(), any_spill, spill_stride, errblk, counters + 1, prm.cancel.host);
+            launch_trace_any_render(sb, tg_any, ds, ws.shO.as<float4>(), ws.shD.as<float4>(), bc + YK_CTRL_SHQ,
+                                    bc + YK_CTRL_HEAD + 1, ws.vis.as<unsigned char>(), any_spill, spill_stride, errblk, counters + 1, prm.cancel.host);
             if (split && n_shadow_launches) ++*n_shadow_launches;
             if (split)
-                launch_trace_any_packet(sb, pg_any, ds, ws.shO2.as<float4>(), ws.shD2.as<float4>(), ws.shq2.as<unsigned>(), bc + YK_CTRL_SHQ2,
-                                        bc + YK_CTRL_HEAD + 2, ws.vis.as<unsigned char>(), counters + 1, prm.cancel);
+                launch_trace_any_packet_render(sb, pg_any, ds, ws.shO2.as<float4>(), ws.shD2.as<float4>(), bc + YK_CTRL_SHQ2,
+                                               bc + YK_CTRL_HEAD + 2, ws.vis.as<unsigned char>(), counters + 1, prm.cancel);
         }
         kt.end(e, 1, sb);
         if (n_shadow_launches) ++*n_shadow_launches;
@@ -168,8 +166,11 @@
             (void)hipEventElapsedTime(&tt, ctx->ev_pool[kt.spans[0].back().first], ctx->ev_pool[kt.spans[0].back().second]);
             (void)hipEventElapsedTime(&ts, ctx->ev_pool[kt.spans[1].back().first], ctx->ev_pool[kt.spans[1].back().second]);
             (void)hipEventElapsedTime(&th, ctx->ev_pool[kt.spans[2].back().first], ctx->ev_pool[kt.spans[2].back().second]);
-            std::fprintf(stderr, "bounce %u: rays %u trace %.3f ms (%.0f Mray/s) | shadow rays %u %.3f ms (%.0f Mray/s) | shade %.3f ms | survivors %u\n", b, h[0],
-                         tt, h[0] / (tt * 1e3), h[YK_CTRL_SHQ] + h[YK_CTRL_SHQ2], ts, (h[YK_CTRL_SHQ] + h[YK_CTRL_SHQ2]) / (ts * 1e3), th, h[YK_CTRL_STRIDE]);
+            std::vector<int> hits(h[0]);
+            (void)hipMemcpy(hits.data(), ws.hit.p, (size_t)h[0] * 4, hipMemcpyDeviceToHost);
+            const size_t n_miss = (size_t)std::count_if(hits.begin(), hits.end(), [](int t) { return t < 0; });
+            std::fprintf(stderr, "bounce %u: rays %u trace %.3f ms (%.0f Mray/s) | shadow rays %u %.3f ms (%.0f Mray/s) | shade %.3f ms | survivors %u | misses %zu\n", b, h[0],
+                         tt, h[0] / (tt * 1e3), h[YK_CTRL_SHQ] + h[YK_CTRL_SHQ2], ts, (h[YK_CTRL_SHQ] + h[YK_CTRL_SHQ2]) / (ts * 1e3), th, h[YK_CTRL_STRIDE], n_miss);
         }
         cur ^= 1u;
     }
@@ -298,7 +299,7 @@
     {
         size_t free_b = 0, total_b = 0;
         if (batch > ctx->ws[0].cap_paths && hipMemGetInfo(&free_b, &total_b) == hipSuccess) {
-            const size_t per_path = (148 + 53 * (size_t)std::max(1u, scene->n_lights) + 36) * (size_t)n_ws;
+            const size_t per_path = (132 + 49 * (size_t)std::max(1u, scene->n_lights) + 32) * (size_t)n_ws;
             const size_t fit = (free_b / 2) / per_path;
             if (fit >= 65536 && batch > fit) batch = fit;
         }
@@ -421,11 +422,11 @@
                           lean ? reinterpret_cast<float4*>(ctrl + YK_CTRL_CAM_O) : nullptr, ctx->pixel_aux.as<uint4>());
             ++n_batches;
             if (is_path) {
-                run_bounces(ctx, ws, bs, scene, prm, pixel_xy, pixel_sample, sample_buf, kt, counters, true, n, (uint32_t)w0, lean, &n_shadow);
+                run_bounces(ctx, ws, bs, scene, prm, pixel_xy, ctx->pixel_aux.as<uint4>(), pixel_sample, sample_buf, kt, counters, true, n, (uint32_t)w0, lean, &n_shadow);
                 n_trace += prm.max_depth;
             } else if (prm.integrator == YK_INTEGRATOR_WHITTED) {
                 int e = kt.begin(bs);
-                launch_whitted(bs, trace_grid(ctx), scene->dev, prm, pixel_xy, pixel_sample, path_buffers(ws, 0), n, sample_buf, ws.spill.as<uint2>(),
+                launch_whitted(bs, trace_grid(ctx), scene->dev, prm, pixel_xy, ctx->pixel_aux.as<uint4>(), pixel_sample, path_buffers(ws, 0), n, sample_buf, ws.spill.as<uint2>(),
                                trace_grid(ctx) * trace_block_size(), errblk, counters);
                 kt.end(e, 0, bs);
                 ++n_trace;
@@ -779,6 +780,7 @@
     HIP_TRY(ctx, ctx->scratch[6].ensure(n * 4));
     HIP_TRY(ctx, ctx->scratch[7].ensure(n * 4));
     HIP_TRY(ctx, ctx->pixel_xy.ensure(n * 4));
+    HIP_TRY(ctx, ctx->pixel_aux.ensure(n * 16));
     HIP_TRY(ctx, ctx->sample_buf.ensure(n * 16));
     HIP_TRY(ctx, hipMemcpyAsync(ctx->scratch[4].p, ray_o, n * 12, hipMemcpyHostToDevice, st));
     HIP_TRY(ctx, hipMemcpyAsync(ctx->scratch[5].p, ray_d, n * 12, hipMemcpyHostToDevice, st));
@@ -790,14 +792,15 @@
     HIP_TRY(ctx, hipMemsetAsync(ctrl, 0, YK_CTRL_WORDS * 4, st));
     launch_raygen_user(st, prm, ctx->scratch[4].as<float>(), ctx->scratch[5].as<float>(), ctx->scratch[6].as<uint16_t>(), ctx->scratch[7].as<uint32_t>(),
                        dimension, (uint32_t)n, path_buffers(ctx->ws[0], 0), ctx->sample_buf.as<float4>(), ctx->pixel_xy.as<uint32_t>(), ctrl + YK_CTRL_BOUNCE(0));
+    launch_pixel_sampler(st, prm.sampler, ctx->pixel_xy.as<uint32_t>(), (uint32_t)n, ctx->pixel_aux.as<uint4>());
     KernelTimer kt;
     kt.ctx = ctx;
     kt.on = false;
     if (prm.integrator == YK_INTEGRATOR_WHITTED)
-        launch_whitted(st, trace_grid(ctx), scene->dev, prm, ctx->pixel_xy.as<uint32_t>(), ctx->scratch[7].as<uint32_t>(), path_buffers(ctx->ws[0], 0), (uint32_t)n,
+        launch_whitted(st, trace_grid(ctx), scene->dev, prm, ctx->pixel_xy.as<uint32_t>(), ctx->pixel_aux.as<uint4>(), ctx->scratch[7].as<uint32_t>(), path_buffers(ctx->ws[0], 0), (uint32_t)n,
                        ctx->sample_buf.as<float4>(), ctx->ws[0].spill.as<uint2>(), trace_grid(ctx) * trace_block_size(), error_block(ctx), counters);
     else
-        run_bounces(ctx, ctx->ws[0], st, scene, prm, ctx->pixel_xy.as<uint32_t>(), ctx->scratch[7].as<uint32_t>(), ctx->sample_buf.as<float4>(), kt, counters, false, (uint32_t)n, 0u, false);
+        run_bounces(ctx, ctx->ws[0], st, scene, prm, ctx->pixel_xy.as<uint32_t>(), ctx->pixel_aux.as<uint4>(), ctx->scratch[7].as<uint32_t>(), ctx->sample_buf.as<float4>(), kt, counters, false, (uint32_t)n, 0u, false);
     HIP_TRY(ctx, hipGetLastError());
     std::vector<float> tmp(n * 4);
     unsigned host_err[4];
@@ -847,6 +850,7 @@
     HIP_TRY(ctx, ctx->scratch[6].ensure(n * 4));
     HIP_TRY(ctx, ctx->scratch[7].ensure(n * 4));
     HIP_TRY(ctx, ctx->pixel_xy.ensure(n * 4));
+    HIP_TRY(ctx, ctx->pixel_aux.ensure(n * 16));
     HIP_TRY(ctx, ctx->sample_buf.ensure(n * 16));
     HIP_TRY(ctx, hipMemcpyAsync(ctx->scratch[4].p, ray_o, n * 12, hipMemcpyHostToDevice, st));
     HIP_TRY(ctx, hipMemcpyAsync(ctx->scratch[5].p, ray_d, n * 12, hipMemcpyHostToDevice, st));
@@ -859,12 +863,13 @@
     prm.cancel = cancel_ref(ctx);
     launch_raygen_user(st, prm, ctx->scratch[4].as<float>(), ctx->scratch[5].as<float>(), ctx->scratch[6].as<uint16_t>(), ctx->scratch[7].as<uint32_t>(),
                        dimension, (uint32_t)n, path_buffers(ctx->ws[0], 0), ctx->sample_buf.as<float4>(), ctx->pixel_xy.as<uint32_t>(), ctrl + YK_CTRL_BOUNCE(0));
+    launch_pixel_sampler(st, prm.sampler, ctx->pixel_xy.as<uint32_t>(), (uint32_t)n, ctx->pixel_aux.as<uint4>());
     const float* lo = scene->dev.root_bmin;
     const float* hi = scene->dev.root_bmax;
     const float dx = hi[0] - lo[0], dy = hi[1] - lo[1], dz = hi[2] - lo[2];
     const int axis = (dx > dy && dx > dz) ? 0 : (dy > dz ? 1 : 2);
     const float min_len = (hi[axis] - lo[axis]) / 10.0f;
-    launch_path_debug(st, trace_grid(ctx), scene->dev, prm, ctx->pixel_xy.as<uint32_t>(), ctx->scratch[7].as<uint32_t>(), path_buffers(ctx->ws[0], 0), (uint32_t)n,
+    launch_path_debug(st, trace_grid(ctx), scene->dev, prm, ctx->pixel_xy.as<uint32_t>(), ctx->pixel_aux.as<uint4>(), ctx->scratch[7].as<uint32_t>(), path_buffers(ctx->ws[0], 0), (uint32_t)n,
                       ctx->sample_buf.as<float4>(), ctx->scratch[1].as<uint32_t>(), ctx->scratch[0].as<float4>(), ray_cap, ctx->scratch[2].as<uint32_t>(), min_len,
                       ctx->ws[0].spill.as<uint2>(), trace_grid(ctx) * trace_block_size(), error_block(ctx));
     HIP_TRY(ctx, hipGetLastError());
diff --git a/yuki_amd/csrc/yk_shade.h b/yuki_amd/csrc/yk_shade.h
--- a/yuki_amd/csrc/yk_shade.h
+++ b/yuki_amd/csrc/yk_shade.h
@@ -12,15 +12,16 @@
     V3 wo;
 };
 
-__device__ __forceinline__ SamplerState path_sampler(const RenderParams& prm, const uint32_t* pixel_xy, const uint32_t* sample_index_tab, uint4 rng,
-                                                     uint32_t dimension, uint32_t sid) {
+__device__ __forceinline__ SamplerState path_sampler(const RenderParams& prm, const uint32_t* pixel_xy, const uint4* pixel_aux, const uint32_t* sample_index_tab,
+                                                     uint2 rng, uint32_t dimension, uint32_t sid) {
     SamplerState st;
     st.rng.state = (u64)rng.x | ((u64)rng.y << 32);
-    st.rng.inc = (u64)rng.z | ((u64)rng.w << 32);
     st.dimension = dimension;
     uint32_t pix, ks;
     split_sample_id(sid, prm.spe, pix, ks);
     const uint32_t xy = pixel_xy[pix];
+    const uint4 aux = pixel_aux[pix];
+    st.rng.inc = (((u64)aux.x | ((u64)aux.y << 32)) << 1) | 1;
     st.px = xy & 0xffffu;
     st.py = xy >> 16;
     st.sample_index = (sample_index_tab ? sample_index_tab[pix] : prm.sample_base) + ks;
diff --git a/yuki_amd/csrc/yk_trace.hip b/yuki_amd/csrc/yk_trace.hip
--- a/yuki_amd/csrc/yk_trace.hip
+++ b/yuki_amd/csrc/yk_trace.hip
@@ -406,7 +406,7 @@
         });
 }
 
-template <int BLOCK, int LDS_DEPTH, int PF_MIN, int START_MIN, int LEAF_MIN, int CHUNK, bool SPHERES, bool WIDE>
+template <int BLOCK, int LDS_DEPTH, int PF_MIN, int START_MIN, int LEAF_MIN, int CHUNK, bool SPHERES, bool WIDE, bool RENDER>
 __global__ __launch_bounds__(BLOCK, TRACE_MIN_WAVES) void k_trace_any_pt(DevScene sc, const float4* __restrict__ shO, const float4* __restrict__ shD,
                                                         const unsigned* __restrict__ slot_of, const unsigned* count_ptr, unsigned* head,
                                                         unsigned char* __restrict__ vis, uint2* spill, unsigned spill_stride, unsigned* ctrl,
@@ -425,7 +425,7 @@
     TraceRay r = idle_ray();
     int sp = 0, area_light = -1;
     const auto unoccluded = [&]() {
-        if (!slot_of) vis[slot] = 0;
+        if (!RENDER && !slot_of) vis[slot] = 0;
         return false;
     };
     persistent_rays<PF_MIN, START_MIN, LEAF_MIN, CHUNK>(
@@ -433,10 +433,10 @@
         [&](unsigned k) {
             pf_o = shO[k];
             pf_d = shD[k];
-            pf_slot = slot_of ? slot_of[k] : k;
+            pf_slot = RENDER ? __float_as_uint(pf_o.w) : (slot_of ? slot_of[k] : k);
         },
         [&]() {
-            r = ray_setup(f4_xyz(pf_o), f4_xyz(pf_d), pf_o.w);
+            r = ray_setup(f4_xyz(pf_o), f4_xyz(pf_d), RENDER ? 0.9999f : pf_o.w);
             area_light = (int)__float_as_uint(pf_d.w);
             slot = pf_slot;
             if (!root_hit(sc, r)) return unoccluded();
@@ -452,7 +452,7 @@
         },
         [&]() {
             if (leaf_any<SPHERES>(sc, cur & ~YK_LEAF_BIT, r, area_light)) {
-                vis[slot] = slot_of ? 2 : 1;
+                vis[slot] = (RENDER || slot_of) ? 2 : 1;
                 return false;
             }
             return pop_any(stk, sp, cur) || unoccluded();
@@ -500,7 +500,7 @@
 };
 
 template <int BLOCK, int LDS_DEPTH>
-__global__ __launch_bounds__(BLOCK) void k_whitted(DevScene sc, RenderParams prm, const uint32_t* pixel_xy, const uint32_t* sample_index_tab, PathBuffers cur,
+__global__ __launch_bounds__(BLOCK) void k_whitted(DevScene sc, RenderParams prm, const uint32_t* pixel_xy, const uint4* pixel_aux, const uint32_t* sample_index_tab, PathBuffers cur,
                                                    uint32_t n, float4* sample_buf, uint2* spill, unsigned spill_stride, unsigned* ctrl,
                                                    unsigned long long* counters) {
     __shared__ unsigned long long lds_stack[LDS_DEPTH * BLOCK];
@@ -512,7 +512,7 @@
         const float4 a = cur.rayO[i], b = cur.rayD[i], c = cur.thru[i];
         V3 o = f4_xyz(a), d = f4_xyz(b);
         const unsigned sid = __float_as_uint(b.w);
-        SamplerState st = path_sampler(prm, pixel_xy, sample_index_tab, cur.rngs[i], __float_as_uint(c.w), sid);
+        SamplerState st = path_sampler(prm, pixel_xy, pixel_aux, sample_index_tab, cur.rngs[i], __float_as_uint(c.w), sid);
         WhittedFrame frames[YK_WHITTED_MAX_DEPTH];
         int sp = 0;
         bool is_specular = false;
@@ -632,7 +632,7 @@
 }
 
 template <int BLOCK, int LDS_DEPTH>
-__global__ __launch_bounds__(BLOCK) void k_path_debug(DevScene sc, RenderParams prm, const uint32_t* pixel_xy, const uint32_t* sample_index_tab, PathBuffers cur,
+__global__ __launch_bounds__(BLOCK) void k_path_debug(DevScene sc, RenderParams prm, const uint32_t* pixel_xy, const uint4* pixel_aux, const uint32_t* sample_index_tab, PathBuffers cur,
                                                       uint32_t n, float4* sample_buf, uint32_t* out_counts, float4* out_rays, unsigned ray_cap,
                                                       uint32_t* out_n_rays, float min_len, uint2* spill, unsigned spill_stride, unsigned* ctrl) {
     __shared__ unsigned long long lds_stack[LDS_DEPTH * BLOCK];
@@ -643,7 +643,7 @@
         const float4 a = cur.rayO[i], b = cur.rayD[i], c = cur.thru[i];
         V3 o = f4_xyz(a), d = f4_xyz(b);
         const unsigned sid = __float_as_uint(b.w);
-        SamplerState st = path_sampler(prm, pixel_xy, sample_index_tab, cur.rngs[i], __float_as_uint(c.w), sid);
+        SamplerState st = path_sampler(prm, pixel_xy, pixel_aux, sample_index_tab, cur.rngs[i], __float_as_uint(c.w), sid);
         RGB L = RGB{0.0f, 0.0f, 0.0f}, beta = RGB{c.x, c.y, c.z};
         unsigned bounces = 0, n_closest = 0, k = 0, type = YK_RAY_DIRECT;
         bool specular_bounce = false, alive = prm.max_depth > 0;
@@ -729,28 +729,38 @@
 #undef YK_LAUNCH_CLOSEST
     }
 }
-void launch_whitted(hipStream_t s, unsigned grid, const DevScene& sc, const RenderParams& prm, const uint32_t* pixel_xy, const uint32_t* sample_index_tab,
+void launch_whitted(hipStream_t s, unsigned grid, const DevScene& sc, const RenderParams& prm, const uint32_t* pixel_xy, const uint4* pixel_aux, const uint32_t* sample_index_tab,
                     PathBuffers cur, uint32_t n, float4* sample_buf, uint2* spill, unsigned spill_stride, unsigned* ctrl, unsigned long long* counters) {
-    hipLaunchKernelGGL((k_whitted<TRACE_BLOCK, TRACE_LDS>), dim3(grid), dim3(TRACE_BLOCK), 0, s, sc, prm, pixel_xy, sample_index_tab, cur, n, sample_buf, spill,
+    hipLaunchKernelGGL((k_whitted<TRACE_BLOCK, TRACE_LDS>), dim3(grid), dim3(TRACE_BLOCK), 0, s, sc, prm, pixel_xy, pixel_aux, sample_index_tab, cur, n, sample_buf, spill,
                        spill_stride, ctrl, counters);
 }
 unsigned whitted_max_depth() { return YK_WHITTED_MAX_DEPTH; }
-void launch_path_debug(hipStream_t s, unsigned grid, const DevScene& sc, const RenderParams& prm, const uint32_t* pixel_xy, const uint32_t* sample_index_tab,
+void launch_path_debug(hipStream_t s, unsigned grid, const DevScene& sc, const RenderParams& prm, const uint32_t* pixel_xy, const uint4* pixel_aux, const uint32_t* sample_index_tab,
                        PathBuffers cur, uint32_t n, float4* sample_buf, uint32_t* out_counts, float4* out_rays, unsigned ray_cap, uint32_t* out_n_rays,
                        float min_len, uint2* spill, unsigned spill_stride, unsigned* ctrl) {
-    hipLaunchKernelGGL((k_path_debug<TRACE_BLOCK, TRACE_LDS>), dim3(grid), dim3(TRACE_BLOCK), 0, s, sc, prm, pixel_xy, sample_index_tab, cur, n, sample_buf,
+    hipLaunchKernelGGL((k_path_debug<TRACE_BLOCK, TRACE_LDS>), dim3(grid), dim3(TRACE_BLOCK), 0, s, sc, prm, pixel_xy, pixel_aux, sample_index_tab, cur, n, sample_buf,
                        out_counts, out_rays, ray_cap, out_n_rays, min_len, spill, spill_stride, ctrl);
 }
 void launch_trace_any(hipStream_t s, unsigned grid, const DevScene& sc, const float4* shO, const float4* shD, const unsigned* slot_of,
                       const unsigned* count_ptr, unsigned* head, unsigned char* vis, uint2* spill, unsigned spill_stride, unsigned* ctrl,
                       unsigned long long* shadow_counter, const unsigned* cancel_host) {
-#define YK_LAUNCH_ANY(SPH, WIDE)                                                                                                                       \
-    hipLaunchKernelGGL((k_trace_any_pt<TRACE_BLOCK, TRACE_ANY_LDS, TRACE_PF_MIN, TRACE_START_MIN, TRACE_LEAF_MIN, TRACE_CHUNK, SPH, WIDE>), dim3(grid),     \
+#define YK_LAUNCH_ANY(SPH, WIDE, RENDER)                                                                                                               \
+    hipLaunchKernelGGL((k_trace_any_pt<TRACE_BLOCK, TRACE_ANY_LDS, TRACE_PF_MIN, TRACE_START_MIN, TRACE_LEAF_MIN, TRACE_CHUNK, SPH, WIDE, RENDER>), dim3(grid), \
                        dim3(TRACE_BLOCK), 0, s, sc, shO, shD, slot_of, count_ptr, head, vis, spill, spill_stride, ctrl, shadow_counter, cancel_host)
     if (sc.spheres) {
-        if (sc.nodes4) YK_LAUNCH_ANY(true, true); else YK_LAUNCH_ANY(true, false);
+        if (sc.nodes4) YK_LAUNCH_ANY(true, true, false); else YK_LAUNCH_ANY(true, false, false);
     } else {
-        if (sc.nodes4) YK_LAUNCH_ANY(false, true); else YK_LAUNCH_ANY(false, false);
+        if (sc.nodes4) YK_LAUNCH_ANY(false, true, false); else YK_LAUNCH_ANY(false, false, false);
+    }
+}
+void launch_trace_any_render(hipStream_t s, unsigned grid, const DevScene& sc, const float4* shO, const float4* shD, const unsigned* count_ptr,
+                             unsigned* head, unsigned char* vis, uint2* spill, unsigned spill_stride, unsigned* ctrl, unsigned long long* shadow_counter,
+                             const unsigned* cancel_host) {
+    const unsigned* slot_of = nullptr;
+    if (sc.spheres) {
+        if (sc.nodes4) YK_LAUNCH_ANY(true, true, true); else YK_LAUNCH_ANY(true, false, true);
+    } else {
+        if (sc.nodes4) YK_LAUNCH_ANY(false, true, true); else YK_LAUNCH_ANY(false, false, true);
     }
 #undef YK_LAUNCH_ANY
 }
```

Result: no change. 2289 Mray/s (-0.2%).
